# FerrisMind/candle-video

Hardware: AMD Instinct MI355X
Metric: frames/sec end-to-end LTX-Video-2B 512x768x97; DiT step ms; VAE decode ms (higher is better)
Workload: dtype bf16; 1 GPU; LTX-Video-0.9.8-2B-distilled 512x768x97, 7 steps (configs.rs:223-240), untiled VAE decode; preset=0.9.8-2b-distilled, denoise_steps=7, parallelism=replicas x1 (no data-path collective)

## Files before the change

candle-video_amd/csrc/capi_ops.hip:

```cpp
#include "conv3d.h"
#include "../../include/ltxhip_ops.h"
#include "../../include/ltxhip_upsampler_st.h"
#include "../../include/ltxhip_stg.h"
#include "../../include/ltxhip_stepcache.h"

static inline int dtc(int d) { return d == 1 ? LTX_DT_BF16 : LTX_DT_F32; }

extern "C" int ltx_op_linear(const void* x, const void* w, const void* bias, void* y, int M, int N, int K, int dtype, int epi,
                             const void* resid, const float* gate, int rows_per_batch, ltx_stream stream) {
    if (!x || !w || !y) LTX_FAIL(LTX_ERR_ARG, "ltx_op_linear: null tensor");
    if (epi < 0 || epi > 3) LTX_FAIL(LTX_ERR_ARG, "ltx_op_linear: epi must be 0..3");
    if ((epi == 2 || epi == 3) && !resid) LTX_FAIL(LTX_ERR_ARG, "ltx_op_linear: residual epilogue needs resid");
    if (epi == 2 && (!gate || rows_per_batch < 1)) LTX_FAIL(LTX_ERR_ARG, "ltx_op_linear: gated epilogue needs gate");
    GemmArgs g; g.A = x; g.W = w; g.C = y; g.bias = bias; g.resid = resid; g.gate = gate;
    g.M = M; g.N = N; g.K = K; g.lda = K; g.ldc = N; g.ldr = N; g.rows_per_batch = rows_per_batch > 0 ? rows_per_batch : 1; g.gate_stride = N;
    return ltx_launch_gemm(g, dtc(dtype), epi, (hipStream_t)stream);
}

extern "C" int64_t ltx_op_ring_packed_bytes(int N, int K) { return (int64_t)ltx_ring_packed_bytes(N, K); }
extern "C" int ltx_op_ring_pack(const void* w, int N, int K, void* out, ltx_stream stream) { return ltx_pack_ring_weights(w, N, K, out, (hipStream_t)stream); }
extern "C" int ltx_op_linear_packed(const void* x, const void* w, const void* w_packed, const void* bias, void* y, int M, int N, int K, int epi,
                                    const void* resid, const float* gate, int rows_per_batch, ltx_stream stream) {
    if (!x || !w || !w_packed || !y) LTX_FAIL(LTX_ERR_ARG, "ltx_op_linear_packed: null tensor");
    if (epi < 0 || epi > 3) LTX_FAIL(LTX_ERR_ARG, "ltx_op_linear_packed: epi must be 0..3");
    if ((epi == 2 || epi == 3) && !resid) LTX_FAIL(LTX_ERR_ARG, "ltx_op_linear_packed: residual epilogue needs resid");
    if (epi == 2 && (!gate || rows_per_batch < 1)) LTX_FAIL(LTX_ERR_ARG, "ltx_op_linear_packed: gated epilogue needs gate");
    GemmArgs g; g.A = x; g.W = w; g.Wp = w_packed; g.C = y; g.bias = bias; g.resid = resid; g.gate = gate;
    g.M = M; g.N = N; g.K = K; g.lda = K; g.ldc = N; g.ldr = N; g.rows_per_batch = rows_per_batch > 0 ? rows_per_batch : 1; g.gate_stride = N;
    return ltx_launch_gemm(g, LTX_DT_BF16, epi, (hipStream_t)stream);
}

extern "C" int ltx_op_linear_rowsq(const void* x, const void* w, const void* bias, void* y, float* rowsq, int M, int N, int K, int dtype, int epi,
                                   const void* resid, const float* gate, int rows_per_batch, ltx_stream stream) {
    if (!x || !w || !y || !rowsq) LTX_FAIL(LTX_ERR_ARG, "ltx_op_linear_rowsq: null tensor");
    if (epi != 0 && epi != 2 && epi != 3) LTX_FAIL(LTX_ERR_ARG, "ltx_op_linear_rowsq: epi must be 0, 2 or 3");
    if (epi >= 2 && !resid) LTX_FAIL(LTX_ERR_ARG, "ltx_op_linear_rowsq: residual epilogue needs resid");
    if (epi == 2 && (!gate || rows_per_batch < 1)) LTX_FAIL(LTX_ERR_ARG, "ltx_op_linear_rowsq: gated epilogue needs gate");
    GemmArgs g; g.A = x; g.W = w; g.C = y; g.bias = bias; g.resid = resid; g.gate = gate; g.M = M; g.N = N; g.K = K; g.lda = K; g.ldc = N; g.ldr = N;
    g.rows_per_batch = rows_per_batch > 0 ? rows_per_batch : 1; g.gate_stride = N; g.rowsq = rowsq;
    return ltx_launch_gemm(g, dtc(dtype), epi, (hipStream_t)stream);
}
extern "C" int ltx_op_rowsq(const void* x, int64_t rows, int N, int ld, float* rowsq, int dtype, ltx_stream stream) {
    return ltx_launch_rowsq(x, dtc(dtype), rows, N, ld, rowsq, (hipStream_t)stream);
}

namespace {
GemmArgs fold_out_args(const void* x, const void* w, const void* bias, void* y, void* y2, float* rowsq, const float* scale2, int scale2_stride,
                       int M, int N, int K, const void* resid, const float* gate, int rows_per_batch) {
    GemmArgs g; g.A = x; g.W = w; g.C = y; g.bias = bias; g.resid = resid; g.gate = gate; g.M = M; g.N = N; g.K = K; g.lda = K; g.ldc = N; g.ldr = N;
    g.rows_per_batch = rows_per_batch > 0 ? rows_per_batch : 1; g.gate_stride = N; g.rowsq = rowsq;
    g.C2 = y2; g.scale2 = scale2; g.scale2_stride = scale2_stride;
    return g;
}
GemmArgs fold_in_args(const void* x, const void* w, void* y, const float* rs_sq, int rs_n, int rs_D, float eps, const float* cvec, int cvec_stride,
                      int M, int N, int K, int rows_per_batch) {
    GemmArgs g; g.A = x; g.W = w; g.C = y; g.M = M; g.N = N; g.K = K; g.lda = K; g.ldc = N;
    g.rows_per_batch = rows_per_batch > 0 ? rows_per_batch : 1;
// ... 98 lines not shown
    a.presum = presum; a.presum_n = presum_n;
    return ltx_launch_rownorm(a, dtc(dtype), (hipStream_t)stream);
}

extern "C" int ltx_op_timestep_embedding(const float* timesteps_host, int n, int vae_flavour, float multiplier, int dtype, void* out, ltx_stream stream) {
    if (!timesteps_host || !out) LTX_FAIL(LTX_ERR_ARG, "ltx_op_timestep_embedding: null argument");
    if (n < 1 || n > 8) LTX_FAIL(LTX_ERR_ARG, "ltx_op_timestep_embedding: batch must be 1..8");
    float tab[128]; ltx_sinusoid_table(vae_flavour, tab);
    float* dtab = nullptr;
    HIP_TRY(hipMalloc((void**)&dtab, sizeof(tab)));
    int rc = LTX_OK;
    if (hipMemcpy(dtab, tab, sizeof(tab), hipMemcpyHostToDevice) != hipSuccess) rc = LTX_ERR_HIP;
    if (rc == LTX_OK) {
        TimeVec tv; tv.n = n;
        for (int i = 0; i < n; ++i) tv.t[i] = timesteps_host[i];
        rc = ltx_launch_sinusoid(out, dtc(dtype), tv, dtab, 128, dtc(dtype) == LTX_DT_BF16, multiplier, (hipStream_t)stream);
        if (rc == LTX_OK && hipStreamSynchronize((hipStream_t)stream) != hipSuccess) rc = LTX_ERR_HIP;
    }
    (void)hipFree(dtab);
    return rc;
}

extern "C" int ltx_op_qknorm_rope(void* x, int64_t rows, int D, int ld, const void* weight, float eps,
                                  const float* cos, const float* sin, int dtype, ltx_stream stream) {
    if (!x || !weight) LTX_FAIL(LTX_ERR_ARG, "ltx_op_qknorm_rope: null tensor");
    QkNormRopeArgs a; a.x = x; a.rows = rows; a.D = D; a.ld = ld; a.nseg = 1; a.w0 = weight; a.eps = eps; a.cos = cos; a.sin = sin;
    return ltx_launch_qknorm_rope(a, dtc(dtype), (hipStream_t)stream);
}

extern "C" int ltx_op_qknorm_rope_segs(void* x, int64_t rows, int D, int ld, int nseg, int64_t seg_stride, const void* w0, const void* w1, const void* w0b,
                                       float eps, const float* cos, const float* sin, float out_scale0, int dtype, ltx_stream stream) {
    if (!x || !w0) LTX_FAIL(LTX_ERR_ARG, "ltx_op_qknorm_rope_segs: null tensor");
    if ((cos == nullptr) != (sin == nullptr) || seg_stride < 0) LTX_FAIL(LTX_ERR_ARG, "ltx_op_qknorm_rope_segs: cos and sin go together; seg_stride >= 0");
    QkNormRopeArgs a; a.x = x; a.rows = rows; a.D = D; a.ld = ld; a.nseg = nseg; a.seg_stride = seg_stride; a.w0 = w0; a.w1 = w1; a.w0b = w0b;
    a.eps = eps; a.cos = cos; a.sin = sin; a.out_scale0 = out_scale0;
    return ltx_launch_qknorm_rope(a, dtc(dtype), (hipStream_t)stream);
}

extern "C" int ltx_op_norm_route(int64_t rows, int D, int dtype, int kind, int flags, int act, int64_t rows_per_batch, int presum_n, int nparts, char* name, int cap) {
    if (!name || cap < 1 || rows < 1 || D < 1 || presum_n < 0 || nparts < 0 || (flags & ~7)) LTX_FAIL(LTX_ERR_ARG, "ltx_op_norm_route: bad argument");
    NormRouteArgs r;
    r.dtype = dtc(dtype); r.rows = rows; r.D = D; r.kind = kind; r.act = act; r.rows_per_batch = rows_per_batch > 0 ? rows_per_batch : 1;
    r.scale = (flags & LTX_NORM_SCALE) != 0; r.shift = (flags & LTX_NORM_SHIFT) != 0; r.weight = (flags & LTX_NORM_WEIGHT) != 0;
    r.presum = presum_n != 0; r.presum_n = presum_n; r.parts = nparts != 0; r.nparts = nparts;
    snprintf(name, (size_t)cap, "%s", ltx_rownorm_route_name(ltx_rownorm_route(r).route));
    return LTX_OK;
}
extern "C" int ltx_op_qknorm_route(int64_t rows, int D, int dtype, char* name, int cap) {
    if (!name || cap < 1 || rows < 1 || D < 1) LTX_FAIL(LTX_ERR_ARG, "ltx_op_qknorm_route: bad argument");
    snprintf(name, (size_t)cap, "%s", ltx_qknorm_route_name(ltx_qknorm_route(dtc(dtype), rows, D, nullptr)));
    return LTX_OK;
}

extern "C" int ltx_op_rope_table(float* cos, float* sin, const float* coords, int B, int F, int H, int W, int D,
                                 const float* rope_scale_host, ltx_stream stream) {
    if (!cos || !sin) LTX_FAIL(LTX_ERR_ARG, "ltx_op_rope_table: null tensor");
    int steps = D / 6; if (steps < 1) steps = 1;
    std::vector<float> fr(steps);
    const float theta_ln = (float)std::log(10000.0);
    for (int i = 0; i < steps; ++i) {
        float lin = steps <= 1 ? 0.0f : (float)i * (float)(1.0 / (double)(steps - 1));
        fr[i] = (float)std::exp((double)(lin * theta_ln)) * (float)(M_PI / 2.0);
    }
    float* dfr = nullptr;
    HIP_TRY(hipMalloc((void**)&dfr, sizeof(float) * steps));
    HIP_TRY(hipMemcpy(dfr, fr.data(), sizeof(float) * steps, hipMemcpyHostToDevice));
    RopeTableArgs r; r.cos = cos; r.sin = sin; r.freqs = dfr; r.B = B; r.D = D;
    if (coords) { r.use_coords = 1; r.coords = coords; r.F = 1; r.H = 1; r.W = F * H * W;
                  r.gscale[0] = (float)(1.0 / 20.0); r.gscale[1] = (float)(1.0 / 2048.0); r.gscale[2] = (float)(1.0 / 2048.0); }
    else { r.F = F; r.H = H; r.W = W;
           if (rope_scale_host) { r.gscale[0] = (float)((double)rope_scale_host[0] / 20.0); r.gscale[1] = (float)((double)rope_scale_host[1] / 2048.0); r.gscale[2] = (float)((double)rope_scale_host[2] / 2048.0); } }
    int rc = ltx_launch_rope_table(r, (hipStream_t)stream);
    hipError_t e = hipStreamSynchronize((hipStream_t)stream);
    (void)hipFree(dfr);
    if (rc != LTX_OK) return rc;
    if (e != hipSuccess) { ltx_set_error(hipGetErrorString(e)); return LTX_ERR_HIP; }
    return LTX_OK;
}

extern "C" int ltx_op_attention(const void* q, const void* k, const void* v, void* o, int B, int Sq, int Sk, int heads, int hd,
                                int ldq, int ldk, int ldv, int ldo, float scale, const float* key_bias, int dtype, ltx_stream stream) {
    if (!q || !k || !v || !o) LTX_FAIL(LTX_ERR_ARG, "ltx_op_attention: null tensor");
    AttnArgs a; a.q = q; a.k = k; a.v = v; a.o = o; a.ldq = ldq; a.ldk = ldk; a.ldv = ldv; a.ldo = ldo;
    a.B = B; a.Sq = Sq; a.Sk = Sk; a.heads = heads; a.hd = hd; a.scale = scale; a.bias = key_bias;
    return ltx_launch_attention(a, dtc(dtype), (hipStream_t)stream);
}

extern "C" int ltx_op_attention_rowsq(const void* q, const void* k, const void* v, void* o, int B, int Sq, int Sk, int heads, int hd,
                                      int ldq, int ldk, int ldv, int ldo, float scale, const float* key_bias,
                                      const float* q_rowsq, int q_rowsq_n, int q_rowsq_D, float q_rowsq_eps, ltx_stream stream) {
    if (!q || !k || !v || !o || !q_rowsq) LTX_FAIL(LTX_ERR_ARG, "ltx_op_attention_rowsq: null tensor");
    AttnArgs a; a.q = q; a.k = k; a.v = v; a.o = o; a.ldq = ldq; a.ldk = ldk; a.ldv = ldv; a.ldo = ldo;
    a.B = B; a.Sq = Sq; a.Sk = Sk; a.heads = heads; a.hd = hd; a.scale = scale; a.bias = key_bias;
    a.q_rowsq = q_rowsq; a.q_rowsq_n = q_rowsq_n; a.q_rowsq_D = q_rowsq_D; a.q_rowsq_eps = q_rowsq_eps;
    return ltx_launch_attention(a, LTX_DT_BF16, (hipStream_t)stream);
}

extern "C" int ltx_op_attention_compact(const void* q, const void* k, const void* v, void* o, int B, int Sq, int Sk, int heads, int hd,
                                        int ldq, int ldk, int ldv, int ldo, float scale, const float* key_bias,
                                        const float* q_rowsq, int q_rowsq_n, int q_rowsq_D, float q_rowsq_eps, int* counts_out, ltx_stream stream) {
    if (!q || !k || !v || !o || !key_bias) LTX_FAIL(LTX_ERR_ARG, "ltx_op_attention_compact: null tensor");
    if (!ltx_attention_cross64_ok(hd, Sk) || B < 1 || ldk != heads * hd || ldv != heads * hd) LTX_FAIL(LTX_ERR_ARG, "ltx_op_attention_compact: bf16, head_dim 64, at most 128 keys, dense k / v rows");
    hipStream_t s = (hipStream_t)stream;
    const int D = heads * hd;
    void *kc = nullptr, *vc = nullptr, *bc = nullptr, *idx = nullptr, *cnt = nullptr;
    auto free_all = [&]() { for (void* p : {kc, vc, bc, idx, cnt}) if (p) (void)hipFree(p); };
    const size_t rows = (size_t)B * Sk;
    if (hipMalloc(&kc, rows * D * 2) != hipSuccess || hipMalloc(&vc, rows * D * 2) != hipSuccess || hipMalloc(&bc, rows * 4) != hipSuccess ||
        hipMalloc(&idx, rows * 4) != hipSuccess || hipMalloc(&cnt, (size_t)B * 4) != hipSuccess) { free_all(); LTX_FAIL(LTX_ERR_HIP, "hipMalloc"); }
    int rc = ltx_launch_key_compact(key_bias, B, Sk, (int*)idx, (int*)cnt, (float*)bc, s);
    if (rc == LTX_OK) rc = ltx_launch_gather_rows(k, kc, (const int*)idx, (const int*)cnt, 1, B, Sk, D * 2, s);
    if (rc == LTX_OK) rc = ltx_launch_gather_rows(v, vc, (const int*)idx, (const int*)cnt, 1, B, Sk, D * 2, s);
    if (rc == LTX_OK) {
        AttnArgs a; a.q = q; a.k = kc; a.v = vc; a.o = o; a.ldq = ldq; a.ldk = D; a.ldv = D; a.ldo = ldo;
        a.B = B; a.Sq = Sq; a.Sk = Sk; a.heads = heads; a.hd = hd; a.scale = scale; a.bias = (const float*)bc; a.k_count = (const int*)cnt;
        if (q_rowsq) { a.q_rowsq = q_rowsq; a.q_rowsq_n = q_rowsq_n; a.q_rowsq_D = q_rowsq_D; a.q_rowsq_eps = q_rowsq_eps; }
        rc = ltx_launch_attention(a, LTX_DT_BF16, s);
    }
    if (rc == LTX_OK && counts_out && hipMemcpyAsync(counts_out, cnt, (size_t)B * 4, hipMemcpyDeviceToDevice, s) != hipSuccess) rc = LTX_ERR_HIP;
    const hipError_t e = hipStreamSynchronize(s);
    free_all();
    if (rc != LTX_OK) return rc;
    if (e != hipSuccess) { ltx_set_error(hipGetErrorString(e)); return LTX_ERR_HIP; }
    return LTX_OK;
}

extern "C" int ltx_op_xattn_fold_route(int dtype, int head_dim, int heads, int D, int KP, int B, int compact, int* fold) {
    if (!fold) LTX_FAIL(LTX_ERR_ARG, "ltx_op_xattn_fold_route: null result");
    *fold = ltx_xattn_fold_route(dtc(dtype), head_dim, heads, D, KP, B, compact != 0) ? 1 : 0;
    return LTX_OK;
// ... 201 lines not shown
```

candle-video_amd/csrc/dit.hip:

```cpp
#include <cstring>
#include <deque>
#include "model_util.h"
#include "options.h"
#include "../../include/ltxhip_cond.h"
#include "../../include/ltxhip_stg.h"
#include "../../include/ltxhip_stepcache.h"
#include "../host/step_cache.h"
#include "lora.h"

struct DitBlock {
    LinearW qkv1, o1, q2, kv2, o2, ff1, ff2;
    void *nq1 = nullptr, *nk1 = nullptr, *nq2 = nullptr, *nk2 = nullptr;
};

struct DitCtx {
    const void* enc = nullptr; const float* mask = nullptr;
    int B = 0, K = 0, iodt = 0; bool valid = false;
    bool fold_q2 = false;
    DevBuf kv, bias;
    bool compact = false;
    DevBuf kvc, biasc, kidx, kcount;
    bool fold_vo = false, vo_oom = false; int KP = 0, fold_opt = 0;
    DevBuf vo, votab; std::vector<XFoldPtrs> votab_host; int counts_host[8] = {0};
    void release() { kv.release(); bias.release(); kvc.release(); biasc.release(); kidx.release(); kcount.release(); vo.release(); votab.release(); valid = false; }
};

struct DitTimeEntry {
    float t[8] = {0}; int B = 0; hipStream_t stream = nullptr; bool valid = false; uint64_t used = 0;
    DevBuf ada, adaf;
    DevBuf cfold; bool cfold_valid = false;
    void release() { ada.release(); adaf.release(); cfold.release(); valid = cfold_valid = false; }
};
struct DitWfold {
    float t = 0.f; hipStream_t stream = nullptr; bool valid = false; uint64_t used = 0; DevBuf w;
    void release() { w.release(); valid = false; }
};
constexpr int kDitTimeEntries = 64;
struct DitGroupEntry {
    std::vector<float> t; int B = 0, G = 0; hipStream_t stream = nullptr; bool valid = false; uint64_t used = 0;
    DevBuf ada, adaf, cfold; bool cfold_valid = false;
    void release() { ada.release(); adaf.release(); cfold.release(); valid = cfold_valid = false; }
};
constexpr int kDitGroupEntries = 8;

struct ltx_dit {
    ltx_dit_config cfg{};
    int dtype = LTX_DT_BF16;
    int device = 0;
    int D = 0;
    LinearW proj_in, te1, te2, te_lin, cap1, cap2, proj_out;
    void* sst_final = nullptr;
    void* sst_blocks = nullptr;
    std::vector<DitBlock> blocks;
    float* rope_freqs = nullptr;
    float* inv_freq = nullptr;
    std::vector<int> skip_blocks;
    int stg_mode = LTX_STG_TRANSFORMER_BLOCK;
    std::deque<DitCtx> ctxs;
    bool ctx_mode = false;
    std::deque<DitTimeEntry> tcache; uint64_t tclock = 0;
    std::deque<DitWfold> wcache;
    std::deque<DitGroupEntry> gcache;
    bool wfold_off = false;
    struct { bool valid = false; const float* coords = nullptr; float rs[3] = {0, 0, 0}; bool has_rs = false; int B = 0, S = 0, F = 0, H = 0, W = 0; hipStream_t stream = nullptr; } rope_key;
    uint64_t weights_epoch = 0;
    void invalidate_weight_derived() {
        ++weights_epoch;
        for (auto& e : wcache) e.valid = false;
        for (auto& e : ctxs) e.valid = false;
        for (auto& e : tcache) e.cfold_valid = false;
        for (auto& e : gcache) e.cfold_valid = false;
    }
    void release_scaled_weights() { for (auto& e : wcache) e.release(); }
    void release_caches() { auto all = [](auto& c) { for (auto& e : c) e.release(); c.clear(); }; all(ctxs); all(tcache); all(wcache); all(gcache); }
    std::vector<void*> owned;
    struct LoraSlots { void* base[7] = {nullptr}; void* merged[7] = {nullptr}; };
    std::vector<LoraSlots> lora_w;
    int n_adapters = 0;
    DevBuf xin, encin, h, n, qkv, attn, ff, c1, encp, kv2, tproj, e1, emb, embs, temb, ada, adaf, cosb, sinb, bias, orig, orig_hsq, outT, rsq, hsq, parts;
    void free_all() {
        for (void* p : owned) if (p) (void)hipFree(p);
        owned.clear();
        for (auto& ls : lora_w) for (void*& p : ls.merged) if (p) { (void)hipFree(p); p = nullptr; }
        lora_w.clear();
        DevBuf* bs[] = {&xin, &encin, &h, &n, &qkv, &attn, &ff, &c1, &encp, &kv2, &tproj, &e1, &emb, &embs, &temb, &ada, &adaf, &cosb, &sinb, &bias, &orig, &orig_hsq, &outT, &rsq, &hsq, &parts};
        for (DevBuf* b : bs) b->release();
        release_caches();
    }
};

struct ltx_step_cache {
    ltx_dit* dit = nullptr;
    struct Row { bool valid = false; int S = 0; uint64_t epoch = 0; };
    std::vector<Row> rows;
    DevBuf prev, resid, parts, sums;
    int64_t prev_rows = 0; int resid_S = 0;
    double* host = nullptr;
    hipStream_t stream = nullptr; bool used = false;
    StepCacheState st;
    void forget() { st = StepCacheState(); for (auto& r : rows) r.valid = false; }
    void* resid_row(int row) const { return (char*)resid.p + (size_t)row * resid_S * dit->D * ltx_dt_size(dit->dtype); }
    const char* row_unusable(int row, int S) const {
        const Row& r = rows[(size_t)row];
        if (!r.valid) return "holds no residual (never computed, or the cache was reset)";
        if (r.S != S) return "holds the residual of another sequence length";
        if (r.epoch != dit->weights_epoch) return "holds a residual of other weights (the adapters changed)";
        return nullptr;
    }
};
struct StepCacheUse { ltx_step_cache* c = nullptr; int row0 = 0; bool reuse = false; };

namespace {

int own_linear(ltx_dit* m, const WeightMap& wm, const std::string& prefix, int in, int out, LinearW* l) {
    LTX_TRY(ltx_load_linear(wm, prefix, in, out, m->dtype, l));
    m->owned.push_back(l->w); if (l->b) m->owned.push_back(l->b);
    return LTX_OK;
// ... 376 lines not shown
    *out = ctx;
    if (ctx) return LTX_OK;
    if (m->ctxs.size() >= 4 || !m->ctx_mode) { for (auto& e : m->ctxs) e.valid = false; }
    for (auto& e : m->ctxs) if (!e.valid) { ctx = &e; break; }
    if (!ctx) { m->ctxs.emplace_back(); ctx = &m->ctxs.back(); }
    ctx->enc = enc; ctx->mask = enc_mask; ctx->B = B; ctx->K = K; ctx->iodt = p.iodt; ctx->fold_q2 = p.fold_q2;
    ctx->fold_opt = ltx_opt().xattn_fold_vo; ctx->fold_vo = false; ctx->KP = 0; ctx->vo_oom = false;
    LTX_TRY(ctx->kv.ensure((size_t)L * MK * 2 * D * esz)); LTX_TRY(ctx->bias.ensure(MK * sizeof(float)));
    ctx->compact = enc_mask && dt == LTX_DT_BF16 && ltx_attention_cross64_ok(c.attention_head_dim, K) && ltx_opt().xattn_compact;
    if (ctx->compact) {
        LTX_TRY(ctx->kvc.ensure((size_t)L * MK * 2 * D * esz)); LTX_TRY(ctx->biasc.ensure(MK * sizeof(float)));
        LTX_TRY(ctx->kidx.ensure(MK * sizeof(int))); LTX_TRY(ctx->kcount.ensure((size_t)B * sizeof(int)));
    }
    if (enc_mask) LTX_TRY(ltx_launch_mask_bias(ctx->bias.as<float>(), enc_mask, MK, s));
    if (ctx->compact) LTX_TRY(ltx_launch_key_compact(ctx->bias.as<float>(), B, K, ctx->kidx.as<int>(), ctx->kcount.as<int>(), ctx->biasc.as<float>(), s));
    const int H = c.num_attention_heads, hd = c.attention_head_dim;
    if (ctx->compact && B <= 8 && ltx_xattn_fold_route(dt, hd, H, D, 32, B, true)) {
        HIP_TRY(hipMemcpyAsync(ctx->counts_host, ctx->kcount.p, (size_t)B * sizeof(int), hipMemcpyDeviceToHost, s));
        HIP_TRY(hipStreamSynchronize(s));
        ctx->KP = ltx_xattn_fold_kp(ctx->counts_host, B);
        ctx->fold_vo = vo_wanted(m, p, ctx);
        if (ctx->fold_vo) {
            (void)ltx_take_oom();
            int rc = ctx->vo.ensure((size_t)L * B * D * H * ctx->KP * esz);
            if (rc == LTX_OK) rc = ctx->votab.ensure((size_t)L * sizeof(XFoldPtrs));
            if (rc != LTX_OK) {
                if (!ltx_take_oom()) return rc;
                ctx->fold_vo = false; ctx->vo_oom = true;
            }
        }
    }
    LTX_TRY(ltx_launch_cast(enc, p.iodt, m->encin.p, dt, MK * c.caption_channels, s));
    LTX_TRY(ltx_linear(m->cap1, m->encin.p, c.caption_channels, m->c1.p, D, (int)MK, dt, EPI_GELU, s));
    LTX_TRY(ltx_linear(m->cap2, m->c1.p, D, m->encp.p, D, (int)MK, dt, EPI_BIAS, s));
    for (int l = 0; l < L; ++l) {
        void* kvl = (char*)ctx->kv.p + (size_t)l * MK * 2 * D * esz;
        LTX_TRY(ltx_linear(m->blocks[l].kv2, m->encp.p, D, kvl, 2 * D, (int)MK, dt, EPI_BIAS, s));
        QkNormRopeArgs k2; k2.x = kvl; k2.rows = MK; k2.D = D; k2.ld = 2 * D; k2.nseg = 1; k2.w0 = m->blocks[l].nk2; k2.eps = 1e-5f;
        if (p.fold_q2) k2.w0b = m->blocks[l].nq2;
        LTX_TRY(ltx_launch_qknorm_rope(k2, dt, s));
    }
    if (ctx->compact) LTX_TRY(ltx_launch_gather_rows(ctx->kv.p, ctx->kvc.p, ctx->kidx.as<int>(), ctx->kcount.as<int>(), L, B, K, (int)(2 * D * esz), s));
    if (ctx->fold_vo) {
        ctx->votab_host.resize(L);
        for (int l = 0; l < L; ++l) ctx->votab_host[l] = XFoldPtrs{m->blocks[l].o2.w, (const char*)ctx->kvc.p + ((size_t)l * MK * 2 * D + D) * esz};
        HIP_TRY(hipMemcpyAsync(ctx->votab.p, ctx->votab_host.data(), (size_t)L * sizeof(XFoldPtrs), hipMemcpyHostToDevice, s));
        XFoldArgs fa; fa.tab = ctx->votab.as<XFoldPtrs>(); fa.vo = ctx->vo.p; fa.L = L; fa.B = B; fa.K = K; fa.ldv = 2 * D; fa.D = D; fa.H = H; fa.KP = ctx->KP;
        LTX_TRY(ltx_launch_xattn_fold(fa, s));
    }
    ctx->valid = true;
    *out = ctx;
    return LTX_OK;
}
int rope_tables(ltx_dit* m, const DitPlan& p, int num_frames, int height, int width, const float* rope_scale, const float* video_coords, hipStream_t s) {
    const ltx_dit_config& c = m->cfg;
    auto& rk = m->rope_key;
    const bool same = m->ctx_mode && rk.valid && rk.coords == video_coords && rk.B == p.B && rk.S == p.S && rk.F == num_frames && rk.H == height && rk.W == width &&
                      rk.stream == s && rk.has_rs == (rope_scale != nullptr) && (!rope_scale || !memcmp(rk.rs, rope_scale, sizeof(rk.rs)));
    if (same) return LTX_OK;
    rk.valid = false;
    RopeTableArgs r;
    r.cos = m->cosb.as<float>(); r.sin = m->sinb.as<float>(); r.freqs = m->rope_freqs;
    r.B = p.B; r.D = p.D;
    if (video_coords) {
        r.use_coords = 1; r.coords = video_coords; r.F = 1; r.H = 1; r.W = p.S;
        r.gscale[0] = (float)(1.0 / 20.0); r.gscale[1] = (float)(1.0 / 2048.0); r.gscale[2] = (float)(1.0 / 2048.0);
    } else {
        r.F = num_frames; r.H = height; r.W = width;
        if (rope_scale) {
            r.gscale[0] = (float)((double)rope_scale[0] * c.patch_size_t / 20.0);
            r.gscale[1] = (float)((double)rope_scale[1] * c.patch_size / 2048.0);
            r.gscale[2] = (float)((double)rope_scale[2] * c.patch_size / 2048.0);
        }
    }
    LTX_TRY(ltx_launch_rope_table(r, s));
    rk.coords = video_coords; rk.B = p.B; rk.S = p.S; rk.F = num_frames; rk.H = height; rk.W = width; rk.stream = s;
    rk.has_rs = rope_scale != nullptr; if (rope_scale) memcpy(rk.rs, rope_scale, sizeof(rk.rs));
    rk.valid = m->ctx_mode;
    return LTX_OK;
}

struct DitCarry {
    bool hsq_valid = false;
    bool hs_valid = false;
    bool hsq_saved = false;
    bool pending = false; const float* pend_gate = nullptr; const void* pend_bias = nullptr;
    void take_pending(RowNormArgs& rn, const ltx_dit* m, const DitPlan& p) {
        if (!pending) return;
        rn.parts = m->parts.as<float>(); rn.nparts = p.ff2_parts; rn.part_stride = p.M * p.D; rn.d_bias = pend_bias; rn.d_gate = pend_gate; rn.d_gate_stride = 6 * p.D;
        rn.x_out = m->h.p; pending = false;
    }
};
struct DitLayerIn {
    DitTables tab; const DitWfold* we = nullptr; const DitCtx* ctx = nullptr; const float* skip_layer_mask = nullptr;
    bool fold_vo = false;
};
bool block_runs(const ltx_dit* m, const float* skip_layer_mask, int B, int l) {
    for (int sb : m->skip_blocks) if (sb == l) return false;
    if (m->stg_mode != LTX_STG_TRANSFORMER_BLOCK) return true;
    bool all = skip_layer_mask != nullptr;
    for (int b = 0; all && b < B; ++b) all = skip_layer_mask[(size_t)l * B + b] == 1.f;
    return !all;
}
int next_block(const ltx_dit* m, const float* skip_layer_mask, int B, int l) {
    for (int n = l + 1; n < m->cfg.num_layers; ++n) if (block_runs(m, skip_layer_mask, B, n)) return n;
    return -1;
}

int dit_block(ltx_dit* m, const DitPlan& p, int l, const DitLayerIn& in, DitCarry& st, hipStream_t s) {
    const ltx_dit_config& c = m->cfg;
    const int dt = p.dt, D = p.D, B = p.B, S = p.S, NB = p.NB, H = c.num_attention_heads, hd = c.attention_head_dim;
    const int64_t M = p.M; const size_t esz = ltx_dt_size(dt);
    const bool wf = in.we != nullptr, fold_out = p.nfold && !wf;
    const DitBlock& b = m->blocks[l];
    TimeVec mv; mv.n = B; bool any = false;
    for (int i = 0; i < 8; ++i) mv.t[i] = 0.f;
    if (in.skip_layer_mask) for (int bb = 0; bb < B; ++bb) { mv.t[bb] = in.skip_layer_mask[(size_t)l * B + bb]; any |= mv.t[bb] != 0.f; }
    const bool stg_attn = any && m->stg_mode != LTX_STG_TRANSFORMER_BLOCK;
    unsigned char pert[8] = {0};
    if (stg_attn) { for (int bb = 0; bb < B; ++bb) pert[bb] = mv.t[bb] != 0.f; any = false; }
    if (any) {
        HIP_TRY(hipMemcpyAsync(m->orig.p, m->h.p, M * D * esz, hipMemcpyDeviceToDevice, s));
        st.hsq_saved = p.presum && st.hsq_valid;
        if (st.hsq_saved) { LTX_TRY(m->orig_hsq.ensure(M * (D / 128) * sizeof(float))); HIP_TRY(hipMemcpyAsync(m->orig_hsq.p, m->hsq.p, M * (D / 128) * sizeof(float), hipMemcpyDeviceToDevice, s)); }
    }
    const int ln = fold_out ? next_block(m, in.skip_layer_mask, B, l) : -1;
    const float* ada = in.tab.ada + (size_t)l * NB * 6 * D;
    DitOperands x{m->h.p, m->n.p, m->qkv.p, m->attn.p, m->ff.p, m->rsq.as<float>(), m->hsq.as<float>(), m->parts.as<float>(), ada,
                  ln >= 0 ? in.tab.ada + (size_t)ln * NB * 6 * D : nullptr, p.nfold ? in.tab.cfold + (size_t)l * NB * 7 * D : nullptr,
                  wf ? (const char*)in.we->w.p + (size_t)l * 7 * D * D * esz : nullptr, c.norm_eps};
    const DitForm fold_in_form = wf ? kFold2 : kFold1;
    RowNormArgs rn; rn.x = m->h.p; rn.y = m->n.p; rn.rows = M; rn.D = D; rn.ldx = D; rn.ldy = D;
    rn.kind = 0; rn.eps = c.norm_eps; rn.shift = ada; rn.scale = ada + D; rn.rows_per_batch = p.Sg; rn.mod_stride = 6 * D;
    if (p.presum && st.hsq_valid) { rn.presum = m->hsq.as<float>(); rn.presum_n = D / 128; }
    const bool fold1 = p.nfold && st.hsq_valid && (wf || st.hs_valid);
    if (!fold1) { st.take_pending(rn, m, p); LTX_TRY(ltx_launch_rownorm(rn, dt, s)); }
    st.hs_valid = false;
    rn.parts = nullptr; rn.nparts = 0; rn.x_out = nullptr; rn.d_bias = nullptr; rn.d_gate = nullptr;
    LTX_TRY(ltx_launch_gemm(gemm_qkv1(p, fold1 ? fold_in_form : kPass, b, x), dt, EPI_BIAS, s));
    const float attn_scale = 1.0f / std::sqrt((float)hd);
    QkNormRopeArgs qa; qa.x = m->qkv.p; qa.rows = M; qa.D = D; qa.ld = p.ldqkv; qa.seg_stride = p.seg; qa.nseg = 2; qa.w0 = b.nq1; qa.w1 = b.nk1;
    qa.eps = 1e-5f; qa.cos = m->cosb.as<float>(); qa.sin = m->sinb.as<float>();
    if (p.fold_q) qa.out_scale0 = attn_scale * 1.4426950408889634f;
    LTX_TRY(ltx_launch_qknorm_rope(qa, dt, s));
    AttnArgs at; at.q = m->qkv.p; at.k = (char*)m->qkv.p + (size_t)p.seg * esz; at.v = (char*)m->qkv.p + (size_t)2 * p.seg * esz; at.o = m->attn.p;
    at.ldq = at.ldk = at.ldv = p.ldqkv; at.ldo = D; at.B = B; at.Sq = S; at.Sk = S; at.heads = H; at.hd = hd; at.scale = attn_scale;
    at.q_prescaled = p.fold_q ? 1 : 0;
    if (!stg_attn) LTX_TRY(ltx_launch_attention(at, dt, s));
    else {
        auto for_runs = [&](bool perturbed, auto&& fn) -> int {
            for (int b0 = 0; b0 < B; ++b0) {
                int b1 = b0;
                while (b1 < B && (pert[b1] != 0) == perturbed) ++b1;
                if (b1 > b0) { LTX_TRY(fn(b0, b1)); b0 = b1; }
            }
            return LTX_OK;
        };
        LTX_TRY(for_runs(false, [&](int b0, int b1) {
            AttnArgs ar = at; ar.B = b1 - b0;
            const size_t in_off = (size_t)b0 * S * p.ldqkv * esz;
            ar.q = (const char*)at.q + in_off; ar.k = (const char*)at.k + in_off; ar.v = (const char*)at.v + in_off; ar.o = (char*)at.o + (size_t)b0 * S * D * esz;
            return ltx_launch_attention(ar, dt, s);
        }));
        if (m->stg_mode == LTX_STG_ATTENTION_VALUES) LTX_TRY(ltx_launch_stg_fill(m->attn.p, D, at.v, p.ldqkv, pert, B, S, D, dt, s));
        else if (!fold1) LTX_TRY(ltx_launch_stg_fill(m->attn.p, D, m->n.p, D, pert, B, S, D, dt, s));
        else
            LTX_TRY(for_runs(true, [&](int b0, int b1) {
                RowNormArgs rp = rn; rp.presum = nullptr; rp.presum_n = 0;
                const size_t row_off = (size_t)b0 * S * D * esz, tab_off = (size_t)b0 * (NB / B) * 6 * D;
                rp.x = (const char*)m->h.p + row_off; rp.y = (char*)m->attn.p + row_off; rp.rows = (int64_t)(b1 - b0) * S;
                rp.shift = ada + tab_off; rp.scale = ada + D + tab_off;
                return ltx_launch_rownorm(rp, dt, s);
            }));
    }
    LTX_TRY(ltx_linear(b.o1, m->attn.p, D, m->h.p, D, (int)M, dt, EPI_GATE_RESID, s, m->h.p, D, ada + 2 * D, 6 * D, p.Sg));
    st.hsq_valid = false;
    const DitCtx* ctx = in.ctx;
    const char* kvl = (const char*)(ctx->compact ? ctx->kvc.p : ctx->kv.p) + (size_t)l * p.MK * 2 * D * esz;
    AttnArgs ax; ax.q = m->qkv.p; ax.k = kvl; ax.v = kvl + (size_t)D * esz; ax.o = m->attn.p;
    ax.ldq = D; ax.ldk = ax.ldv = 2 * D; ax.ldo = D; ax.B = B; ax.Sq = S; ax.Sk = p.K; ax.heads = H; ax.hd = hd; ax.scale = attn_scale;
    ax.bias = ctx->mask ? ctx->bias.as<float>() : nullptr;
    if (ctx->compact) { ax.bias = ctx->biasc.as<float>(); ax.k_count = ctx->kcount.as<int>(); }
    const int HK = H * ctx->KP;
    if (in.fold_vo) { ax.p_out = m->attn.p; ax.ldp = HK; ax.o = nullptr; }
    if (p.fold_q2) {
        LTX_TRY(ltx_launch_gemm(gemm_q2(p, b, x), dt, EPI_BIAS, s));
        ax.q_rowsq = m->rsq.as<float>(); ax.q_rowsq_n = D / 128; ax.q_rowsq_D = D; ax.q_rowsq_eps = 1e-5f;
    } else {
        LTX_TRY(linear_of(b.q2, gemm_q2(p, b, x), dt, EPI_BIAS, s));
        QkNormRopeArgs q2; q2.x = m->qkv.p; q2.rows = M; q2.D = D; q2.ld = D; q2.nseg = 1; q2.w0 = b.nq2; q2.eps = 1e-5f;
        LTX_TRY(ltx_launch_qknorm_rope(q2, dt, s));
    }
    LTX_TRY(ltx_launch_attention(ax, dt, s));
    if (in.fold_vo) {
        for (int bb = 0; bb < B; ++bb) {
            const DitVo vo{(const char*)ctx->vo.p + (size_t)l * B * D * HK * esz, HK, bb};
            LTX_TRY(ltx_launch_gemm(gemm_o2(p, fold_out ? kFold1 : kPass, b, x, &vo), dt, EPI_RESID, s));
        }
        st.hs_valid = fold_out;
    } else if (fold_out) { LTX_TRY(ltx_launch_gemm(gemm_o2(p, kFold1, b, x), dt, EPI_RESID, s)); st.hs_valid = true; }
    else LTX_TRY(linear_of(b.o2, gemm_o2(p, kPass, b, x), dt, EPI_RESID, s));
    st.hsq_valid = p.presum;
    if (p.nfold && st.hsq_valid && (wf || st.hs_valid)) LTX_TRY(ltx_launch_gemm(gemm_ff1(p, fold_in_form, b, x), dt, EPI_GELU, s));
    else {
        rn.shift = ada + 3 * D; rn.scale = ada + 4 * D;
        rn.presum = nullptr; rn.presum_n = 0;
        if (p.presum && st.hsq_valid) { rn.presum = m->hsq.as<float>(); rn.presum_n = D / 128; }
        LTX_TRY(ltx_launch_rownorm(rn, dt, s));
        LTX_TRY(linear_of(b.ff1, gemm_ff1(p, kPass, b, x), dt, EPI_GELU, s));
    }
    st.hs_valid = false;
    if (p.defer_ff2) {
        LTX_TRY(ltx_launch_gemm(gemm_ff2(p, kDefer, b, x), dt, EPI_BIAS, s));
        st.pending = true; st.pend_gate = ada + 5 * D; st.pend_bias = b.ff2.b;
    } else if (ln >= 0) { LTX_TRY(ltx_launch_gemm(gemm_ff2(p, kFold1, b, x), dt, EPI_GATE_RESID, s)); st.hs_valid = true; }
    else LTX_TRY(linear_of(b.ff2, gemm_ff2(p, kPass, b, x), dt, EPI_GATE_RESID, s));
    st.hsq_valid = p.presum;
    if (!any) return LTX_OK;
    LTX_TRY(ltx_launch_skip_blend(m->h.p, m->orig.p, mv, S, D, dt, s));
    bool binary = true;
    for (int bb = 0; bb < B; ++bb) binary &= mv.t[bb] == 0.f || mv.t[bb] == 1.f;
    if (st.hsq_valid && st.hsq_saved && binary) {
        const size_t rowb = (size_t)S * (D / 128) * sizeof(float);
        for (int bb = 0; bb < B; ++bb)
            if (mv.t[bb] == 1.f) HIP_TRY(hipMemcpyAsync((char*)m->hsq.p + bb * rowb, (const char*)m->orig_hsq.p + bb * rowb, rowb, hipMemcpyDeviceToDevice, s));
    } else st.hsq_valid = false;
    st.hs_valid = false;
    if (fold_out && st.hsq_valid && ln >= 0) { LTX_TRY(ltx_launch_mod_scale(m->h.p, x.ada_next + D, 6 * D, m->n.p, NB, p.Sg, D, dt, s)); st.hs_valid = true; }
    return LTX_OK;
}

int dit_forward_b8(ltx_dit* m, const void* hidden, const void* enc, const float* timestep, int G,
                   const float* enc_mask, int B, int S, int K, int num_frames, int height, int width,
                   const float* rope_scale, const float* video_coords, const float* skip_layer_mask,
                   ltx_dtype io_dtype, void* out, ltx_stream stream, const StepCacheUse* sc = nullptr) {
    if (B < 1 || B > 8) LTX_FAIL(LTX_ERR_ARG, "ltx_dit_forward: internal batch chunk must be 1..8");
    if (S < 1 || K < 1) LTX_FAIL(LTX_ERR_ARG, "ltx_dit_forward: empty sequence");
    if (!video_coords && (int64_t)num_frames * height * width != S)
        LTX_FAIL(LTX_ERR_ARG, "ltx_dit_forward: num_frames*height*width must equal S when video_coords is absent");
    HIP_TRY(hipSetDevice(m->device));
    if (G < 1 || S % G != 0) LTX_FAIL(LTX_ERR_ARG, "ltx_dit_forward: the modulation groups must divide the sequence");
    hipStream_t s = (hipStream_t)stream;
    const ltx_dit_config& c = m->cfg;
    const DitPlan p = ltx_dit_plan(c, m->dtype, io_dtype == LTX_BF16 ? LTX_DT_BF16 : LTX_DT_F32, B, S, K, G, skip_layer_mask != nullptr);
    const int dt = p.dt, D = p.D, L = c.num_layers;
    const int64_t M = p.M, MK = p.MK; const size_t esz = ltx_dt_size(dt);
    const size_t nte = p.NB == p.B ? (size_t)p.B : 8;
    const size_t MD = M * D * esz, KD = MK * D * esz, part = M * (D / 128) * sizeof(float), rope = M * (D / 2) * sizeof(float);
    const std::pair<DevBuf*, size_t> ws[] = {
        {&m->xin, M * c.in_channels * esz}, {&m->encin, MK * c.caption_channels * esz}, {&m->h, MD}, {&m->n, MD}, {&m->qkv, 3 * MD}, {&m->attn, MD}, {&m->ff, 4 * MD},
        {&m->c1, KD}, {&m->encp, KD}, {&m->kv2, 2 * KD}, {&m->tproj, nte * 256 * esz}, {&m->e1, nte * D * esz}, {&m->emb, nte * D * esz}, {&m->embs, nte * D * esz},
        {&m->temb, nte * 6 * D * esz}, {&m->cosb, rope}, {&m->sinb, rope}, {&m->bias, MK * sizeof(float)}, {&m->outT, M * c.out_channels * esz},
        {&m->rsq, p.fold_q2 ? part : 0}, {&m->hsq, p.presum ? part : 0}, {&m->parts, p.defer_ff2 ? (size_t)p.ff2_parts * M * D * sizeof(float) : 0}, {&m->orig, skip_layer_mask ? MD : 0}};
    for (const auto& w : ws) LTX_TRY(w.first->ensure(w.second));
    const bool reuse = sc && sc->reuse;
    if (reuse) {
        for (int b = 0; b < B; ++b)
            if (const char* why = sc->c->row_unusable(sc->row0 + b, S))
                LTX_FAIL(LTX_ERR_ARG, "ltx_dit_forward_cached: reuse asked of cache row " + std::to_string(sc->row0 + b) + ", which " + why);
    } else if (sc) {
        ltx_step_cache* k = sc->c;
        if (k->resid_S != S) { for (auto& r : k->rows) r.valid = false; k->resid_S = S; }
        LTX_TRY(k->resid.ensure(k->rows.size() * (size_t)S * D * esz));
        for (int b = 0; b < B; ++b) k->rows[(size_t)sc->row0 + b].valid = false;
    }

    LTX_TRY(ltx_launch_cast(hidden, p.iodt, m->xin.p, dt, p.M * c.in_channels, s));
    if (reuse) LTX_TRY(ltx_linear(m->proj_in, m->xin.p, c.in_channels, m->h.p, D, (int)p.M, dt, EPI_RESID, s, sc->c->resid_row(sc->row0), D));
    else LTX_TRY(ltx_linear(m->proj_in, m->xin.p, c.in_channels, m->h.p, D, (int)p.M, dt, EPI_BIAS, s));
    if (sc && !reuse) HIP_TRY(hipMemcpyAsync(sc->c->resid_row(sc->row0), m->h.p, MD, hipMemcpyDeviceToDevice, s));

    DitLayerIn in; in.skip_layer_mask = skip_layer_mask;
    DitPlan pt = p; if (reuse) pt.nfold = false;
    LTX_TRY(G == 1 ? time_tables(m, pt, timestep, B, s, &in.tab) : group_tables(m, pt, timestep, s, &in.tab));
    DitCtx* ctx = nullptr;
    DitCarry st;
    if (!reuse) {
        LTX_TRY(scaled_weights(m, p, timestep, in.tab.ada, s, &in.we));
        LTX_TRY(text_context(m, p, enc, enc_mask, s, &ctx)); in.ctx = ctx;
        in.fold_vo = ctx->fold_vo;
        LTX_TRY(rope_tables(m, p, num_frames, height, width, rope_scale, video_coords, s));

        for (int l = 0; l < L; ++l)
            if (block_runs(m, skip_layer_mask, B, l)) LTX_TRY(dit_block(m, p, l, in, st, s));
    }
    const bool resid_late = sc && !reuse && st.pending;
    if (sc && !reuse && !resid_late) LTX_TRY(ltx_launch_step_residual(m->h.p, sc->c->resid_row(sc->row0), p.M, D, dt, s));

    RowNormArgs rn; rn.x = m->h.p; rn.y = m->n.p; rn.rows = p.M; rn.D = D; rn.ldx = D; rn.ldy = D;
    rn.kind = 1; rn.eps = 1e-6f; rn.shift = in.tab.adaf; rn.scale = in.tab.adaf + (size_t)p.NB * D;
    rn.rows_per_batch = p.Sg; rn.mod_stride = D;
    st.take_pending(rn, m, p);
    LTX_TRY(ltx_launch_rownorm(rn, dt, s));
    if (resid_late) LTX_TRY(ltx_launch_step_residual(m->h.p, sc->c->resid_row(sc->row0), p.M, D, dt, s));
    if (sc && !reuse)
        for (int b = 0; b < B; ++b) sc->c->rows[(size_t)sc->row0 + b] = {true, S, m->weights_epoch};
    void* dst = p.iodt == dt ? out : m->outT.p;
    LTX_TRY(ltx_linear(m->proj_out, m->n.p, D, dst, c.out_channels, (int)p.M, dt, EPI_BIAS, s));
    if (p.iodt != dt) LTX_TRY(ltx_launch_cast(m->outT.p, dt, out, p.iodt, p.M * c.out_channels, s));
    if (ctx && !m->ctx_mode) ctx->valid = false;
    return LTX_OK;
// ... 6 lines not shown
    const size_t esz = io_dtype == LTX_BF16 ? 2 : 4;
    const int L = m->cfg.num_layers;
    if (skip_layer_mask && m->stg_mode != LTX_STG_TRANSFORMER_BLOCK)
        for (size_t i = 0; i < (size_t)L * B; ++i)
            if (skip_layer_mask[i] != 0.f && skip_layer_mask[i] != 1.f)
                LTX_FAIL(LTX_ERR_ARG, "ltx_dit_forward: skip_layer_mask[" + std::to_string(i / B) + ", " + std::to_string(i % B) + "] = " + std::to_string(skip_layer_mask[i]) +
                                      ": the attention STG modes take 0 and 1 only (fractional masks: LTX_STG_TRANSFORMER_BLOCK)");
    std::vector<float> mask_chunk;
    float t_row[8];
    for (int b0 = 0; b0 < B; b0 += 8) {
        const int bc = B - b0 < 8 ? B - b0 : 8;
        const float* slm = skip_layer_mask;
        if (skip_layer_mask && bc != B) {
            mask_chunk.resize((size_t)L * bc);
            for (int l = 0; l < L; ++l) for (int b = 0; b < bc; ++b) mask_chunk[(size_t)l * bc + b] = skip_layer_mask[(size_t)l * B + b0 + b];
            slm = mask_chunk.data();
        }
        const float* tc = timestep + (size_t)b0 * (F ? F : 1);
        int G = 1;
        if (F) {
            bool uniform = true;
            for (int b = 0; b < bc; ++b) for (int f = 1; f < F; ++f) uniform = uniform && memcmp(&tc[(size_t)b * F + f], &tc[(size_t)b * F], sizeof(float)) == 0;
            if (uniform) { for (int b = 0; b < bc; ++b) t_row[b] = tc[(size_t)b * F]; tc = t_row; } else G = F;
        }
        StepCacheUse use; if (sc) { use = *sc; use.row0 += b0; }
        LTX_TRY(dit_forward_b8(m, (const char*)hidden + (size_t)b0 * S * m->cfg.in_channels * esz, enc ? (const char*)enc + (size_t)b0 * K * m->cfg.caption_channels * esz : nullptr,
                               tc, G, enc_mask ? enc_mask + (size_t)b0 * K : nullptr, bc, S, K, num_frames, height, width, rope_scale,
                               video_coords ? video_coords + (size_t)b0 * S * 3 : nullptr, slm, io_dtype,
                               (char*)out + (size_t)b0 * S * m->cfg.out_channels * esz, stream, sc ? &use : nullptr));
    }
    return LTX_OK;
}

}

extern "C" int ltx_dit_forward(ltx_dit* m, const void* hidden, const void* enc, const float* timestep,
                               const float* enc_mask, int B, int S, int K, int num_frames, int height, int width,
                               const float* rope_scale, const float* video_coords, const float* skip_layer_mask,
                               ltx_dtype io_dtype, void* out, ltx_stream stream) {
    if (!m || !hidden || !enc || !timestep || !out) LTX_FAIL(LTX_ERR_ARG, "ltx_dit_forward: null argument");
    if (B < 1) LTX_FAIL(LTX_ERR_ARG, "ltx_dit_forward: batch must be at least 1");
    return dit_forward_chunks(m, hidden, enc, timestep, 0, enc_mask, B, S, K, num_frames, height, width, rope_scale, video_coords, skip_layer_mask, io_dtype, out, stream);
}

extern "C" int ltx_dit_forward_frames(ltx_dit* m, const void* hidden, const void* enc, const float* timestep,
                                      const float* enc_mask, int B, int S, int K, int num_frames, int height, int width,
                                      const float* rope_scale, const float* video_coords, const float* skip_layer_mask,
                                      ltx_dtype io_dtype, void* out, ltx_stream stream) {
    if (!m || !hidden || !enc || !timestep || !out) LTX_FAIL(LTX_ERR_ARG, "ltx_dit_forward_frames: null argument");
    if (B < 1) LTX_FAIL(LTX_ERR_ARG, "ltx_dit_forward_frames: batch must be at least 1");
    if (num_frames < 1 || height < 1 || width < 1 || (int64_t)num_frames * height * width != S)
        LTX_FAIL(LTX_ERR_ARG, "ltx_dit_forward_frames: S must equal num_frames*height*width (tokens in pack order, with or without video_coords)");
    return dit_forward_chunks(m, hidden, enc, timestep, num_frames, enc_mask, B, S, K, num_frames, height, width, rope_scale, video_coords, skip_layer_mask, io_dtype, out, stream);
}

extern "C" int ltx_dit_context_cache(ltx_dit* m, int enable) {
    if (!m) LTX_FAIL(LTX_ERR_ARG, "ltx_dit_context_cache: null handle");
    for (auto& e : m->ctxs) e.valid = false;
    m->rope_key.valid = false;
    m->ctx_mode = enable != 0;
    return LTX_OK;
}

extern "C" void ltx_step_cache_params_default(ltx_step_cache_params* p) {
    if (!p) return;
    const StepCachePolicy d;
    p->rel_l1_thresh = d.thresh; for (int k = 0; k < 5; ++k) p->coeff[k] = d.coeff[k];
    p->pattern = nullptr; p->n_pattern = 0;
}

extern "C" int ltx_step_cache_create(ltx_dit* dit, int rows, ltx_step_cache** out) {
    if (!dit || !out) LTX_FAIL(LTX_ERR_ARG, "ltx_step_cache_create: null argument");
    *out = nullptr;
    if (rows < 1) LTX_FAIL(LTX_ERR_ARG, "ltx_step_cache_create: rows must be at least 1, got " + std::to_string(rows));
    if (!ltx_step_measure_blocks(1, dit->D, dit->dtype))
        LTX_FAIL(LTX_ERR_UNSUPPORTED, "ltx_step_cache_create: inner dim " + std::to_string(dit->D) + " is not a multiple of 128 the measure kernel serves");
    HIP_TRY(hipSetDevice(dit->device));
    ltx_step_cache* c = new ltx_step_cache();
    c->dit = dit; c->rows.resize((size_t)rows);
    int rc = c->sums.ensure(2 * sizeof(double));
    if (rc == LTX_OK && hipHostMalloc((void**)&c->host, 2 * sizeof(double), hipHostMallocDefault) != hipSuccess) {
        (void)hipGetLastError(); ltx_set_error("ltx_step_cache_create: hipHostMalloc of the result pair"); rc = LTX_ERR_HIP;
    }
    if (rc != LTX_OK) { c->sums.release(); delete c; return rc; }
    *out = c;
    return LTX_OK;
}

extern "C" void ltx_step_cache_destroy(ltx_step_cache* c) {
    if (!c) return;
    (void)hipSetDevice(c->dit->device);
    if (c->used) (void)hipStreamSynchronize(c->stream);
    c->prev.release(); c->resid.release(); c->parts.release(); c->sums.release();
    if (c->host) (void)hipHostFree(c->host);
    delete c;
}

extern "C" int ltx_step_cache_reset(ltx_step_cache* c) {
    if (!c) LTX_FAIL(LTX_ERR_ARG, "ltx_step_cache_reset: null handle");
    c->forget();
    return LTX_OK;
}

static int step_cache_policy_of(const ltx_step_cache_params* params, const char* who, StepCachePolicy* pol) {
    if (!params) LTX_FAIL(LTX_ERR_ARG, std::string(who) + ": null step cache parameters");
    pol->thresh = params->rel_l1_thresh; for (int k = 0; k < 5; ++k) pol->coeff[k] = params->coeff[k];
// ... 192 lines not shown
```

candle-video_amd/csrc/kernels.h:

```cpp
#pragma once
#include <hip/hip_runtime.h>
#include <hip/hip_ext.h>
#include <stdint.h>

enum { LTX_DT_F32 = 0, LTX_DT_BF16 = 1 };
static inline size_t ltx_dt_size(int dt) { return dt == LTX_DT_BF16 ? 2 : 4; }

enum { LTX_PROF_GEMM = 0, LTX_PROF_CONV = 1, LTX_PROF_ATTN_SELF = 2, LTX_PROF_ATTN_CROSS = 3, LTX_PROF_ROWNORM = 4, LTX_PROF_NKINDS = 5 };
bool ltx_prof_begin(int kind, double work, hipStream_t s, void** token);
void ltx_prof_end(void* token, hipStream_t s);
enum { LTX_PROFK_GEMM128 = 0, LTX_PROFK_GEMM_BIG = 1, LTX_PROFK_GEMM_P8 = 2, LTX_PROFK_CONV_HALO = 3, LTX_PROFK_GEMM_ASM = 4, LTX_PROFK_GEMM_ASM16 = 5, LTX_PROFK_GEMM_RING = 6, LTX_PROFK_N = 7 };
void ltx_prof_kernel(int which);
bool ltx_prof_kernel_events(hipEvent_t* a, hipEvent_t* b);
#define LTX_LAUNCH_TIMED(kernel, grid, block, shmem, stream, ...) do {                                           \
        hipEvent_t _pa = nullptr, _pb = nullptr;                                                                   \
        if (ltx_prof_kernel_events(&_pa, &_pb)) hipExtLaunchKernelGGL(kernel, grid, block, shmem, stream, _pa, _pb, 0, __VA_ARGS__); \
        else hipLaunchKernelGGL(kernel, grid, block, shmem, stream, __VA_ARGS__);                                  \
    } while (0)

enum { EPI_BIAS = 0, EPI_GELU = 1, EPI_GATE_RESID = 2, EPI_RESID = 3, EPI_D2S = 4, EPI_UNPATCH = 5, EPI_S2D = 6, EPI_D2S_G = 7 };

struct GemmArgs {
    const void* A = nullptr;
    const void* W = nullptr;
// ... 72 lines not shown
struct RowNormArgs {
    const void* x = nullptr; void* y = nullptr;
    int64_t rows = 0; int D = 0; int ldx = 0, ldy = 0;
    int kind = 0;
    float eps = 1e-6f;
    const void* weight = nullptr;
    const float* scale = nullptr;
    const float* shift = nullptr;
    int64_t rows_per_batch = 1; int mod_stride = 0;
    int act = 0;
    const float* presum = nullptr; int presum_n = 0;
    const float* parts = nullptr; int nparts = 0; int64_t part_stride = 0;
    const void* d_bias = nullptr; const float* d_gate = nullptr; int d_gate_stride = 0; void* x_out = nullptr;
};
int ltx_launch_rownorm(const RowNormArgs& a, int dtype, hipStream_t s);

enum NormRoute { NORM_REFUSED = 0, NORM_NARROW, NORM_BLOCK, NORM_WIDE, NORM_REREAD, NORM_PRESUM, NORM_PRESUM_LEAN,
                 NORM_WIDE_DEFER, NORM_WIDE_DEFER4, NORM_BLOCK_DEFER, NORM_BLOCK_DEFER4,
                 NORM_WIDE_ROWS };
struct NormRouteArgs {
    int dtype = LTX_DT_BF16; int64_t rows = 0; int D = 0; int kind = 0;
    bool scale = false, shift = false, weight = false; int act = 0; int64_t rows_per_batch = 1;
    bool presum = false; int presum_n = 0;
    bool parts = false; int nparts = 0;
};
struct NormDecision {
    NormRoute route = NORM_REFUSED; const char* why = nullptr;
    int presum_r = 4; bool presum_wide = false, presum_nt = false;
};
NormRouteArgs ltx_rownorm_route_args(const RowNormArgs& a, int dtype);
NormDecision ltx_rownorm_route(const NormRouteArgs& r);
const char* ltx_rownorm_route_name(NormRoute r);

struct StepMeasureArgs {
    const void* h = nullptr; void* prev = nullptr;
    const float* shift = nullptr; const float* scale = nullptr; int mod_stride = 0;
    int64_t rows = 0; int D = 0; int64_t rows_per_batch = 1; float eps = 1e-6f; int first = 0;
    double* part = nullptr;
};
int64_t ltx_step_measure_blocks(int64_t rows, int D, int dtype);
int ltx_launch_step_measure(const StepMeasureArgs& a, int dtype, hipStream_t s);
int ltx_launch_step_measure_finish(const double* part, int64_t nblk, double* sums, hipStream_t s);
int ltx_launch_step_residual(const void* h, void* r, int64_t rows, int D, int dtype, hipStream_t s);

struct QkNormRopeArgs {
    void* x = nullptr;
    int64_t rows = 0; int D = 0; int ld = 0; int nseg = 1;
    int64_t seg_stride = 0;
    const void* w0 = nullptr; const void* w1 = nullptr;
    const void* w0b = nullptr;
    float eps = 1e-5f;
    const float* cos = nullptr; const float* sin = nullptr;
    float out_scale0 = 1.f;
};
int ltx_launch_qknorm_rope(const QkNormRopeArgs& a, int dtype, hipStream_t s);
enum QkNormRoute { QKNORM_REFUSED = 0, QKNORM_BLOCK, QKNORM_FUSED4, QKNORM_FUSED8, QKNORM_CACHED, QKNORM_REREAD };
QkNormRoute ltx_qknorm_route(int dtype, int64_t rows, int D, const char** why);
const char* ltx_qknorm_route_name(QkNormRoute r);

struct RopeTableArgs {
    float* cos = nullptr; float* sin = nullptr;
    const float* coords = nullptr;
    const float* freqs = nullptr;
    int B = 1, F = 1, H = 1, W = 1, D = 0;
    int use_coords = 0;
    float gscale[3] = {1.f, 1.f, 1.f};
};
int ltx_launch_rope_table(const RopeTableArgs& a, hipStream_t s);

struct AttnArgs {
    const void* q = nullptr; const void* k = nullptr; const void* v = nullptr; void* o = nullptr;
    int ldq = 0, ldk = 0, ldv = 0, ldo = 0;
    int B = 1, Sq = 0, Sk = 0, heads = 0, hd = 0;
    float scale = 1.f;
    const float* bias = nullptr;
    const float* bias2d = nullptr;
    int q_prescaled = 0;
    int xcd_heads = 0;
    int wide_o = 0;
    const float* q_rowsq = nullptr; int q_rowsq_n = 0, q_rowsq_D = 0; float q_rowsq_eps = 0.f;
    const int* k_count = nullptr;
    void* p_out = nullptr; int ldp = 0;
    const int* gate_flag = nullptr; int gate_ticket = 0;
};
bool ltx_attention_q128_fits(const AttnArgs& a);
int ltx_launch_attention_q128(const AttnArgs& a, hipStream_t s, int** flag_out, int* ticket_out);
int ltx_q64_fallback_read(unsigned long long* out, int reset);
int ltx_q128_fallback_read(unsigned long long* out, int reset);
int ltx_attention_q128_prepare();
int ltx_launch_attention(const AttnArgs& a, int dtype, hipStream_t s);
int ltx_launch_attention_q64(const AttnArgs& a, hipStream_t s);
bool ltx_attention_q64_fits(const AttnArgs& a);
bool ltx_attention_prescale_ok(int hd);
bool ltx_attention_cross64_ok(int hd, int Sk);
bool ltx_xattn_fold_route(int dtype, int head_dim, int heads, int D, int KP, int B, bool compact);
int ltx_xattn_fold_kp(const int* counts_host, int B);
struct XFoldPtrs { const void* w; const void* v; };
struct XFoldArgs { const XFoldPtrs* tab = nullptr; void* vo = nullptr; int L = 0, B = 0, K = 0, ldv = 0, D = 0, H = 0, KP = 0; };
int ltx_launch_xattn_fold(const XFoldArgs& a, hipStream_t s);
bool ltx_attention_rowsq_ok(int hd, int Sk, int D);

constexpr int LTX_MAX_BATCH = 16;
struct TimeVec { float t[LTX_MAX_BATCH]; int n; };
int ltx_launch_gguf_dequant(const void* blocks_dev, int ggml_type, int64_t numel, void* dst, int dst_dtype, hipStream_t s);
int ltx_launch_sinusoid(void* out, int dtype, const TimeVec& tv, const float* tab, int half, int round_t, float tmul, hipStream_t s);
int ltx_launch_silu(const void* x, void* y, int64_t n, int dtype, hipStream_t s);
int ltx_launch_noise_inject(const void* x, void* y, const float* noise, const void* scale, const void* resid, int64_t rows, int C, int64_t HW, int dtype, hipStream_t s);
int ltx_launch_cast(const void* x, int xdt, void* y, int ydt, int64_t n, hipStream_t s);
int ltx_launch_ada(float* out, const void* tables, const void* temb, int nl, int B, int width, int dtype, hipStream_t s);
int ltx_launch_mask_bias(float* out, const float* mask, int64_t n, hipStream_t s);
int ltx_launch_key_compact(const float* bias, int B, int K, int* idx, int* count, float* bias_c, hipStream_t s);
int ltx_launch_gather_rows(const void* src, void* dst, const int* idx, const int* count, int nl, int B, int K, int row_bytes, hipStream_t s);
int ltx_launch_skip_blend(void* h, const void* orig, const TimeVec& m, int64_t rows_per_batch, int D, int dtype, hipStream_t s);
struct StgRows { int n; int b[LTX_MAX_BATCH]; };
int ltx_launch_stg_fill(void* dst, int ldd, const void* src, int lds, const unsigned char* rows_host, int B, int64_t S, int D, int dtype, hipStream_t s);
int ltx_launch_scale_cols(const void* W, const float* scale, void* out, int64_t N, int K, int dtype, hipStream_t s);
int ltx_launch_mod_scale(const void* h, const float* scale, int scale_stride, void* y, int B, int64_t rows_per_batch, int D, int dtype, hipStream_t s);

struct GroupIdx { int v[128]; };
// ... 52 lines not shown
```

candle-video_amd/csrc/model_util.h:

```cpp
#pragma once
#include <map>
#include <memory>
#include <string>
#include <vector>
#include <cmath>
#include "common.h"
#include "kernels.h"
#include "../../include/ltxhip.h"
#include "../../include/ltxhip_stepcache.h"

void ltx_note_oom();
bool ltx_take_oom();

struct DevBuf {
    void* p = nullptr;
    size_t bytes = 0;
    int ensure(size_t n) {
        if (n <= bytes) return LTX_OK;
        if (p) { HIP_TRY(hipDeviceSynchronize()); HIP_TRY(hipFree(p)); p = nullptr; bytes = 0; }
        const hipError_t e = hipMalloc(&p, n);
        if (e != hipSuccess) {
            p = nullptr;
            if (e == hipErrorOutOfMemory) ltx_note_oom();
            (void)hipGetLastError();
// ... 9 lines not shown
struct LinearW {
    void* w = nullptr;
    void* b = nullptr;
    int in = 0, out = 0;
    mutable std::shared_ptr<void> wp;
    mutable bool wp_tried = false;
};

struct WeightMap {
    std::map<std::string, const ltx_weight*> m;
    WeightMap(const ltx_weight* w, size_t n) { for (size_t i = 0; i < n; ++i) if (w[i].name) m[w[i].name] = &w[i]; }
    const ltx_weight* find(const std::string& k) const { auto it = m.find(k); return it == m.end() ? nullptr : it->second; }
};

static inline int64_t ltx_numel(const ltx_weight* w) {
    int64_t n = 1;
    for (int i = 0; i < w->ndim; ++i) n *= w->shape[i];
    return n;
}

int ltx_upload_cast(const ltx_weight* w, void* dst, int dst_dtype, int64_t expect_numel, const std::string& name);
int ltx_load_tensor(const WeightMap& wm, const std::string& name, int64_t numel, int dtype, void** out, bool optional = false);
int ltx_load_linear(const WeightMap& wm, const std::string& prefix, int in, int out, int dtype, LinearW* l);
int ltx_stage_src(const ltx_weight* w, const void** dev_src, void** temp_to_free);

inline void ltx_sinusoid_table(int vae_flavour, float tab[128]) {
    if (!vae_flavour) {
        for (int i = 0; i < 128; ++i) { const float ex = (float)i / 128.0f; const float pw = (float)std::pow(10000.0, (double)ex); tab[i] = 1.0f / pw; }
    } else {
        const float coef = (float)(-std::log(10000.0) / 128.0);
        for (int i = 0; i < 128; ++i) { const float x = (float)i * coef; tab[i] = (float)std::exp((double)x); }
    }
}

int ltx_linear(const LinearW& l, const void* x, int lda, void* y, int ldc, int M, int dtype, int epi, hipStream_t s,
               const void* resid = nullptr, int ldr = 0, const float* gate = nullptr, int gate_stride = 0, int rows_per_batch = 1,
               float* rowsq = nullptr);

struct DitPlan {
    int dt = 0, iodt = 0, D = 0, B = 0, S = 0, K = 0;
    int64_t M = 0, MK = 0;
    int NB = 0, Sg = 0;
    int64_t seg = 0; int ldqkv = 0;
    bool fold_q2 = false;
    bool presum = false;
    bool nfold = false;
    bool defer_ff2 = false; int ff2_parts = 1;
    bool dense_qkv = false;
    bool fold_q = false;
};
DitPlan ltx_dit_plan(const ltx_dit_config& c, int dt, int iodt, int B, int S, int K, int G, bool skip_mask);

int ltx_step_cache_params_check(const ltx_step_cache_params* params, const char* who);

int ltx_pipeline_schedule(const ltx_pipeline_params* p, int S, std::vector<float>* sig, std::vector<int64_t>* ts);
```

candle-video_amd/csrc/options.cpp:

```cpp
#include "options.h"
#include <atomic>
#include <cstdio>
#include <cstdlib>
#include <cstring>
#include <map>
#include <mutex>
#include <string>
#include "errors.h"

namespace {
std::mutex g_mu;
LtxOptions g_opt;
std::atomic<bool> g_loaded{false};
std::map<std::string, int> g_exp;

struct ListBit { const char* name; unsigned bit; };
const ListBit kFam[] = {{"asm16", LTX_FAM_ASM16}, {"ring", LTX_FAM_RING}, {"p8", LTX_FAM_P8}, {"halo", LTX_FAM_HALO}, {"halo_out", LTX_FAM_HALO_OUT}, {"big", LTX_FAM_BIG}};
const ListBit kAttn[] = {{"q64", LTX_ATTN_Q64}, {"q128", LTX_ATTN_Q128}, {"cross", LTX_ATTN_CROSS}, {"pipe", LTX_ATTN_PIPE}};

template <size_t N> bool parse_list(const char* v, const ListBit (&tab)[N], unsigned* out) {
    unsigned bits = 0;
    std::string s(v ? v : "");
    size_t p = 0;
    while (p < s.size()) {
        size_t q = s.find('+', p); if (q == std::string::npos) q = s.size();
        const std::string item = s.substr(p, q - p);
        bool ok = item.empty();
        for (const auto& t : tab) if (item == t.name) { bits |= t.bit; ok = true; }
        if (!ok) return false;
        p = q + 1;
    }
    *out = bits;
    return true;
}

struct IntField { const char* name; int LtxOptions::*field; };
const IntField kInts[] = {
    {"gemm_tune", &LtxOptions::gemm_tune}, {"gemm_wide_epi", &LtxOptions::gemm_wide_epi}, {"gemm_trace", &LtxOptions::gemm_trace},
    {"attn_q64_big", &LtxOptions::attn_q64_big}, {"vae_tile_batch", &LtxOptions::vae_tile_batch}, {"prof_kernel_events", &LtxOptions::prof_kernel_events}, {"ff2_defer", &LtxOptions::ff2_defer},
    {"gemm_splitk", &LtxOptions::gemm_splitk}, {"q2_fold", &LtxOptions::q2_fold}, {"norm_presum", &LtxOptions::norm_presum}, {"norm_lean", &LtxOptions::norm_lean},
    {"xattn_compact", &LtxOptions::xattn_compact}, {"xattn_fold_vo", &LtxOptions::xattn_fold_vo}, {"dense_qkv", &LtxOptions::dense_qkv}, {"vae_fuse_norm", &LtxOptions::vae_fuse_norm}, {"t5_attn_mfma", &LtxOptions::t5_attn_mfma}, {"guidance_batch", &LtxOptions::guidance_batch}, {"norm_fold", &LtxOptions::norm_fold}, {"norm_fold_copies", &LtxOptions::norm_fold_copies}, {"attn_q64_stream", &LtxOptions::attn_q64_stream},
};

bool set_one(LtxOptions& o, const std::string& key, const char* value) {
    static const LtxOptions dflt;
    for (const auto& f : kInts) if (key == f.name) {
        if (!value) { o.*(f.field) = dflt.*(f.field); return true; }
        char* end = nullptr; const long v = strtol(value, &end, 10);
        if (end == value || *end) return false;
        o.*(f.field) = (int)v; return true;
    }
    if (key == "gemm_plan") {
        if (!value) { o.gemm_plan[0] = 0; return true; }
        if (strlen(value) >= sizeof(o.gemm_plan)) return false;
        strcpy(o.gemm_plan, value); return true;
    }
    if (key == "gemm_off") return value ? parse_list(value, kFam, &o.gemm_off) : (o.gemm_off = 0, true);
    if (key == "attn_off") return value ? parse_list(value, kAttn, &o.attn_off) : (o.attn_off = 0, true);
    if (key.rfind("x_", 0) == 0) {
        if (!value) { g_exp.erase(key); return true; }
        char* end = nullptr; const long v = strtol(value, &end, 10);
        if (end == value || *end) return false;
        g_exp[key] = (int)v; return true;
    }
    return false;
}

bool parse_string(LtxOptions& o, const char* text, std::string* bad) {
    std::string s(text ? text : "");
    size_t p = 0;
    while (p < s.size()) {
        size_t q = s.find(',', p); if (q == std::string::npos) q = s.size();
        const std::string item = s.substr(p, q - p);
        p = q + 1;
        if (item.empty()) continue;
        const size_t eq = item.find('=');
        if (eq == std::string::npos || !set_one(o, item.substr(0, eq), item.c_str() + eq + 1)) { if (bad) *bad = item; return false; }
    }
    return true;
}

void load_locked() {
    g_opt = LtxOptions(); g_exp.clear();
    std::string bad;
    if (!parse_string(g_opt, getenv("LTX_OPTIONS"), &bad))
        fprintf(stderr, "[ltx] LTX_OPTIONS: entry '%s' not understood (see include/ltxhip.h); it and what follows it are ignored\n", bad.c_str());
    g_loaded.store(true, std::memory_order_release);
}
}

const LtxOptions& ltx_opt() {
    if (!g_loaded.load(std::memory_order_acquire)) { std::lock_guard<std::mutex> lock(g_mu); if (!g_loaded.load(std::memory_order_relaxed)) load_locked(); }
// ... 50 lines not shown
```

candle-video_amd/csrc/options.h:

```cpp
#pragma once

enum { LTX_FAM_ASM16 = 1, LTX_FAM_RING = 2, LTX_FAM_P8 = 4, LTX_FAM_HALO = 8, LTX_FAM_HALO_OUT = 16, LTX_FAM_BIG = 32 };
enum { LTX_ATTN_Q64 = 1, LTX_ATTN_Q128 = 2, LTX_ATTN_CROSS = 4, LTX_ATTN_PIPE = 8 };

struct LtxOptions {
    int gemm_tune = 1;
    char gemm_plan[40] = {0};
    unsigned gemm_off = 0;
    int gemm_wide_epi = 1;
    int gemm_trace = 0;
    int attn_q64_big = -1;
    int vae_tile_batch = 0;
    int prof_kernel_events = 1;
    int ff2_defer = 1;
    int gemm_splitk = 1;
    int q2_fold = 1;
    int norm_presum = 1;
    int norm_lean = 1;
    int xattn_compact = 1;
    int xattn_fold_vo = 1;
    int attn_q64_stream = 0;
    int norm_fold = 2;
    int norm_fold_copies = 10;
    int guidance_batch = 1;
    int dense_qkv = 1;
    int vae_fuse_norm = 1;
    int t5_attn_mfma = 1;
    unsigned attn_off = 0;
};

const LtxOptions& ltx_opt();
int ltx_exp_lookup(const char* name, int dflt);
#ifdef LTX_EXPERIMENTS
#define ltx_exp(name, dflt) ltx_exp_lookup(name, dflt)
#else
#define ltx_exp(name, dflt) (dflt)
#endif
```

candle-video_amd/csrc/qknorm_rope.hip:

```cpp
#include "common.h"
#include "kernels.h"
#include "norm_common.h"
#include "options.h"

namespace {

template <typename T>
__device__ __forceinline__ void qk_finish(Chunk16 v, float rinv, int c, const T* w, const T* wb, bool rope, const Chunk16& co, const Chunk16& si, T* x, bool active) {
    constexpr int CH = ElemTraits<T>::CHUNK;
    float f[CH]; chunk_to_f32<T>(v, f);
    Chunk16 wc; wc.u = *reinterpret_cast<const u32x4*>(w + c * CH);
    float wv[CH]; chunk_to_f32<T>(wc, wv);
#pragma unroll
    for (int j = 0; j < CH; ++j) f[j] = f[j] * rinv * wv[j];
    if (wb) {
        Chunk16 wc2; wc2.u = *reinterpret_cast<const u32x4*>(wb + c * CH);
        float wv2[CH]; chunk_to_f32<T>(wc2, wv2);
#pragma unroll
        for (int j = 0; j < CH; ++j) f[j] *= wv2[j];
    }
    if (rope) {
#pragma unroll
        for (int p = 0; p < CH / 2; ++p) {
            const float re = f[2 * p], im = f[2 * p + 1];
            f[2 * p] = re * co.f[p] - im * si.f[p];
            f[2 * p + 1] = im * co.f[p] + re * si.f[p];
        }
    }
    Chunk16 o; f32_to_chunk<T>(f, o);
    if (active) *reinterpret_cast<u32x4*>(x + c * CH) = o.u;
}

template <typename T, bool CACHED>
__global__ __launch_bounds__(256) void qknorm_rope_kernel(const QkNormRopeArgs a, int lpr) {
    constexpr int CH = ElemTraits<T>::CHUNK;
    const int lane = threadIdx.x & 63, wave = threadIdx.x >> 6;
    const int rpw = 64 / lpr;
    const int64_t row = ((int64_t)blockIdx.x * 4 + wave) * rpw + lane / lpr;
    const int sub = lane % lpr;
    const bool active = row < a.rows;
    const int64_t rr = active ? row : a.rows - 1;
    const int nch = a.D / CH;
    const float* cs = a.cos ? a.cos + rr * (a.D / 2) : nullptr;
    const float* sn = a.sin ? a.sin + rr * (a.D / 2) : nullptr;
    auto finish = [&](Chunk16 v, int c, float rinv, const T* w, const T* wb, T* x) {
        float f[CH]; chunk_to_f32<T>(v, f);
        Chunk16 wc; wc.u = *reinterpret_cast<const u32x4*>(w + c * CH);
        float wv[CH]; chunk_to_f32<T>(wc, wv);
#pragma unroll
        for (int i = 0; i < CH; ++i) f[i] = f[i] * rinv * wv[i];
        if (wb) {
            Chunk16 wc2; wc2.u = *reinterpret_cast<const u32x4*>(wb + c * CH);
            float wv2[CH]; chunk_to_f32<T>(wc2, wv2);
#pragma unroll
            for (int i = 0; i < CH; ++i) f[i] *= wv2[i];
        }
        if (cs) {
            float co[CH / 2], si[CH / 2];
            if constexpr (CH == 8) {
                f32x4 c4 = *reinterpret_cast<const f32x4*>(cs + c * 4), s4 = *reinterpret_cast<const f32x4*>(sn + c * 4);
#pragma unroll
                for (int p = 0; p < 4; ++p) { co[p] = c4[p]; si[p] = s4[p]; }
            } else {
#pragma unroll
                for (int p = 0; p < CH / 2; ++p) { co[p] = cs[c * (CH / 2) + p]; si[p] = sn[c * (CH / 2) + p]; }
            }
#pragma unroll
            for (int p = 0; p < CH / 2; ++p) {
                float re = f[2 * p], im = f[2 * p + 1];
                f[2 * p] = re * co[p] - im * si[p];
                f[2 * p + 1] = im * co[p] + re * si[p];
            }
        }
        Chunk16 o; f32_to_chunk<T>(f, o);
        if (active) *reinterpret_cast<u32x4*>(x + c * CH) = o.u;
    };
    for (int seg = 0; seg < a.nseg; ++seg) {
        T* x = reinterpret_cast<T*>(a.x) + rr * a.ld + (int64_t)seg * (a.seg_stride ? a.seg_stride : a.D);
        const T* w = reinterpret_cast<const T*>(seg == 0 ? a.w0 : a.w1);
        const T* wb = seg == 0 ? reinterpret_cast<const T*>(a.w0b) : nullptr;
        const float oscale = seg == 0 ? a.out_scale0 : 1.0f;
        if constexpr (CACHED) {
            Chunk16 v[NSLOT];
#pragma unroll
            for (int i = 0; i < NSLOT; ++i) {
                int c = sub + i * lpr;
                v[i].u = (u32x4){0u, 0u, 0u, 0u};
                if (c < nch) v[i].u = *reinterpret_cast<const u32x4*>(x + c * CH);
            }
            const float rinv = rinv_qk(group_sum(cached_sq<T>(v), lpr), a.D, a.eps, oscale);
#pragma unroll
            for (int i = 0; i < NSLOT; ++i) { int c = sub + i * lpr; if (c < nch) finish(v[i], c, rinv, w, wb, x); }
        } else {
            float ss = 0.f;
            for (int c = sub; c < nch; c += lpr) { Chunk16 v; v.u = *reinterpret_cast<const u32x4*>(x + c * CH); ss = add_sq<T>(v, ss); }
            const float rinv = rinv_qk(group_sum(ss, lpr), a.D, a.eps, oscale);
            for (int c = sub; c < nch; c += lpr) { Chunk16 v; v.u = *reinterpret_cast<const u32x4*>(x + c * CH); finish(v, c, rinv, w, wb, x); }
        }
    }
}

template <typename T, int NS, int OCC = 5>
__global__ __launch_bounds__(256, OCC) void qknorm_rope_fused_kernel(const QkNormRopeArgs a, int lpr) {
    constexpr int CH = ElemTraits<T>::CHUNK;
    static_assert(CH == 8, "bf16 rows only");
    const int lane = threadIdx.x & 63, wave = threadIdx.x >> 6;
    const int rpw = 64 / lpr;
    const int64_t row = ((int64_t)blockIdx.x * 4 + wave) * rpw + lane / lpr;
    const int sub = lane % lpr;
    const bool active = row < a.rows;
    const int64_t rr = active ? row : a.rows - 1;
    const int nch = a.D / CH;
    const bool rope = a.cos != nullptr;
    const float* cs = rope ? a.cos + rr * (a.D / 2) : nullptr;
    const float* sn = rope ? a.sin + rr * (a.D / 2) : nullptr;
    T* x0 = reinterpret_cast<T*>(a.x) + rr * a.ld;
    const int64_t sst = a.seg_stride ? a.seg_stride : a.D;
    Chunk16 v[2][NS];
    Chunk16 co[NS], si[NS];
#pragma unroll
    for (int i = 0; i < NS; ++i) {
        const int c = sub + i * lpr;
        const bool in = c < nch;
        v[0][i].u = (u32x4){0u, 0u, 0u, 0u}; v[1][i].u = (u32x4){0u, 0u, 0u, 0u};
        if (in) v[0][i].u = *reinterpret_cast<const u32x4*>(x0 + c * CH);
        if (in && a.nseg == 2) v[1][i].u = *reinterpret_cast<const u32x4*>(x0 + sst + c * CH);
        if (in && rope) { co[i].u = *reinterpret_cast<const u32x4*>(cs + c * 4); si[i].u = *reinterpret_cast<const u32x4*>(sn + c * 4); }
    }
    float rinv[2] = {0.f, 0.f};
#pragma unroll
    for (int seg = 0; seg < 2; ++seg) {
        if (seg >= a.nseg) break;
        rinv[seg] = rinv_qk(group_sum(cached_sq<T>(v[seg]), lpr), a.D, a.eps, seg == 0 ? a.out_scale0 : 1.0f);
    }
#pragma unroll
    for (int i = 0; i < NS; ++i) {
        const int c = sub + i * lpr;
        if (c >= nch) continue;
#pragma unroll
        for (int seg = 0; seg < 2; ++seg) {
            if (seg >= a.nseg) break;
            const T* w = reinterpret_cast<const T*>(seg == 0 ? a.w0 : a.w1);
            const T* wb = seg == 0 ? reinterpret_cast<const T*>(a.w0b) : nullptr;
            asm volatile("" : "+v"(v[seg][i].u));
            qk_finish<T>(v[seg][i], rinv[seg], c, w, wb, rope, co[i], si[i], x0 + seg * sst, active);
            __builtin_amdgcn_sched_barrier(0);
        }
    }
}

template <typename T>
__global__ __launch_bounds__(256) void qknorm_rope_block_kernel(const QkNormRopeArgs a) {
    constexpr int CH = ElemTraits<T>::CHUNK, NC = 2;
    static_assert(CH == 8, "bf16 rows only");
    __shared__ float red[2][4];
    const int tid = threadIdx.x, lane = tid & 63, wave = tid >> 6;
    const int64_t row = blockIdx.x;
    const int nch = a.D / CH;
    const bool rope = a.cos != nullptr;
    const float* cs = rope ? a.cos + row * (a.D / 2) : nullptr;
    const float* sn = rope ? a.sin + row * (a.D / 2) : nullptr;
    T* x0 = reinterpret_cast<T*>(a.x) + row * a.ld;
    const int64_t sst = a.seg_stride ? a.seg_stride : a.D;
    Chunk16 v[2][NC];
    Chunk16 co[NC], si[NC];
#pragma unroll
    for (int i = 0; i < NC; ++i) {
        const int c = tid + i * 256;
        const bool in = c < nch;
        v[0][i].u = (u32x4){0u, 0u, 0u, 0u}; v[1][i].u = (u32x4){0u, 0u, 0u, 0u};
        if (in) v[0][i].u = *reinterpret_cast<const u32x4*>(x0 + c * CH);
        if (in && a.nseg == 2) v[1][i].u = *reinterpret_cast<const u32x4*>(x0 + sst + c * CH);
        if (in && rope) { co[i].u = *reinterpret_cast<const u32x4*>(cs + c * 4); si[i].u = *reinterpret_cast<const u32x4*>(sn + c * 4); }
    }
    float ss[2] = {cached_sq<T>(v[0]), cached_sq<T>(v[1])};
    block_sum<2>(ss, red, lane, wave);
    const float rinv[2] = {rinv_qk(ss[0], a.D, a.eps, a.out_scale0), rinv_qk(ss[1], a.D, a.eps, 1.0f)};
#pragma unroll
    for (int i = 0; i < NC; ++i) {
        const int c = tid + i * 256;
        if (c >= nch) continue;
#pragma unroll
        for (int seg = 0; seg < 2; ++seg) {
            if (seg >= a.nseg) break;
            const T* w = reinterpret_cast<const T*>(seg == 0 ? a.w0 : a.w1);
            const T* wb = seg == 0 ? reinterpret_cast<const T*>(a.w0b) : nullptr;
            qk_finish<T>(v[seg][i], rinv[seg], c, w, wb, rope, co[i], si[i], x0 + seg * sst, true);
        }
    }
}

__global__ void rope_table_kernel(const RopeTableArgs a) {
    const int half = a.D / 2;
    const int64_t S = (int64_t)a.F * a.H * a.W;
    const int64_t total = (int64_t)a.B * S * half;
    const int rem_pairs = (a.D % 6) / 2;
    for (int64_t i = (int64_t)blockIdx.x * blockDim.x + threadIdx.x; i < total; i += (int64_t)gridDim.x * blockDim.x) {
        const int p = (int)(i % half);
        const int64_t row = i / half;
        float co = 1.0f, si = 0.0f;
        if (p >= rem_pairs) {
            const int fi = p - rem_pairs;
            const int step = fi / 3, ax = fi - step * 3;
            float g;
            if (a.use_coords) {
                g = a.coords[row * 3 + ax] * a.gscale[ax];
            } else {
                const int64_t s = row % S;
                const int w = (int)(s % a.W); const int64_t t1 = s / a.W;
                const int h = (int)(t1 % a.H); const int f = (int)(t1 / a.H);
                const float idx = ax == 0 ? (float)f : (ax == 1 ? (float)h : (float)w);
                g = idx * a.gscale[ax];
            }
            const float ang = a.freqs[step] * (g * 2.0f - 1.0f);
            co = cosf(ang); si = sinf(ang);
        }
        a.cos[i] = co; a.sin[i] = si;
    }
}

}

QkNormRoute ltx_qknorm_route(int dtype, int64_t rows, int D, const char** why) {
    const int ch = dtype == LTX_DT_BF16 ? 8 : 4;
    if (D < ch || D % ch != 0) { if (why) *why = "qknorm: D/ld must be multiples of the 16-byte chunk"; return QKNORM_REFUSED; }
    const int nch = D / ch, lpr = pick_lpr(nch);
    const bool cached = nch <= NSLOT * lpr;
    if (dtype == LTX_DT_BF16) {
        if (rows <= 512 && nch > 64 && nch <= 512) return QKNORM_BLOCK;
        if (nch <= 4 * lpr) return QKNORM_FUSED4;
        if (nch <= 8 * lpr && ltx_exp("qknorm_fused8", 1)) return QKNORM_FUSED8;
    }
    return cached ? QKNORM_CACHED : QKNORM_REREAD;
}

const char* ltx_qknorm_route_name(QkNormRoute r) {
    static const char* const names[] = {"refused", "block", "fused4", "fused8", "cached", "reread"};
    return names[r];
}

int ltx_launch_qknorm_rope(const QkNormRopeArgs& a, int dtype, hipStream_t s) {
    const int ch = dtype == LTX_DT_BF16 ? 8 : 4;
    if (a.rows <= 0) return LTX_OK;
    if (a.D % ch != 0 || a.ld % ch != 0) LTX_FAIL(LTX_ERR_ARG, "qknorm: D/ld must be multiples of the 16-byte chunk");
    if (a.nseg < 1 || a.nseg > 2 || !a.w0 || (a.nseg == 2 && !a.w1)) LTX_FAIL(LTX_ERR_ARG, "qknorm: bad segments/weights");
    const char* why = nullptr;
    const QkNormRoute route = ltx_qknorm_route(dtype, a.rows, a.D, &why);
    if (route == QKNORM_REFUSED) LTX_FAIL(LTX_ERR_ARG, why);
    const int nch = a.D / ch, lpr = pick_lpr(nch);
    const int64_t rows_per_block = 4 * (64 / lpr);
    dim3 grid((unsigned)cdiv64(a.rows, rows_per_block)), block(256);
    const bool bf16 = dtype == LTX_DT_BF16;
    switch (route) {
    case QKNORM_BLOCK: hipLaunchKernelGGL((qknorm_rope_block_kernel<bf16_t>), dim3((unsigned)a.rows), block, 0, s, a); break;
    case QKNORM_FUSED4: hipLaunchKernelGGL((qknorm_rope_fused_kernel<bf16_t, 4>), grid, block, 0, s, a, lpr); break;
    case QKNORM_FUSED8: hipLaunchKernelGGL((qknorm_rope_fused_kernel<bf16_t, 8, 2>), grid, block, 0, s, a, lpr); break;
    case QKNORM_CACHED:
        if (bf16) hipLaunchKernelGGL((qknorm_rope_kernel<bf16_t, true>), grid, block, 0, s, a, lpr);
        else hipLaunchKernelGGL((qknorm_rope_kernel<float, true>), grid, block, 0, s, a, lpr);
        break;
    default:
        if (bf16) hipLaunchKernelGGL((qknorm_rope_kernel<bf16_t, false>), grid, block, 0, s, a, lpr);
        else hipLaunchKernelGGL((qknorm_rope_kernel<float, false>), grid, block, 0, s, a, lpr);
        break;
    }
    LTX_CHECK_LAUNCH();
    return LTX_OK;
}

int ltx_launch_rope_table(const RopeTableArgs& a, hipStream_t s) {
    if (a.D % 2 != 0 || a.D < 6) LTX_FAIL(LTX_ERR_ARG, "rope: dim must be even and >= 6");
    const int64_t total = (int64_t)a.B * a.F * a.H * a.W * (a.D / 2);
    int64_t blocks = cdiv64(total, 256); if (blocks > 8192) blocks = 8192;
    hipLaunchKernelGGL(rope_table_kernel, dim3((unsigned)blocks), dim3(256), 0, s, a);
    LTX_CHECK_LAUNCH();
    return LTX_OK;
}
```

candle-video_amd/host/pipeline.hip:

```cpp
#include <cmath>
#include <cstring>
#include <string>
#include <vector>
#include "../csrc/model_util.h"
#include "../csrc/options.h"
#include "../../include/ltxhip_cond.h"
#include "../../include/ltxhip_guidance.h"
#include "../../include/ltxhip_keyframes.h"
#include "../../include/ltxhip_stepcache.h"
#include "cond_plan.h"
#include "step_plan.h"

extern "C" float ltx_calculate_shift(int seq_len, int base_seq_len, int max_seq_len, float base_shift, float max_shift) {
    float m = (max_shift - base_shift) / (float)(max_seq_len - base_seq_len);
    float b = base_shift - m * (float)base_seq_len;
    return (float)seq_len * m + b;
}

extern "C" int ltx_sched_set_timesteps(const float* sigmas_in, int n, float mu, int use_mu, float shift,
                                       float shift_terminal, int use_shift_terminal, float* sigmas_out, int64_t* timesteps_out) {
    if (!sigmas_in || n < 1 || !sigmas_out) LTX_FAIL(LTX_ERR_ARG, "ltx_sched_set_timesteps: bad argument");
    std::vector<float> s(sigmas_in, sigmas_in + n);
    if (use_mu) {
        const float emu = std::exp(mu);
        for (float& v : s) { float base = std::pow(1.0f / v - 1.0f, 1.0f); v = emu / (emu + base); }
    } else {
        for (float& v : s) v = shift * v / (1.0f + (shift - 1.0f) * v);
    }
    if (use_shift_terminal) {
        const float one_minus_last = 1.0f - s[n - 1];
        const float denom = 1.0f - shift_terminal;
        if (std::fabs(denom) < 1e-12f) LTX_FAIL(LTX_ERR_ARG, "shift_terminal too close to 1.0");
        const float scale = one_minus_last / denom;
        for (float& v : s) v = 1.0f - ((1.0f - v) / scale);
    }
    for (int i = 0; i < n; ++i) {
        sigmas_out[i] = s[i];
        if (timesteps_out) timesteps_out[i] = (int64_t)(s[i] * 1000.0f);
    }
    sigmas_out[n] = 0.0f;
    return LTX_OK;
}

namespace {
double betacf(double a, double b, double x) {
    const double tiny = 1e-300;
    double c = 1.0, d = 1.0 - (a + b) * x / (a + 1.0);
    if (std::fabs(d) < tiny) d = tiny;
    d = 1.0 / d;
    double h = d;
    for (int m = 1; m <= 500; ++m) {
        const double m2 = 2.0 * m;
        double aa = m * (b - m) * x / ((a + m2 - 1.0) * (a + m2));
        d = 1.0 + aa * d; if (std::fabs(d) < tiny) d = tiny;
        c = 1.0 + aa / c; if (std::fabs(c) < tiny) c = tiny;
        d = 1.0 / d; h *= d * c;
        aa = -(a + m) * (a + b + m) * x / ((a + m2) * (a + m2 + 1.0));
        d = 1.0 + aa * d; if (std::fabs(d) < tiny) d = tiny;
        c = 1.0 + aa / c; if (std::fabs(c) < tiny) c = tiny;
        d = 1.0 / d;
        const double del = d * c;
        h *= del;
        if (std::fabs(del - 1.0) < 1e-16) break;
    }
// ... 68 lines not shown
        state = old * 6364136223846793005ULL + inc;
        uint32_t xorshifted = (uint32_t)(((old >> 18) ^ old) >> 27);
        uint32_t rot = (uint32_t)(old >> 59);
        return (xorshifted >> rot) | (xorshifted << ((0u - rot) & 31));
    }
    float next_f32() { return (float)(next_u32() >> 8) * 5.9604645e-8f; }
    void next_gaussian(float& z0, float& z1) {
        float u1;
        do { u1 = next_f32(); } while (!(u1 > 1e-7f));
        float u2 = next_f32();
        float mag = std::sqrt(-2.0f * std::log(u1));
        const float two_pi_u2 = 2.0f * 3.14159265358979323846f * u2;
        z0 = mag * std::cos(two_pi_u2); z1 = mag * std::sin(two_pi_u2);
    }
};
}

extern "C" int ltx_pcg32_randn(uint64_t seed, uint64_t inc, size_t n, float* out) {
    if (!out) LTX_FAIL(LTX_ERR_ARG, "ltx_pcg32_randn: null output");
    Pcg32 r(seed, inc);
    for (size_t i = 0; i < n; i += 2) {
        float a, b; r.next_gaussian(a, b);
        out[i] = a; if (i + 1 < n) out[i + 1] = b;
    }
    return LTX_OK;
}

extern "C" int ltx_pcg32_u32(uint64_t seed, uint64_t inc, size_t n, uint32_t* out) {
    if (!out) LTX_FAIL(LTX_ERR_ARG, "ltx_pcg32_u32: null output");
    Pcg32 r(seed, inc);
    for (size_t i = 0; i < n; ++i) out[i] = r.next_u32();
    return LTX_OK;
}

extern "C" int ltx_device_alloc(size_t bytes, int device, void** out) {
    if (!out) LTX_FAIL(LTX_ERR_ARG, "ltx_device_alloc: null output");
    HIP_TRY(hipSetDevice(device));
    HIP_TRY(hipMalloc(out, bytes ? bytes : 1));
    return LTX_OK;
}
extern "C" int ltx_device_free(void* p) { if (p) HIP_TRY(hipFree(p)); return LTX_OK; }
extern "C" int ltx_memcpy_h2d(void* dst_device, const void* src_host, size_t bytes, ltx_stream stream) {
    HIP_TRY(hipMemcpyAsync(dst_device, src_host, bytes, hipMemcpyHostToDevice, (hipStream_t)stream));
    return LTX_OK;
}
extern "C" int ltx_memcpy_d2h(void* dst_host, const void* src_device, size_t bytes, ltx_stream stream) {
    HIP_TRY(hipMemcpyAsync(dst_host, src_device, bytes, hipMemcpyDeviceToHost, (hipStream_t)stream));
    return LTX_OK;
}
extern "C" int ltx_stream_synchronize(ltx_stream stream) { HIP_TRY(hipStreamSynchronize((hipStream_t)stream)); return LTX_OK; }

extern "C" int ltx_build_video_coords(int F, int H, int W, int frame_rate, int ts_ratio, int sp_ratio, float* out) {
    if (!out || F < 1 || H < 1 || W < 1 || frame_rate < 1) LTX_FAIL(LTX_ERR_ARG, "ltx_build_video_coords: bad argument");
    const float inv_fr = (float)(1.0 / (double)frame_rate);
    size_t i = 0;
    for (int f = 0; f < F; ++f)
        for (int h = 0; h < H; ++h)
            for (int w = 0; w < W; ++w) {
                float vf = (float)f * (float)ts_ratio + (1.0f - (float)ts_ratio);
                vf = std::fmin(std::fmax(vf, 0.0f), 1000.0f) * inv_fr;
                out[i++] = vf; out[i++] = (float)h * (float)sp_ratio; out[i++] = (float)w * (float)sp_ratio;
            }
    return LTX_OK;
}

static GuidanceArgs guidance_args(const void* text, const void* uncond, const void* perturbed, ltx_dtype pred_dtype, float* latents, float* noise_pred_out,
                                  int B, int64_t n, float guidance_scale, float guidance_rescale, float stg_scale, float dt, float sigma, float sigma_next,
                                  const float* step_noise, void* stats_ws, const unsigned char* hold, int num_frames, int64_t frame_elems) {
    GuidanceArgs a;
    a.text = text; a.uncond = uncond; a.pert = perturbed; a.pred_dtype = pred_dtype == LTX_BF16 ? LTX_DT_BF16 : LTX_DT_F32;
    a.latents = latents; a.noise_out = noise_pred_out; a.B = B; a.n_per_batch = n;
    a.guidance_scale = guidance_scale; a.guidance_rescale = guidance_rescale; a.stg_scale = stg_scale;
    if (step_noise) { a.sigma = sigma; a.sigma_next = sigma_next; a.step_noise = step_noise; } else a.dt = dt;
    a.stats = reinterpret_cast<double*>(stats_ws);
    if (hold) { a.hold = hold; a.num_frames = num_frames; a.frame_elems = frame_elems; }
    return a;
}

extern "C" int ltx_guidance_step(const void* text, const void* uncond, const void* perturbed, ltx_dtype pred_dtype,
                                 float* latents, float* noise_pred_out, int B, int64_t n,
                                 float guidance_scale, float guidance_rescale, float stg_scale, float dt,
                                 void* stats_ws, ltx_stream stream) {
    return ltx_launch_guidance_step(guidance_args(text, uncond, perturbed, pred_dtype, latents, noise_pred_out, B, n, guidance_scale, guidance_rescale, stg_scale,
                                                  dt, 0.0f, 0.0f, nullptr, stats_ws, nullptr, 1, 0), (hipStream_t)stream);
}

extern "C" int ltx_guidance_step_stochastic(const void* text, const void* uncond, const void* perturbed, ltx_dtype pred_dtype,
                                            float* latents, float* noise_pred_out, int B, int64_t n,
                                            float guidance_scale, float guidance_rescale, float stg_scale,
                                            float sigma, float sigma_next, const float* step_noise,
                                            void* stats_ws, ltx_stream stream) {
    if (!step_noise || !latents) LTX_FAIL(LTX_ERR_ARG, "ltx_guidance_step_stochastic: latents and step_noise are required");
    return ltx_launch_guidance_step(guidance_args(text, uncond, perturbed, pred_dtype, latents, noise_pred_out, B, n, guidance_scale, guidance_rescale, stg_scale,
                                                  0.0f, sigma, sigma_next, step_noise, stats_ws, nullptr, 1, 0), (hipStream_t)stream);
}

extern "C" int ltx_guidance_step_held(const void* text, const void* uncond, const void* perturbed, ltx_dtype pred_dtype,
                                      float* latents, float* noise_pred_out, int B, int64_t n,
                                      float guidance_scale, float guidance_rescale, float stg_scale, float dt,
                                      void* stats_ws, const unsigned char* hold, int num_frames, int64_t frame_elems, ltx_stream stream) {
    if (!hold) LTX_FAIL(LTX_ERR_ARG, "ltx_guidance_step_held: hold is required");
    return ltx_launch_guidance_step_held(guidance_args(text, uncond, perturbed, pred_dtype, latents, noise_pred_out, B, n, guidance_scale, guidance_rescale, stg_scale,
                                                       dt, 0.0f, 0.0f, nullptr, stats_ws, hold, num_frames, frame_elems), (hipStream_t)stream);
}

extern "C" int ltx_guidance_step_stochastic_held(const void* text, const void* uncond, const void* perturbed, ltx_dtype pred_dtype,
                                                 float* latents, float* noise_pred_out, int B, int64_t n,
                                                 float guidance_scale, float guidance_rescale, float stg_scale,
                                                 float sigma, float sigma_next, const float* step_noise,
                                                 void* stats_ws, const unsigned char* hold, int num_frames, int64_t frame_elems, ltx_stream stream) {
    if (!step_noise || !latents) LTX_FAIL(LTX_ERR_ARG, "ltx_guidance_step_stochastic_held: latents and step_noise are required");
    if (!hold) LTX_FAIL(LTX_ERR_ARG, "ltx_guidance_step_stochastic_held: hold is required");
    return ltx_launch_guidance_step_held(guidance_args(text, uncond, perturbed, pred_dtype, latents, noise_pred_out, B, n, guidance_scale, guidance_rescale, stg_scale,
                                                       0.0f, sigma, sigma_next, step_noise, stats_ws, hold, num_frames, frame_elems), (hipStream_t)stream);
}
// ... 52 lines not shown
    if (stg_scale < 0.0f) LTX_FAIL(LTX_ERR_ARG, "ltx_guidance_step_ex: negative stg_scale");
    if (pred_dtype != LTX_F32 && pred_dtype != LTX_BF16) LTX_FAIL(LTX_ERR_ARG, "ltx_guidance_step_ex: bad dtype");
    GuidanceExArgs a;
    a.g = guidance_args(text, uncond, perturbed, pred_dtype, latents, noise_pred_out, B, n, guidance_scale, guidance_rescale, stg_scale,
                        dt, sigma, sigma_next, step_noise, nullptr, hold, num_frames, frame_elems);
    a.cfg_star = cfg_star; a.rescale_form = rescale_form; a.ws = ws; a.scalars_out = scalars_out;
    return ltx_launch_guidance_step_ex(a, (hipStream_t)stream);
}

extern "C" int ltx_cond_apply(float* latents, const float* cond_tokens, int cond_frames, const unsigned char* hold,
                              int B, int num_frames, int tokens_per_frame, int channels, ltx_stream stream) {
    if (!hold) LTX_FAIL(LTX_ERR_ARG, "ltx_cond_apply: hold is required");
    if (!latents || !cond_tokens || B < 1 || num_frames < 1 || cond_frames < 1 || tokens_per_frame < 1 || channels < 1)
        LTX_FAIL(LTX_ERR_ARG, "ltx_cond_apply: bad argument");
    bool any = false;
    for (int b = 0; b < B; ++b)
        for (int f = 0; f < num_frames; ++f)
            if (hold[(size_t)b * num_frames + f]) {
                if (f >= cond_frames) LTX_FAIL(LTX_ERR_ARG, "ltx_cond_apply: held frame " + std::to_string(f) + " lies beyond the " + std::to_string(cond_frames) + " conditioning frame(s)");
                any = true;
            }
    if (!any) return LTX_OK;
    hipStream_t s = (hipStream_t)stream;
    const size_t nh = (size_t)B * num_frames;
    unsigned char* hd = nullptr;
    HIP_TRY(hipMalloc((void**)&hd, nh));
    struct Free { void* p; ~Free() { (void)hipFree(p); } } guard{hd};
    HIP_TRY(hipMemcpyAsync(hd, hold, nh, hipMemcpyHostToDevice, s));
    LTX_TRY(ltx_launch_cond_apply(latents, cond_tokens, cond_frames, hd, B, num_frames, (int64_t)tokens_per_frame * channels, s));
    HIP_TRY(hipStreamSynchronize(s));
    return LTX_OK;
}

static thread_local float g_timing[4] = {0, 0, 0, 0};
extern "C" int ltx_pipeline_last_timing(float ms[4]) {
    if (!ms) LTX_FAIL(LTX_ERR_ARG, "null output");
    for (int i = 0; i < 4; ++i) ms[i] = g_timing[i];
    return LTX_OK;
}

static thread_local int t_steps[2] = {0, 0};
extern "C" int ltx_pipeline_last_steps(int* executed, int* requested) {
    if (executed) *executed = t_steps[0];
    if (requested) *requested = t_steps[1];
    return LTX_OK;
}

namespace {
struct PipeCache {
    DevBuf stats, coords, hold, gws;
    DevBuf kf_coords, kf_clean, kf_grid;
    DevBuf g_lat, g_emb, g_mask, g_pred, g_coords;
    int coords_key[6] = {-1, -1, -1, -1, -1, -1};
};
PipeCache& pipe_cache(int device) {
    thread_local std::map<int, PipeCache> caches;
    return caches[device];
}
struct PipeScratch {
    hipEvent_t ev[4] = {nullptr, nullptr, nullptr, nullptr};
    std::vector<hipEvent_t> step_ev;
    int new_event(hipEvent_t* out) {
        hipEvent_t e = nullptr;
        HIP_TRY(hipEventCreate(&e));
        step_ev.push_back(e); *out = e;
        return LTX_OK;
    }
    ~PipeScratch() {
        for (auto e : ev) if (e) (void)hipEventDestroy(e);
        for (auto e : step_ev) (void)hipEventDestroy(e);
    }
};
}

int ltx_pipeline_schedule(const ltx_pipeline_params* p, int S, std::vector<float>* sig, std::vector<int64_t>* ts) {
    const int N = p->num_inference_steps;
    if (N < 1) LTX_FAIL(LTX_ERR_ARG, "num_inference_steps must be >= 1");
    std::vector<float> sig_in(N);
    sig->assign(N + 1, 0.0f); ts->assign(N, 0);
    const bool custom = p->sigmas != nullptr;
    for (int i = 0; i < N; ++i)
        sig_in[i] = custom ? p->sigmas[i] : (N == 1 ? 1.0f : 1.0f + (1.0f / (float)N - 1.0f) * (float)i / (float)(N - 1));
    const float mu = custom ? 0.0f : ltx_calculate_shift(S, 256, 4096, 0.5f, 1.15f);
    return ltx_sched_set_timesteps(sig_in.data(), N, mu, 1, 1.0f, p->shift_terminal, p->use_shift_terminal, sig->data(), ts->data());
}

struct CondRun {
    int G = 0, E = 0;
    std::vector<float> tcap;
    std::vector<unsigned char> hold;
    int hold_rows = 1;
    const float* coords = nullptr;
    std::vector<CondPlaceEntry> place;
    float noise_scale = 0.0f; const float* cond_noise = nullptr;
    std::vector<int> hard;
};

struct LatentGeom { int ts_ratio = 8, sp_ratio = 32, F = 0, H = 0, W = 0; };
static int latent_geom(ltx_vae* vae, const ltx_pipeline_params* p, LatentGeom* g) {
    if (vae) { ltx_vae_config vc; LTX_TRY(ltx_vae_get_config(vae, &vc)); g->ts_ratio = vc.temporal_compression_ratio; g->sp_ratio = vc.spatial_compression_ratio; }
    if (g->ts_ratio >= 1) g->F = (p->num_frames - 1) / g->ts_ratio + 1;
    if (g->sp_ratio >= 1) { g->H = p->height / g->sp_ratio; g->W = p->width / g->sp_ratio; }
    return LTX_OK;
}
static bool any_held(const unsigned char* hold, int B, int F) {
    for (size_t j = 0; j < (size_t)B * (F > 0 ? F : 0); ++j) if (hold[j]) return true;
// ... 13 lines not shown
        LTX_TRY(pc.g_pred.ensure((size_t)3 * B * n * sizeof(float)));
        if (!plan.any_batched) return LTX_OK;
        LTX_TRY(pc.g_lat.ensure((size_t)3 * B * n * sizeof(float))); LTX_TRY(pc.g_emb.ensure(3 * emb_n * sizeof(float)));
        LTX_TRY(pc.g_mask.ensure(3 * mask_n * sizeof(float))); LTX_TRY(pc.g_coords.ensure(3 * coords_n * sizeof(float)));
        const bool present[3] = {plan.any_cfg, true, plan.any_stg};
        for (int k = 0; k < 3; ++k) {
            if (!present[k]) continue;
            HIP_TRY(hipMemcpyAsync(pc.g_emb.as<float>() + (size_t)k * emb_n, src_emb[k], emb_n * sizeof(float), hipMemcpyDeviceToDevice, s));
            HIP_TRY(hipMemcpyAsync(pc.g_mask.as<float>() + (size_t)k * mask_n, src_mask[k], mask_n * sizeof(float), hipMemcpyDeviceToDevice, s));
            HIP_TRY(hipMemcpyAsync(pc.g_coords.as<float>() + (size_t)k * coords_n, coords_dev, coords_n * sizeof(float), hipMemcpyDeviceToDevice, s));
        }
        return LTX_OK;
    }
};

struct PipeStepCache { const ltx_step_cache_params* params; unsigned char* reused_out; float* distance_out; };

static int pipeline_run(ltx_dit* dit, ltx_vae* vae, const ltx_pipeline_params* p, const CondRun* cr, const StepPlan& plan, const PipeIO& io,
                        const PipeStepCache* scd = nullptr) {
    float* const latents = io.latents; const int B = io.B, K = io.K;
    if (!dit || !p || !latents || !io.prompt_embeds || !io.prompt_mask) LTX_FAIL(LTX_ERR_ARG, "ltx_pipeline_call: null argument");
    if (!p->output_latent && (!vae || !io.out_video)) LTX_FAIL(LTX_ERR_ARG, "ltx_pipeline_call: decode requested without vae/out_video");
    if (p->height % 32 != 0 || p->width % 32 != 0) LTX_FAIL(LTX_ERR_ARG, "`height` and `width` must be divisible by 32");
    if (p->num_inference_steps < 1) LTX_FAIL(LTX_ERR_ARG, "num_inference_steps must be >= 1");
    if (plan.any_cfg && (!io.neg_embeds || !io.neg_mask)) LTX_FAIL(LTX_ERR_ARG, "classifier-free guidance needs negative embeddings and mask");
    if (p->stochastic_sampling && !p->step_noise) LTX_FAIL(LTX_ERR_ARG, "stochastic_sampling needs step_noise [steps,B,S*C]");
    hipStream_t s = (hipStream_t)io.stream;
    ltx_dit_config dc; LTX_TRY(ltx_dit_get_config(dit, &dc));
    LatentGeom lg; LTX_TRY(latent_geom(vae, p, &lg));
    const int F = lg.F, H = lg.H, W = lg.W;
    const int G = cr ? cr->G : F, E = cr ? cr->E : 0;
    const int S = G * H * W, C = dc.in_channels, L = dc.num_layers;
    const int64_t n = (int64_t)S * C;
    if (cr && (G != E + F || cr->tcap.size() != (size_t)B * G || cr->hold.size() != (size_t)cr->hold_rows * B * G ||
               (cr->hold_rows != 1 && cr->hold_rows != p->num_inference_steps) || (E > 0 && !cr->coords)))
        LTX_FAIL(LTX_ERR_ARG, "pipeline: inconsistent conditioning description");

    if (plan.set_skip) LTX_TRY(ltx_dit_set_skip_blocks(dit, plan.perm_skip, plan.n_perm_skip));
    const int N = p->num_inference_steps;
    std::vector<float> sig; std::vector<int64_t> ts;
    LTX_TRY(ltx_pipeline_schedule(p, F * H * W, &sig, &ts));

    PipeScratch sc;
    int cur_dev = 0; HIP_TRY(hipGetDevice(&cur_dev));
    PipeCache& pc = pipe_cache(cur_dev);
    const bool classic = plan.mix == STEP_MIX_CLASSIC;
    LTX_TRY(pc.stats.ensure(64 * B));
    if (!classic) LTX_TRY(pc.gws.ensure(ltx_guidance_ex_ws_bytes(B, n)));
    if (cr) {
        LTX_TRY(pc.hold.ensure(cr->hold.size()));
        HIP_TRY(hipMemcpyAsync(pc.hold.p, cr->hold.data(), cr->hold.size(), hipMemcpyHostToDevice, s));
        HIP_TRY(hipStreamSynchronize(s));
    }
    auto upload_coords = [&](DevBuf& buf, const float* row) -> int {
        std::vector<float> all((size_t)B * S * 3);
        for (int b = 0; b < B; ++b) std::memcpy(all.data() + (size_t)b * S * 3, row, sizeof(float) * S * 3);
        LTX_TRY(buf.ensure(all.size() * sizeof(float)));
        HIP_TRY(hipMemcpyAsync(buf.p, all.data(), all.size() * sizeof(float), hipMemcpyHostToDevice, s));
        HIP_TRY(hipStreamSynchronize(s));
        return LTX_OK;
    };
    const int key[6] = {B, F, H, W, p->frame_rate, lg.ts_ratio * 1000 + lg.sp_ratio};
    if (cr && cr->coords) {
        LTX_TRY(upload_coords(pc.kf_coords, cr->coords));
    } else if (std::memcmp(key, pc.coords_key, sizeof(key)) != 0) {
        std::vector<float> vc((size_t)S * 3);
        LTX_TRY(ltx_build_video_coords(F, H, W, p->frame_rate, lg.ts_ratio, lg.sp_ratio, vc.data()));
        LTX_TRY(upload_coords(pc.coords, vc.data()));
        std::memcpy(pc.coords_key, key, sizeof(key));
    }
    const float* coords = (cr && cr->coords ? pc.kf_coords : pc.coords).as<float>();
    BranchBatch bb{pc, B, n, (size_t)B * K * dc.caption_channels, (size_t)B * K, (size_t)B * S * 3,
                   {io.neg_embeds, io.prompt_embeds, io.prompt_embeds}, {io.neg_mask, io.prompt_mask, io.prompt_mask}};
    LTX_TRY(bb.stage(plan, coords, s));
    for (auto& e : sc.ev) HIP_TRY(hipEventCreate(&e));
    HIP_TRY(hipEventRecord(sc.ev[0], s));
    const int64_t group_elems = (int64_t)H * W * C;
    const bool noised = cr && cr->noise_scale > 0.0f && !cr->hard.empty();
    if (cr && !cr->place.empty()) LTX_TRY(ltx_launch_cond_place(latents, cr->place.data(), (int)cr->place.size(), B, G, group_elems, s));
    if (noised) {
        LTX_TRY(pc.kf_clean.ensure((size_t)B * n * sizeof(float)));
        HIP_TRY(hipMemcpyAsync(pc.kf_clean.p, latents, (size_t)B * n * sizeof(float), hipMemcpyDeviceToDevice, s));
    }
    struct CtxScope { ltx_dit* d; ~CtxScope() { (void)ltx_dit_context_cache(d, 0); } } ctx_scope{dit};
    LTX_TRY(ltx_dit_context_cache(dit, 1));
    struct CacheScope { ltx_step_cache* c = nullptr; ~CacheScope() { ltx_step_cache_destroy(c); } } cache;
    if (scd) {
        LTX_TRY(ltx_step_cache_create(dit, 3 * B, &cache.c));
        for (int i = 0; i < N; ++i) { if (scd->reused_out) scd->reused_out[i] = 0; if (scd->distance_out) scd->distance_out[i] = 0.0f; }
    }
    const bool hooked = p->interrupt != nullptr || p->on_step != nullptr;
    bool stopped = false; int steps_run = 0;
    std::vector<float> tframes;
    std::vector<float> slm;
    std::vector<hipEvent_t> done_ev;
    for (int i = 0; i < N; ++i) {
        if (hooked) {
            if (done_ev.size() >= 2) HIP_TRY(hipEventSynchronize(done_ev[done_ev.size() - 2]));
            if (!stopped && p->on_step && p->on_step(p->on_step_user, i, N, ts[i]) != 0) stopped = true;
            if (stopped || (p->interrupt && *p->interrupt)) continue;
        }
        ++steps_run;
        float tvals[8]; for (int b = 0; b < 8; ++b) tvals[b] = (float)ts[i];
        hipEvent_t e0, e1, e2;
        LTX_TRY(sc.new_event(&e0)); LTX_TRY(sc.new_event(&e1)); LTX_TRY(sc.new_event(&e2));
        HIP_TRY(hipEventRecord(e0, s));
        const StepEntry& st = plan.steps[(size_t)i];
        const int frows = st.batched ? st.rows : B;
        if (cr) {
            tframes.resize((size_t)frows * G);
            for (size_t r = 0; r < tframes.size() / ((size_t)B * G); ++r)
                for (size_t j = 0; j < (size_t)B * G; ++j) tframes[r * B * G + j] = std::fmin((float)ts[i], cr->tcap[j]);
        }
        if (noised) {
            const float kn = (float)((double)cr->noise_scale * (double)sig[i] * (double)sig[i]);
            LTX_TRY(ltx_launch_cond_noise(latents, pc.kf_clean.as<float>(), cr->cond_noise + (size_t)i * B * n, cr->hard.data(), (int)cr->hard.size(), B, G, group_elems, kn, s));
        }
        const unsigned char* hold_i = cr ? pc.hold.as<unsigned char>() + (cr->hold_rows > 1 ? (size_t)i * B * G : 0) : nullptr;
        int reuse = 0;
        if (scd) {
            float dist = 0.0f;
            LTX_TRY(ltx_step_cache_decide(cache.c, dit, latents, cr ? tframes.data() : tvals, cr ? G : 0, B, S, cr ? G : F, H, W, LTX_F32, i, N, scd->params, &reuse, &dist, s));
            LTX_TRY(ltx_step_cache_require(cache.c, dit, st.slot0 * B, st.nbr * B, S, &reuse));
            if (scd->reused_out) scd->reused_out[i] = (unsigned char)reuse;
            if (scd->distance_out) scd->distance_out[i] = dist;
        }
        auto forward = [&](const void* x, const void* emb, const float* mk, int rows, const float* vc, const float* skip, void* pred, int slot) -> int {
            if (scd) return ltx_dit_forward_cached(dit, cache.c, slot * B, reuse, cr ? G : 0, x, emb, cr ? tframes.data() : tvals, mk, rows, S, K, cr ? G : F, H, W, nullptr, vc, skip, LTX_F32, pred, s);
            if (cr) return ltx_dit_forward_frames(dit, x, emb, tframes.data(), mk, rows, S, K, G, H, W, nullptr, vc, skip, LTX_F32, pred, s);
            return ltx_dit_forward(dit, x, emb, tvals, mk, rows, S, K, F, H, W, nullptr, vc, skip, LTX_F32, pred, s);
        };
        if (st.stg) step_skip_rows(L, frows, st.batched ? (st.nbr - 1) * B : 0, B, st.guide.skip, st.guide.n_skip, &slm);
        if (st.batched) {
            for (int r = 0; r < st.nbr; ++r) HIP_TRY(hipMemcpyAsync(pc.g_lat.as<float>() + (size_t)r * B * n, latents, (size_t)B * n * sizeof(float), hipMemcpyDeviceToDevice, s));
            LTX_TRY(forward(pc.g_lat.p, bb.emb(st.slot0), bb.mask(st.slot0), st.rows, bb.coords(st.slot0), st.stg ? slm.data() : nullptr, bb.pred(st.slot0), st.slot0));
        } else {
            for (int k = st.slot0; k < st.slot0 + st.nbr; ++k) LTX_TRY(forward(latents, bb.src_emb[k], bb.src_mask[k], B, coords, k == 2 ? slm.data() : nullptr, bb.pred(k), k));
        }
// ... 279 lines not shown
```

candle-video_amd/ltxhip/__init__.py:

```python
from __future__ import annotations

import ctypes as C
import os
from dataclasses import dataclass, field
from typing import Dict, List, Optional, Sequence, Tuple

import torch

_HERE = os.path.dirname(os.path.abspath(__file__))
_LIB_PATH = os.environ.get("LTXHIP_LIB") or os.path.join(os.path.dirname(_HERE), "libltxhip.so")

if not os.path.exists(_LIB_PATH):
    raise ImportError(
        f"ltxhip: {_LIB_PATH} is missing — build it with `make -C candle-video_amd` "
        "(or `python -c 'import __graft_entry__ as g; g.build()'`). There is no CPU fallback.")
lib = C.CDLL(_LIB_PATH)

LTX_F32, LTX_BF16 = 0, 1


class LtxError(RuntimeError):
    pass


# ... 227 lines not shown
UPSAMPLER_SYMBOLS = sorted(_UP_SIGS)
for _name, _sig in _UP_SIGS.items():
    _fn = getattr(lib, _name)
    _fn.argtypes = _sig
    _fn.restype = None if _name in ("ltx_upsampler_config_default", "ltx_upsampler_destroy") else C.c_int
LTX_GN_SILU, LTX_GN_GUARDS = 1, 2


class UpsamplerStConfigC(C.Structure):
    _fields_ = [("in_channels", C.c_int), ("mid_channels", C.c_int), ("num_blocks_per_stage", C.c_int),
                ("spatial_upsample", C.c_int), ("temporal_upsample", C.c_int)]


_UP_ST_SIGS = {
    "ltx_upsampler_st_config_default": [_vp], "ltx_upsampler_create_st": [_vp, _vp, _sz, _i, _i, _vp],
    "ltx_upsampler_create_from_file_st": [_vp, C.c_char_p, _i, _i, _vp], "ltx_upsampler_get_st_config": [_vp, _vp],
    "ltx_upsampler_out_shape": [_vp, _i, _i, _i, _vp, _vp, _vp],
    "ltx_op_conv3d_shuffle": [_vp, _vp, _vp, _i, _vp, _i, _i, _i, _i, _i, _i, _i, _i, _i, _vp],
    "ltx_op_pixel_shuffle_guarded": [_vp, _vp, _i, _i, _i, _i, _i, _i, _vp],
}
UPSAMPLER_ST_SYMBOLS = sorted(_UP_ST_SIGS)
for _name, _sig in _UP_ST_SIGS.items():
    _fn = getattr(lib, _name)
    _fn.argtypes = _sig
    _fn.restype = None if _name == "ltx_upsampler_st_config_default" else C.c_int


_STG_SIGS = {
    "ltx_dit_set_stg_mode": [_vp, _i], "ltx_dit_get_stg_mode": [_vp, C.POINTER(C.c_int)],
    "ltx_stg_mode_from_name": [C.c_char_p, C.POINTER(C.c_int)],
    "ltx_op_stg_fill": [_vp, _i, _vp, _i, _vp, _i, _i, _i, _i, _vp],
}
STG_SYMBOLS = sorted(_STG_SIGS)
for _name, _sig in _STG_SIGS.items():
    _fn = getattr(lib, _name)
    _fn.argtypes = _sig
    _fn.restype = C.c_int
LTX_STG_TRANSFORMER_BLOCK, LTX_STG_ATTENTION_SKIP, LTX_STG_ATTENTION_VALUES = 0, 1, 2
STG_MODES = ("transformer_block", "attention_skip", "attention_values")


def stg_mode_from_name(name: str) -> int:
    out = C.c_int(0)
    _check(lib.ltx_stg_mode_from_name(name.encode() if name is not None else None, C.byref(out)))
    return out.value


class GuidanceScheduleC(C.Structure):
    _fields_ = [("n", C.c_int), ("guidance_scale", C.POINTER(C.c_float)), ("stg_scale", C.POINTER(C.c_float)), ("rescale", C.POINTER(C.c_float)),
                ("skip_blocks", C.POINTER(C.c_int)), ("skip_offsets", C.POINTER(C.c_int)), ("guidance_timesteps", C.POINTER(C.c_float)),
                ("cfg_star", C.c_int), ("rescale_form", C.c_int)]


_GUIDANCE_SIGS = {
    "ltx_guidance_schedule_resolve": [_vp, _vp, _i, _vp],
    "ltx_guidance_ws_bytes": [_i, _i64],
    "ltx_guidance_step_ex": [_vp, _vp, _vp, _i, _vp, _vp, _i, _i64, _f, _f, _f, _i, _i, _f, _f, _f, _vp, _vp, _i, _i64, _vp, _vp, _vp],
    "ltx_pipeline_call_sched": [_vp, _vp, _vp, _vp, _vp, _vp, _vp, _vp, _vp, _vp, _vp, _i, _i, _vp, _vp],
    "ltx_pipeline_call_multiscale_sched": [_vp, _vp, _vp, _vp, _vp, _vp, _vp, _f, _vp, _vp, _vp, _vp, _vp, _vp, _vp, _i, _i, _vp, _vp, _vp],
}
GUIDANCE_SYMBOLS = sorted(_GUIDANCE_SIGS)
for _name, _sig in _GUIDANCE_SIGS.items():
    _fn = getattr(lib, _name)
    _fn.argtypes = _sig
    _fn.restype = C.c_size_t if _name == "ltx_guidance_ws_bytes" else C.c_int
LTX_RESCALE_CFG, LTX_RESCALE_MIX = 0, 1
RESCALE_FORMS = ("cfg", "mix")


class CondItemC(C.Structure):
    _fields_ = [("tokens", C.POINTER(C.c_float)), ("cond_frames", C.c_int), ("frame_index", C.c_int), ("strength", C.c_float)]


class CondGroupC(C.Structure):
    _fields_ = [("item", C.c_int), ("item_frame", C.c_int), ("strength", C.c_float)]


_KEYFRAME_SIGS = {
    "ltx_cond_layout": [_vp, _i, _i, _i, _i, _i, _i, _i, _vp, _vp, _vp, _i, _vp],
    "ltx_cond_place": [_vp, _vp, _i, _vp, _i, _i, _i, _i, _vp],
    "ltx_cond_noise": [_vp, _vp, _vp, _vp, _i, _i, _i, _i, _f, _f, _vp],
    "ltx_cond_step_hold": [_vp, _i, _f, _f, _vp, _vp],
    "ltx_pipeline_call_keyframes": [_vp, _vp, _vp, _vp, _vp, _i, _f, _vp, _vp, _vp, _vp, _vp, _vp, _vp, _i, _i, _vp, _vp],
}
KEYFRAME_SYMBOLS = sorted(_KEYFRAME_SIGS)
for _name, _sig in _KEYFRAME_SIGS.items():
    _fn = getattr(lib, _name)
    _fn.argtypes = _sig
    _fn.restype = C.c_int


class StepCacheParamsC(C.Structure):
    _fields_ = [("rel_l1_thresh", C.c_float), ("coeff", C.c_float * 5), ("pattern", C.POINTER(C.c_ubyte)), ("n_pattern", C.c_int)]


_STEPCACHE_SIGS = {
    "ltx_step_cache_params_default": [_vp], "ltx_step_cache_create": [_vp, _i, _vp], "ltx_step_cache_destroy": [_vp], "ltx_step_cache_reset": [_vp],
    "ltx_step_cache_decide": [_vp, _vp, _vp, _vp, _i, _i, _i, _i, _i, _i, _i, _i, _i, _vp, _vp, _vp, _vp],
    "ltx_step_cache_require": [_vp, _vp, _i, _i, _i, _vp],
    "ltx_dit_forward_cached": [_vp, _vp, _i, _i, _i, _vp, _vp, _vp, _vp, _i, _i, _i, _i, _i, _i, _vp, _vp, _vp, _i, _vp, _vp],
    "ltx_step_cache_read_residual": [_vp, _i, _vp, _vp],
    "ltx_pipeline_call_cached": [_vp, _vp, _vp, _vp, _vp, _vp, _vp, _vp, _vp, _vp, _vp, _vp, _i, _i, _vp, _vp, _vp, _vp],
    "ltx_op_step_measure_ws_bytes": [_i64, _i, _i],
    "ltx_op_step_measure": [_vp, _vp, _vp, _vp, _i, _i64, _i, _i64, _f, _i, _i, _vp, _vp, _vp],
    "ltx_op_step_residual": [_vp, _vp, _i64, _i, _i, _vp],
}
# ... 206 lines not shown
                               "the dtype the call uses (hidden_states' dtype / float32): a temporary copy has no stable identity")
        vc = _dev(video_coords, torch.float32) if video_coords is not None else None
        if getattr(self, "_ctx_cache", False) and vc is not None and vc.data_ptr() != video_coords.data_ptr():
            raise LtxError("context_cache(True) needs video_coords that are already a contiguous float32 device tensor: the RoPE "
                           "tables of the scope are kept per coords POINTER, a temporary copy has no stable identity")
        slm = None
        if skip_layer_mask is not None:
            slm = _floats(skip_layer_mask.detach().float().cpu().flatten().tolist())
        rs = _floats(rope_interpolation_scale) if rope_interpolation_scale is not None else None
        out = torch.empty(B, S, self.config.out_channels, dtype=io, device=h.device)
        _check(lib.ltx_dit_forward(self._h, _ptr(h), _ptr(e), _floats(t), _ptr(m), B, S, K, num_frames, height, width,
                                   rs, _ptr(vc), slm, _dt(io), _ptr(out), _stream()))
        return out


    def forward_frames(self, hidden_states: torch.Tensor, encoder_hidden_states: torch.Tensor, timestep,
                       encoder_attention_mask: Optional[torch.Tensor], num_frames: int, height: int, width: int,
                       rope_interpolation_scale: Optional[Tuple[float, float, float]] = None,
                       video_coords: Optional[torch.Tensor] = None,
                       skip_layer_mask: Optional[torch.Tensor] = None) -> torch.Tensor:
        io = hidden_states.dtype if hidden_states.dtype in (torch.float32, torch.bfloat16) else torch.float32
        h = _dev(hidden_states, io)
        e = _dev(encoder_hidden_states, io)
        if h.dim() != 3 or e.dim() != 3:
            raise LtxError("hidden_states must be [B,S,C] and encoder_hidden_states [B,K,C]")
        B, S, _ = h.shape
        K = e.shape[1]
        t = torch.as_tensor(timestep, dtype=torch.float32).detach().flatten().cpu().tolist()
        if len(t) != B * num_frames:
            raise LtxError(f"timestep must have {B} x {num_frames} entries (batch rows x latent frames)")
        if num_frames * height * width != S:
            raise LtxError("forward_frames: S must equal num_frames*height*width (tokens in pack order, with or without video_coords)")
        m = _dev(encoder_attention_mask, torch.float32) if encoder_attention_mask is not None else None
        vc = _dev(video_coords, torch.float32) if video_coords is not None else None
        if getattr(self, "_ctx_cache", False) and (e.data_ptr() != encoder_hidden_states.data_ptr() or (m is not None and m.data_ptr() != encoder_attention_mask.data_ptr())
                                                   or (vc is not None and vc.data_ptr() != video_coords.data_ptr())):
            raise LtxError("context_cache(True) needs encoder_hidden_states / encoder_attention_mask / video_coords that are already contiguous "
                           "device tensors of the dtype the call uses: a temporary copy has no stable identity")
        slm = _floats(skip_layer_mask.detach().float().cpu().flatten().tolist()) if skip_layer_mask is not None else None
        rs = _floats(rope_interpolation_scale) if rope_interpolation_scale is not None else None
        out = torch.empty(B, S, self.config.out_channels, dtype=io, device=h.device)
        _check(lib.ltx_dit_forward_frames(self._h, _ptr(h), _ptr(e), _floats(t), _ptr(m), B, S, K, num_frames, height, width,
                                          rs, _ptr(vc), slm, _dt(io), _ptr(out), _stream()))
        return out

    def set_stg_mode(self, mode):
        _check(lib.ltx_dit_set_stg_mode(self._h, stg_mode_from_name(mode) if isinstance(mode, str) else int(mode)))

    @property
    def stg_mode(self) -> str:
        out = C.c_int(0)
        _check(lib.ltx_dit_get_stg_mode(self._h, C.byref(out)))
        return STG_MODES[out.value]

    def set_adapters(self, loras: Sequence["LtxLora"] = (), scales: Optional[Sequence[float]] = None):
        loras = list(loras)
        scales = [1.0] * len(loras) if scales is None else [float(v) for v in scales]
        if len(scales) != len(loras):
            raise LtxError(f"set_adapters: {len(loras)} adapters but {len(scales)} scales")
        arr = (C.c_void_p * max(len(loras), 1))(*[l._h for l in loras])
        _check(lib.ltx_dit_set_adapters(self._h, arr, _floats(scales) if scales else None, len(loras), _stream()))
        self._adapters = loras

    def adapter_count(self) -> int:
        return int(lib.ltx_dit_adapter_count(self._h))

    def linear_shape(self, which: int):
        D = self.config.num_attention_heads * self.config.attention_head_dim
        return (4 * D if which == 8 else D, 4 * D if which == 9 else self.config.cross_attention_dim if which in (5, 6) else D)

    def read_linear(self, block: int, which: int, device="cuda") -> torch.Tensor:
        if not 0 <= which < 10:
            raise LtxError("read_linear: which must be 0..9 (LORA_TARGETS)")
        out = torch.empty(self.linear_shape(which), dtype=self.dtype, device=device)
        _check(lib.ltx_dit_read_linear(self._h, block, which, _ptr(out), _stream()))
        return out


def lora_parse_key(key: str):
    buf = C.create_string_buffer(1024)
    role = C.c_int(0)
    _check(lib.ltx_lora_parse_key(key.encode(), buf, C.c_size_t(len(buf)), C.byref(role)))
    return buf.value.decode(), role.value


class LtxLora:

    def __init__(self):
        raise LtxError("use LtxLora.from_file or LtxLora.from_tensors")

    @classmethod
    def from_tensors(cls, model: LtxVideoTransformer3DModel, tensors: Dict[str, torch.Tensor], strict: bool = False) -> "LtxLora":
        self = cls.__new__(cls)
        arr, keep = _make_weights(tensors)
        self._h = C.c_void_p()
        nu = C.c_int(0)
        _check(lib.ltx_lora_create(model._h, arr, C.c_size_t(len(tensors)), int(strict), C.byref(self._h), C.byref(nu)))
        del keep
        self.n_unmatched = nu.value
        return self

    @classmethod
    def from_file(cls, model: LtxVideoTransformer3DModel, path: str, strict: bool = False) -> "LtxLora":
        self = cls.__new__(cls)
        self._h = C.c_void_p()
        nu = C.c_int(0)
# ... 1566 lines not shown
    def rownorm_presum(x, presum, eps=1e-6, weight=None, scale=None, shift=None, rows_per_batch=1, act=0):
        rows, D = x.shape
        y = torch.empty_like(x)
        ms = scale.shape[-1] if scale is not None else 0
        _check(lib.ltx_op_rownorm_presum(_ptr(x.contiguous()), _ptr(y), C.c_int64(rows), D, C.c_float(eps), _ptr(weight), _ptr(scale), _ptr(shift),
                                         C.c_int64(rows_per_batch), ms, act, _ptr(presum), presum.shape[-1], _dt(x.dtype), _stream()))
        return y

    @staticmethod
    def qknorm_rope(x, weight, eps=1e-5, cos=None, sin=None):
        x = x.clone().contiguous()
        rows, D = x.shape
        _check(lib.ltx_op_qknorm_rope(_ptr(x), C.c_int64(rows), D, D, _ptr(weight), C.c_float(eps), _ptr(cos), _ptr(sin),
                                      _dt(x.dtype), _stream()))
        return x

    @staticmethod
    def qknorm_rope_segs(x, rows, D, ld, nseg, seg_stride, w0, w1=None, w0b=None, eps=1e-5, cos=None, sin=None, out_scale0=1.0):
        if not x.is_contiguous():
            raise LtxError("qknorm_rope_segs: the buffer is used as it lies in memory; pass a contiguous tensor")
        _check(lib.ltx_op_qknorm_rope_segs(_ptr(x), C.c_int64(rows), D, ld, nseg, C.c_int64(seg_stride), _ptr(w0), _ptr(w1), _ptr(w0b),
                                           C.c_float(eps), _ptr(cos), _ptr(sin), C.c_float(out_scale0), _dt(x.dtype), _stream()))
        return x

    @staticmethod
    def norm_route(rows, D, dtype=torch.bfloat16, kind=0, scale=False, shift=None, weight=False, act=0, rows_per_batch=1, presum_n=0, nparts=0) -> str:
        buf = C.create_string_buffer(32)
        flags = (1 if scale else 0) | (2 if (scale if shift is None else shift) else 0) | (4 if weight else 0)
        _check(lib.ltx_op_norm_route(C.c_int64(rows), D, _dt(dtype), kind, flags, act, C.c_int64(rows_per_batch), presum_n, nparts, buf, 32))
        return buf.value.decode()

    @staticmethod
    def qknorm_route(rows, D, dtype=torch.bfloat16) -> str:
        buf = C.create_string_buffer(32)
        _check(lib.ltx_op_qknorm_route(C.c_int64(rows), D, _dt(dtype), buf, 32))
        return buf.value.decode()

    @staticmethod
    def timestep_embedding(timesteps, vae_flavour=False, multiplier=1.0, dtype=torch.float32, device="cuda"):
        ts = [float(t) for t in timesteps]
        out = torch.empty(len(ts), 256, dtype=dtype, device=device)
        _check(lib.ltx_op_timestep_embedding(_floats(ts), len(ts), int(bool(vae_flavour)), C.c_float(multiplier), _dt(dtype), _ptr(out), _stream()))
        return out

    @staticmethod
    def rope_table(B, F, H, W, D, coords=None, rope_scale=None, device="cuda"):
        cos = torch.empty(B * F * H * W, D // 2, dtype=torch.float32, device=device)
        sin = torch.empty_like(cos)
        _check(lib.ltx_op_rope_table(_ptr(cos), _ptr(sin), _ptr(coords), B, F, H, W, D,
                                     _floats(rope_scale) if rope_scale is not None else None, _stream()))
        return cos, sin

    @staticmethod
    def attention(q, k, v, heads, scale, key_bias=None):
        B, Sq, D = q.shape
        Sk = k.shape[1]
        o = torch.empty_like(q)
        _check(lib.ltx_op_attention(_ptr(q.contiguous()), _ptr(k.contiguous()), _ptr(v.contiguous()), _ptr(o), B, Sq, Sk, heads, D // heads,
                                    D, D, D, D, C.c_float(scale), _ptr(key_bias), _dt(q.dtype), _stream()))
        return o

    @staticmethod
    def attention_prescaled(q, k, v, heads):
        B, Sq, D = q.shape
        def rows(t):
            return t if t.stride(2) == 1 and t.stride(0) == t.shape[1] * t.stride(1) and t.stride(1) % 8 == 0 else t.contiguous()
        q, k, v = rows(q), rows(k), rows(v)
        o = torch.empty(B, Sq, D, dtype=q.dtype, device=q.device)
        _check(lib.ltx_op_attention_prescaled(_ptr(q), _ptr(k), _ptr(v), _ptr(o), B, Sq, k.shape[1],
                                              heads, D // heads, q.stride(1), k.stride(1), v.stride(1), D, _stream()))
        return o

    @staticmethod
    def conv3d(x_cl, w, bias, causal=False, resid=None):
        B, T, H, W, Cin = x_cl.shape
        Cout = w.shape[0]
        y = torch.empty(B, T, H, W, Cout, dtype=x_cl.dtype, device=x_cl.device)
        _check(lib.ltx_op_conv3d(_ptr(x_cl.contiguous()), _ptr(w.contiguous()), _ptr(bias.to(w.dtype).contiguous()), _dt(w.dtype), _ptr(y), _ptr(resid),
                                 B, T, H, W, Cin, Cout, int(causal), _dt(x_cl.dtype), _stream()))
        return y

    @staticmethod
    def conv3d_norm(x_cl, w, bias, causal=False, eps=1e-6, act=1, scale=None, shift=None):
        B, T, H, W, Cin = x_cl.shape
        Cout = w.shape[0]
        if (scale is None) != (shift is None):
            raise LtxError("conv3d_norm: scale and shift come together")
        ms = 0
        if scale is not None:
            for t in (scale, shift):
                if t.dtype != torch.float32 or tuple(t.shape) != (B, Cout) or t.stride(1) != 1:
                    raise LtxError(f"conv3d_norm: scale / shift must be f32 [{B}, {Cout}] with dense rows")
            ms = scale.stride(0) if B > 1 else max(scale.stride(0), Cout)
            if B > 1 and shift.stride(0) != ms:
                raise LtxError("conv3d_norm: scale and shift must share one row stride")
        y = torch.empty(B, T, H, W, Cout, dtype=x_cl.dtype, device=x_cl.device)
        _check(lib.ltx_op_conv3d_norm(_ptr(x_cl.contiguous()), _ptr(w.contiguous()), _ptr(bias.to(w.dtype).contiguous()), _dt(w.dtype), _ptr(y),
                                      _ptr(scale), _ptr(shift), ms, C.c_float(eps), act, B, T, H, W, Cin, Cout, int(causal), _dt(x_cl.dtype), _stream()))
        return y

    @staticmethod
    def upsample3d(x_cl, w, bias, causal=False, residual=True):
        B, T, H, W, Cin = x_cl.shape
        Cout = w.shape[0]
        y = torch.empty(B, 2 * T - 1, 2 * H, 2 * W, Cout // 8, dtype=x_cl.dtype, device=x_cl.device)
        _check(lib.ltx_op_upsample3d(_ptr(x_cl.contiguous()), _ptr(w.contiguous()), _ptr(bias.to(w.dtype).contiguous()), _dt(w.dtype), _ptr(y),
# ... 109 lines not shown
```

rust/ltxhip-sys/src/lib.rs:

```rust
#![allow(non_camel_case_types)]

use core::ffi::{c_char, c_float, c_int, c_void};
use core::mem::{align_of, size_of};

pub const LTX_F32: c_int = 0;
pub const LTX_BF16: c_int = 1;

#[repr(C)]
pub struct ltx_weight {
    pub name: *const c_char,
    pub data: *const c_void,
    pub dtype: c_int,
    pub ndim: c_int,
    pub shape: [i64; 5],
    pub on_device: c_int,
}

#[repr(C)]
#[derive(Clone, Copy, Debug)]
pub struct ltx_dit_config {
    pub in_channels: c_int,
    pub out_channels: c_int,
    pub patch_size: c_int,
    pub patch_size_t: c_int,
// ... 283 lines not shown
    pub fn ltx_latent_renoise(tokens: *mut c_float, noise: *const c_float, sigma: c_float, n: usize, stream: ltx_stream) -> c_int;
    pub fn ltx_pipeline_first_sigma(p: *const ltx_pipeline_params, s: c_int, sigma0: *mut c_float) -> c_int;
    pub fn ltx_upsampler_warmup(up: *mut ltx_upsampler, b: c_int, f: c_int, h: c_int, w: c_int, stream: ltx_stream) -> c_int;
    pub fn ltx_pipeline_call_multiscale(dit: *mut ltx_dit, vae: *mut ltx_vae, up: *mut ltx_upsampler, p_first: *const ltx_pipeline_params,
                                        p_second: *const ltx_pipeline_params, adain_factor: c_float, latents_lo: *mut c_float, noise_hi: *const c_float,
                                        prompt_embeds: *const c_float, prompt_mask: *const c_float, neg_embeds: *const c_float, neg_mask: *const c_float,
                                        decode_noise: *const c_float, b: c_int, k: c_int, latents_hi_out: *mut c_float, out_video: *mut c_float,
                                        stream: ltx_stream) -> c_int;
    pub fn ltx_pipeline_multiscale_last_timing(ms: *mut c_float) -> c_int;
    pub fn ltx_op_groupnorm(x: *const c_void, y: *mut c_void, resid: *const c_void, weight: *const c_void, bias: *const c_void, b: c_int, f: c_int, h: c_int,
                            w: c_int, c: c_int, groups: c_int, eps: c_float, flags: c_int, dtype: c_int, stream: ltx_stream) -> c_int;
}


#[repr(C)]
#[derive(Clone, Copy, Debug)]
pub struct ltx_upsampler_st_config {
    pub in_channels: c_int,
    pub mid_channels: c_int,
    pub num_blocks_per_stage: c_int,
    pub spatial_upsample: c_int,
    pub temporal_upsample: c_int,
}

pub const UPSAMPLER_ST_LAYOUT_LTX_UPSAMPLER_ST_CONFIG: (usize, usize) = (20, 4);
const _: () = assert!(size_of::<ltx_upsampler_st_config>() == UPSAMPLER_ST_LAYOUT_LTX_UPSAMPLER_ST_CONFIG.0 && align_of::<ltx_upsampler_st_config>() == UPSAMPLER_ST_LAYOUT_LTX_UPSAMPLER_ST_CONFIG.1);

extern "C" {
    pub fn ltx_upsampler_st_config_default(cfg: *mut ltx_upsampler_st_config);
    pub fn ltx_upsampler_create_st(cfg: *const ltx_upsampler_st_config, weights: *const ltx_weight, n_weights: usize, model_dtype: c_int, device: c_int,
                                   out: *mut *mut ltx_upsampler) -> c_int;
    pub fn ltx_upsampler_create_from_file_st(cfg: *const ltx_upsampler_st_config, path: *const c_char, model_dtype: c_int, device: c_int,
                                             out: *mut *mut ltx_upsampler) -> c_int;
    pub fn ltx_upsampler_get_st_config(up: *const ltx_upsampler, out: *mut ltx_upsampler_st_config) -> c_int;
    pub fn ltx_upsampler_out_shape(up: *const ltx_upsampler, f: c_int, h: c_int, w: c_int, fo: *mut c_int, ho: *mut c_int, wo: *mut c_int) -> c_int;
    pub fn ltx_op_conv3d_shuffle(x: *const c_void, w: *const c_void, bias: *const c_void, wdtype: c_int, y: *mut c_void, b: c_int, f: c_int, h: c_int,
                                 wd: c_int, cin: c_int, o: c_int, st: c_int, ss: c_int, dtype: c_int, stream: ltx_stream) -> c_int;
    pub fn ltx_op_pixel_shuffle_guarded(x: *const c_void, y: *mut c_void, b: c_int, f: c_int, h: c_int, w: c_int, c: c_int, dtype: c_int, stream: ltx_stream) -> c_int;
}


pub const LTX_STG_TRANSFORMER_BLOCK: c_int = 0;
pub const LTX_STG_ATTENTION_SKIP: c_int = 1;
pub const LTX_STG_ATTENTION_VALUES: c_int = 2;

extern "C" {
    pub fn ltx_dit_set_stg_mode(m: *mut ltx_dit, mode: c_int) -> c_int;
    pub fn ltx_dit_get_stg_mode(m: *const ltx_dit, out: *mut c_int) -> c_int;
    pub fn ltx_stg_mode_from_name(name: *const c_char, out: *mut c_int) -> c_int;
    pub fn ltx_op_stg_fill(dst: *mut c_void, ldd: c_int, src: *const c_void, lds: c_int, rows: *const u8, b: c_int, s: c_int, d: c_int, dtype: c_int,
                           stream: ltx_stream) -> c_int;
}


pub const LTX_RESCALE_CFG: c_int = 0;
pub const LTX_RESCALE_MIX: c_int = 1;

#[repr(C)]
#[derive(Clone, Copy, Debug)]
pub struct ltx_guidance_schedule {
    pub n: c_int,
    pub guidance_scale: *const c_float,
    pub stg_scale: *const c_float,
    pub rescale: *const c_float,
    pub skip_blocks: *const c_int,
    pub skip_offsets: *const c_int,
    pub guidance_timesteps: *const c_float,
    pub cfg_star: c_int,
    pub rescale_form: c_int,
}

pub const GUIDANCE_LAYOUT_LTX_GUIDANCE_SCHEDULE: (usize, usize) = (64, 8);
const _: () = assert!(size_of::<ltx_guidance_schedule>() == GUIDANCE_LAYOUT_LTX_GUIDANCE_SCHEDULE.0 && align_of::<ltx_guidance_schedule>() == GUIDANCE_LAYOUT_LTX_GUIDANCE_SCHEDULE.1);

extern "C" {
    pub fn ltx_guidance_schedule_resolve(sched: *const ltx_guidance_schedule, sigmas: *const c_float, n_steps: c_int, entry_of_step: *mut c_int) -> c_int;
    pub fn ltx_guidance_ws_bytes(b: c_int, n: i64) -> usize;
    pub fn ltx_guidance_step_ex(text: *const c_void, uncond: *const c_void, perturbed: *const c_void, pred_dtype: c_int, latents: *mut c_float,
                                noise_pred_out: *mut c_float, b: c_int, n: i64, guidance_scale: c_float, guidance_rescale: c_float, stg_scale: c_float,
                                cfg_star: c_int, rescale_form: c_int, dt: c_float, sigma: c_float, sigma_next: c_float, step_noise: *const c_float,
                                hold: *const u8, num_frames: c_int, frame_elems: i64, ws: *mut c_void, scalars_out: *mut c_float, stream: ltx_stream) -> c_int;
    pub fn ltx_pipeline_call_sched(dit: *mut ltx_dit, vae: *mut ltx_vae, p: *const ltx_pipeline_params, sched: *const ltx_guidance_schedule,
                                   cond: *const ltx_conditioning, latents: *mut c_float, prompt_embeds: *const c_float, prompt_mask: *const c_float,
                                   neg_embeds: *const c_float, neg_mask: *const c_float, decode_noise: *const c_float, b: c_int, k: c_int,
                                   out_video: *mut c_float, stream: ltx_stream) -> c_int;
    pub fn ltx_pipeline_call_multiscale_sched(dit: *mut ltx_dit, vae: *mut ltx_vae, up: *mut ltx_upsampler, p_first: *const ltx_pipeline_params,
                                              p_second: *const ltx_pipeline_params, sched_first: *const ltx_guidance_schedule,
                                              sched_second: *const ltx_guidance_schedule, adain_factor: c_float, latents_lo: *mut c_float,
                                              noise_hi: *const c_float, prompt_embeds: *const c_float, prompt_mask: *const c_float, neg_embeds: *const c_float,
                                              neg_mask: *const c_float, decode_noise: *const c_float, b: c_int, k: c_int, latents_hi_out: *mut c_float,
                                              out_video: *mut c_float, stream: ltx_stream) -> c_int;
}


#[repr(C)]
#[derive(Clone, Copy, Debug)]
pub struct ltx_cond_item {
    pub tokens: *const c_float,
    pub cond_frames: c_int,
    pub frame_index: c_int,
    pub strength: c_float,
}

#[repr(C)]
#[derive(Clone, Copy, Debug)]
pub struct ltx_cond_group {
// ... 71 lines not shown
```

Measured before the change: 531.4 frames/sec.

## Factor RoPE tables into per-frame and per-pixel parts for raster coordinates

```diff
diff --git a/candle-video_amd/csrc/capi_ops.hip b/candle-video_amd/csrc/capi_ops.hip
--- a/candle-video_amd/csrc/capi_ops.hip
+++ b/candle-video_amd/csrc/capi_ops.hip
@@ -3,6 +3,9 @@
 #include "../../include/ltxhip_upsampler_st.h"
 #include "../../include/ltxhip_stg.h"
 #include "../../include/ltxhip_stepcache.h"
+#include "../../include/ltxhip_rope.h"
+#include "../host/rope_raster.h"
+#include "options.h"
 
 static inline int dtc(int d) { return d == 1 ? LTX_DT_BF16 : LTX_DT_F32; }
 
@@ -207,9 +210,7 @@
     return LTX_OK;
 }
 
-extern "C" int ltx_op_rope_table(float* cos, float* sin, const float* coords, int B, int F, int H, int W, int D,
-                                 const float* rope_scale_host, ltx_stream stream) {
-    if (!cos || !sin) LTX_FAIL(LTX_ERR_ARG, "ltx_op_rope_table: null tensor");
+static int rope_freqs_dev(int D, float** out) {
     int steps = D / 6; if (steps < 1) steps = 1;
     std::vector<float> fr(steps);
     const float theta_ln = (float)std::log(10000.0);
@@ -217,20 +218,80 @@
         float lin = steps <= 1 ? 0.0f : (float)i * (float)(1.0 / (double)(steps - 1));
         fr[i] = (float)std::exp((double)(lin * theta_ln)) * (float)(M_PI / 2.0);
     }
-    float* dfr = nullptr;
-    HIP_TRY(hipMalloc((void**)&dfr, sizeof(float) * steps));
-    HIP_TRY(hipMemcpy(dfr, fr.data(), sizeof(float) * steps, hipMemcpyHostToDevice));
-    RopeTableArgs r; r.cos = cos; r.sin = sin; r.freqs = dfr; r.B = B; r.D = D;
-    if (coords) { r.use_coords = 1; r.coords = coords; r.F = 1; r.H = 1; r.W = F * H * W;
+    HIP_TRY(hipMalloc((void**)out, sizeof(float) * steps));
+    if (hipMemcpy(*out, fr.data(), sizeof(float) * steps, hipMemcpyHostToDevice) != hipSuccess) { (void)hipFree(*out); *out = nullptr; LTX_FAIL(LTX_ERR_HIP, "rope: upload of the frequencies"); }
+    return LTX_OK;
+}
+static void rope_table_source(RopeTableArgs& r, const float* coords, int F, int H, int W, bool factored, const float* rope_scale_host) {
+    if (coords) { r.use_coords = 1; r.coords = coords; r.F = factored ? F : 1; r.H = factored ? H : 1; r.W = factored ? W : F * H * W;
                   r.gscale[0] = (float)(1.0 / 20.0); r.gscale[1] = (float)(1.0 / 2048.0); r.gscale[2] = (float)(1.0 / 2048.0); }
     else { r.F = F; r.H = H; r.W = W;
            if (rope_scale_host) { r.gscale[0] = (float)((double)rope_scale_host[0] / 20.0); r.gscale[1] = (float)((double)rope_scale_host[1] / 2048.0); r.gscale[2] = (float)((double)rope_scale_host[2] / 2048.0); } }
-    int rc = ltx_launch_rope_table(r, (hipStream_t)stream);
-    hipError_t e = hipStreamSynchronize((hipStream_t)stream);
+}
+static int rope_table_run(RopeTableArgs& r, int D, hipStream_t s) {
+    float* dfr = nullptr;
+    LTX_TRY(rope_freqs_dev(D, &dfr));
+    r.freqs = dfr; r.D = D;
+    int rc = ltx_launch_rope_table(r, s);
+    hipError_t e = hipStreamSynchronize(s);
     (void)hipFree(dfr);
     if (rc != LTX_OK) return rc;
     if (e != hipSuccess) { ltx_set_error(hipGetErrorString(e)); return LTX_ERR_HIP; }
     return LTX_OK;
+}
+
+extern "C" int ltx_op_rope_table(float* cos, float* sin, const float* coords, int B, int F, int H, int W, int D,
+                                 const float* rope_scale_host, ltx_stream stream) {
+    if (!cos || !sin) LTX_FAIL(LTX_ERR_ARG, "ltx_op_rope_table: null tensor");
+    RopeTableArgs r; r.cos = cos; r.sin = sin; r.B = B;
+    rope_table_source(r, coords, F, H, W, false, rope_scale_host);
+    return rope_table_run(r, D, (hipStream_t)stream);
+}
+
+extern "C" int ltx_rope_coords_raster(const float* coords_host, int B, int F, int H, int W, int* raster) {
+    if (!coords_host || !raster || B < 1 || F < 1 || H < 1 || W < 1) LTX_FAIL(LTX_ERR_ARG, "ltx_rope_coords_raster: bad argument");
+    *raster = rope_coords_raster(coords_host, B, F, H, W) ? 1 : 0;
+    return LTX_OK;
+}
+
+extern "C" int ltx_op_rope_table_factored(float* cos_t, float* sin_t, float* cos_hw, float* sin_hw, const float* coords, int F, int H, int W, int D,
+                                          const float* rope_scale_host, ltx_stream stream) {
+    if (!cos_t || !sin_t || !cos_hw || !sin_hw) LTX_FAIL(LTX_ERR_ARG, "ltx_op_rope_table_factored: null tensor");
+    if (F < 1 || H < 1 || W < 1) LTX_FAIL(LTX_ERR_ARG, "ltx_op_rope_table_factored: empty raster");
+    RopeTableArgs r; r.cos_t = cos_t; r.sin_t = sin_t; r.cos_hw = cos_hw; r.sin_hw = sin_hw;
+    rope_table_source(r, coords, F, H, W, true, rope_scale_host);
+    return rope_table_run(r, D, (hipStream_t)stream);
+}
+
+extern "C" int ltx_op_qknorm_rope_grid(void* x, int B, int F, int H, int W, int D, int ld, int nseg, int64_t seg_stride, const void* w0, const void* w1, const void* w0b,
+                                       float eps, const float* coords, const float* coords_host, const float* rope_scale_host, float out_scale0, int dtype,
+                                       char* route, int cap, ltx_stream stream) {
+    if (!x || !w0) LTX_FAIL(LTX_ERR_ARG, "ltx_op_qknorm_rope_grid: null tensor");
+    if (B < 1 || F < 1 || H < 1 || W < 1 || D < 6 || D % 2 != 0 || seg_stride < 0 || (route && cap < 1)) LTX_FAIL(LTX_ERR_ARG, "ltx_op_qknorm_rope_grid: bad argument");
+    const int64_t S = (int64_t)F * H * W, rows = (int64_t)B * S;
+    const int half = D / 2;
+    const bool fact = ltx_opt().rope_factored && (!coords || (coords_host && rope_coords_raster(coords_host, B, F, H, W)));
+    const char* why = nullptr;
+    const QkNormRoute rt = ltx_qknorm_route(dtc(dtype), rows, D, &why);
+    if (route) snprintf(route, (size_t)cap, "%s", ltx_qknorm_form_name(rt, fact));
+    const size_t n = (fact ? (size_t)F + (size_t)H * W : (size_t)rows) * half;
+    float* tab = nullptr;
+    HIP_TRY(hipMalloc((void**)&tab, 2 * n * sizeof(float)));
+    RopeTableArgs r; r.B = B;
+    QkNormRopeArgs a; a.x = x; a.rows = rows; a.D = D; a.ld = ld; a.nseg = nseg; a.seg_stride = seg_stride; a.w0 = w0; a.w1 = w1; a.w0b = w0b;
+    a.eps = eps; a.out_scale0 = out_scale0;
+    if (fact) {
+        r.cos_t = tab; r.cos_hw = tab + (size_t)F * half; r.sin_t = tab + n; r.sin_hw = tab + n + (size_t)F * half;
+        a.cos_t = r.cos_t; a.sin_t = r.sin_t; a.cos_hw = r.cos_hw; a.sin_hw = r.sin_hw; a.hw = H * W; a.S = S;
+    } else {
+        r.cos = tab; r.sin = tab + n; a.cos = r.cos; a.sin = r.sin;
+    }
+    rope_table_source(r, coords, F, H, W, fact, rope_scale_host);
+    int rc = rope_table_run(r, D, (hipStream_t)stream);
+    if (rc == LTX_OK) rc = ltx_launch_qknorm_rope(a, dtc(dtype), (hipStream_t)stream);
+    if (rc == LTX_OK && hipStreamSynchronize((hipStream_t)stream) != hipSuccess) { ltx_set_error("ltx_op_qknorm_rope_grid: the launch failed"); rc = LTX_ERR_HIP; }
+    (void)hipFree(tab);
+    return rc;
 }
 
 extern "C" int ltx_op_attention(const void* q, const void* k, const void* v, void* o, int B, int Sq, int Sk, int heads, int hd,
diff --git a/candle-video_amd/csrc/dit.hip b/candle-video_amd/csrc/dit.hip
--- a/candle-video_amd/csrc/dit.hip
+++ b/candle-video_amd/csrc/dit.hip
@@ -62,7 +62,8 @@
     std::deque<DitWfold> wcache;
     std::deque<DitGroupEntry> gcache;
     bool wfold_off = false;
-    struct { bool valid = false; const float* coords = nullptr; float rs[3] = {0, 0, 0}; bool has_rs = false; int B = 0, S = 0, F = 0, H = 0, W = 0; hipStream_t stream = nullptr; } rope_key;
+    struct { bool valid = false; const float* coords = nullptr; float rs[3] = {0, 0, 0}; bool has_rs = false; int B = 0, S = 0, F = 0, H = 0, W = 0; hipStream_t stream = nullptr; bool fact = false; } rope_key;
+    struct { bool raster = false; int F = 0, H = 0, W = 0; } rope_hint;
     uint64_t weights_epoch = 0;
     void invalidate_weight_derived() {
         ++weights_epoch;
@@ -545,18 +546,32 @@
     *out = ctx;
     return LTX_OK;
 }
+bool rope_factored_form(const ltx_dit* m, const DitPlan& p, int num_frames, int height, int width, const float* video_coords) {
+    if (!ltx_opt().rope_factored || num_frames < 1 || height < 1 || width < 1 || (int64_t)num_frames * height * width != p.S) return false;
+    const auto& h = m->rope_hint;
+    return !video_coords || (h.raster && h.F == num_frames && h.H == height && h.W == width);
+}
+size_t rope_table_bytes(const DitPlan& p, bool fact, int num_frames, int height, int width) {
+    return (fact ? (size_t)num_frames + (size_t)height * width : (size_t)p.M) * (p.D / 2) * sizeof(float);
+}
 int rope_tables(ltx_dit* m, const DitPlan& p, int num_frames, int height, int width, const float* rope_scale, const float* video_coords, hipStream_t s) {
     const ltx_dit_config& c = m->cfg;
     auto& rk = m->rope_key;
-    const bool same = m->ctx_mode && rk.valid && rk.coords == video_coords && rk.B == p.B && rk.S == p.S && rk.F == num_frames && rk.H == height && rk.W == width &&
+    const bool fact = rope_factored_form(m, p, num_frames, height, width, video_coords);
+    const bool same = m->ctx_mode && rk.valid && rk.coords == video_coords && rk.B == p.B && rk.S == p.S && rk.F == num_frames && rk.H == height && rk.W == width && rk.fact == fact &&
                       rk.stream == s && rk.has_rs == (rope_scale != nullptr) && (!rope_scale || !memcmp(rk.rs, rope_scale, sizeof(rk.rs)));
     if (same) return LTX_OK;
     rk.valid = false;
     RopeTableArgs r;
     r.cos = m->cosb.as<float>(); r.sin = m->sinb.as<float>(); r.freqs = m->rope_freqs;
     r.B = p.B; r.D = p.D;
+    if (fact) {
+        r.cos_t = r.cos; r.sin_t = r.sin; r.cos_hw = r.cos + (size_t)num_frames * (p.D / 2); r.sin_hw = r.sin + (size_t)num_frames * (p.D / 2);
+        r.cos = r.sin = nullptr;
+    }
     if (video_coords) {
         r.use_coords = 1; r.coords = video_coords; r.F = 1; r.H = 1; r.W = p.S;
+        if (fact) { r.F = num_frames; r.H = height; r.W = width; }
         r.gscale[0] = (float)(1.0 / 20.0); r.gscale[1] = (float)(1.0 / 2048.0); r.gscale[2] = (float)(1.0 / 2048.0);
     } else {
         r.F = num_frames; r.H = height; r.W = width;
@@ -569,8 +584,16 @@
     LTX_TRY(ltx_launch_rope_table(r, s));
     rk.coords = video_coords; rk.B = p.B; rk.S = p.S; rk.F = num_frames; rk.H = height; rk.W = width; rk.stream = s;
     rk.has_rs = rope_scale != nullptr; if (rope_scale) memcpy(rk.rs, rope_scale, sizeof(rk.rs));
+    rk.fact = fact;
     rk.valid = m->ctx_mode;
     return LTX_OK;
+}
+void rope_table_args(const ltx_dit* m, const DitPlan& p, QkNormRopeArgs* q) {
+    const auto& rk = m->rope_key;
+    const float* co = m->cosb.as<float>(); const float* si = m->sinb.as<float>();
+    if (!rk.fact) { q->cos = co; q->sin = si; return; }
+    const size_t nt = (size_t)rk.F * (p.D / 2);
+    q->cos_t = co; q->sin_t = si; q->cos_hw = co + nt; q->sin_hw = si + nt; q->hw = rk.H * rk.W; q->S = p.S;
 }
 
 struct DitCarry {
@@ -633,7 +656,7 @@
     LTX_TRY(ltx_launch_gemm(gemm_qkv1(p, fold1 ? fold_in_form : kPass, b, x), dt, EPI_BIAS, s));
     const float attn_scale = 1.0f / std::sqrt((float)hd);
     QkNormRopeArgs qa; qa.x = m->qkv.p; qa.rows = M; qa.D = D; qa.ld = p.ldqkv; qa.seg_stride = p.seg; qa.nseg = 2; qa.w0 = b.nq1; qa.w1 = b.nk1;
-    qa.eps = 1e-5f; qa.cos = m->cosb.as<float>(); qa.sin = m->sinb.as<float>();
+    qa.eps = 1e-5f; rope_table_args(m, p, &qa);
     if (p.fold_q) qa.out_scale0 = attn_scale * 1.4426950408889634f;
     LTX_TRY(ltx_launch_qknorm_rope(qa, dt, s));
     AttnArgs at; at.q = m->qkv.p; at.k = (char*)m->qkv.p + (size_t)p.seg * esz; at.v = (char*)m->qkv.p + (size_t)2 * p.seg * esz; at.o = m->attn.p;
@@ -739,7 +762,8 @@
     const int dt = p.dt, D = p.D, L = c.num_layers;
     const int64_t M = p.M, MK = p.MK; const size_t esz = ltx_dt_size(dt);
     const size_t nte = p.NB == p.B ? (size_t)p.B : 8;
-    const size_t MD = M * D * esz, KD = MK * D * esz, part = M * (D / 128) * sizeof(float), rope = M * (D / 2) * sizeof(float);
+    const size_t MD = M * D * esz, KD = MK * D * esz, part = M * (D / 128) * sizeof(float);
+    const size_t rope = rope_table_bytes(p, rope_factored_form(m, p, num_frames, height, width, video_coords), num_frames, height, width);
     const std::pair<DevBuf*, size_t> ws[] = {
         {&m->xin, M * c.in_channels * esz}, {&m->encin, MK * c.caption_channels * esz}, {&m->h, MD}, {&m->n, MD}, {&m->qkv, 3 * MD}, {&m->attn, MD}, {&m->ff, 4 * MD},
         {&m->c1, KD}, {&m->encp, KD}, {&m->kv2, 2 * KD}, {&m->tproj, nte * 256 * esz}, {&m->e1, nte * D * esz}, {&m->emb, nte * D * esz}, {&m->embs, nte * D * esz},
@@ -852,6 +876,15 @@
     if (num_frames < 1 || height < 1 || width < 1 || (int64_t)num_frames * height * width != S)
         LTX_FAIL(LTX_ERR_ARG, "ltx_dit_forward_frames: S must equal num_frames*height*width (tokens in pack order, with or without video_coords)");
     return dit_forward_chunks(m, hidden, enc, timestep, num_frames, enc_mask, B, S, K, num_frames, height, width, rope_scale, video_coords, skip_layer_mask, io_dtype, out, stream);
+}
+
+void ltx_dit_rope_raster_hint(ltx_dit* m, int raster, int F, int H, int W) {
+    m->rope_hint.raster = raster != 0; m->rope_hint.F = F; m->rope_hint.H = H; m->rope_hint.W = W;
+}
+extern "C" int ltx_dit_rope_form(const ltx_dit* m, int* factored) {
+    if (!m || !factored) LTX_FAIL(LTX_ERR_ARG, "ltx_dit_rope_form: null argument");
+    *factored = m->rope_key.fact ? 1 : 0;
+    return LTX_OK;
 }
 
 extern "C" int ltx_dit_context_cache(ltx_dit* m, int enable) {
diff --git a/candle-video_amd/csrc/kernels.h b/candle-video_amd/csrc/kernels.h
--- a/candle-video_amd/csrc/kernels.h
+++ b/candle-video_amd/csrc/kernels.h
@@ -148,11 +148,16 @@
     float eps = 1e-5f;
     const float* cos = nullptr; const float* sin = nullptr;
     float out_scale0 = 1.f;
+    const float* cos_t = nullptr; const float* sin_t = nullptr;
+    const float* cos_hw = nullptr; const float* sin_hw = nullptr;
+    int hw = 0; int64_t S = 0;
+    bool factored() const { return cos_t != nullptr; }
 };
 int ltx_launch_qknorm_rope(const QkNormRopeArgs& a, int dtype, hipStream_t s);
 enum QkNormRoute { QKNORM_REFUSED = 0, QKNORM_BLOCK, QKNORM_FUSED4, QKNORM_FUSED8, QKNORM_CACHED, QKNORM_REREAD };
 QkNormRoute ltx_qknorm_route(int dtype, int64_t rows, int D, const char** why);
 const char* ltx_qknorm_route_name(QkNormRoute r);
+const char* ltx_qknorm_form_name(QkNormRoute r, bool factored);
 
 struct RopeTableArgs {
     float* cos = nullptr; float* sin = nullptr;
@@ -161,6 +166,7 @@
     int B = 1, F = 1, H = 1, W = 1, D = 0;
     int use_coords = 0;
     float gscale[3] = {1.f, 1.f, 1.f};
+    float* cos_t = nullptr; float* sin_t = nullptr; float* cos_hw = nullptr; float* sin_hw = nullptr;
 };
 int ltx_launch_rope_table(const RopeTableArgs& a, hipStream_t s);
 
diff --git a/candle-video_amd/csrc/model_util.h b/candle-video_amd/csrc/model_util.h
--- a/candle-video_amd/csrc/model_util.h
+++ b/candle-video_amd/csrc/model_util.h
@@ -85,5 +85,6 @@
 DitPlan ltx_dit_plan(const ltx_dit_config& c, int dt, int iodt, int B, int S, int K, int G, bool skip_mask);
 
 int ltx_step_cache_params_check(const ltx_step_cache_params* params, const char* who);
+void ltx_dit_rope_raster_hint(ltx_dit* m, int raster, int F, int H, int W);
 
 int ltx_pipeline_schedule(const ltx_pipeline_params* p, int S, std::vector<float>* sig, std::vector<int64_t>* ts);
diff --git a/candle-video_amd/csrc/options.cpp b/candle-video_amd/csrc/options.cpp
--- a/candle-video_amd/csrc/options.cpp
+++ b/candle-video_amd/csrc/options.cpp
@@ -37,7 +37,7 @@
 struct IntField { const char* name; int LtxOptions::*field; };
 const IntField kInts[] = {
     {"gemm_tune", &LtxOptions::gemm_tune}, {"gemm_wide_epi", &LtxOptions::gemm_wide_epi}, {"gemm_trace", &LtxOptions::gemm_trace},
-    {"attn_q64_big", &LtxOptions::attn_q64_big}, {"vae_tile_batch", &LtxOptions::vae_tile_batch}, {"prof_kernel_events", &LtxOptions::prof_kernel_events}, {"ff2_defer", &LtxOptions::ff2_defer},
+    {"attn_q64_big", &LtxOptions::attn_q64_big}, {"vae_tile_batch", &LtxOptions::vae_tile_batch}, {"prof_kernel_events", &LtxOptions::prof_kernel_events}, {"ff2_defer", &LtxOptions::ff2_defer}, {"rope_factored", &LtxOptions::rope_factored},
     {"gemm_splitk", &LtxOptions::gemm_splitk}, {"q2_fold", &LtxOptions::q2_fold}, {"norm_presum", &LtxOptions::norm_presum}, {"norm_lean", &LtxOptions::norm_lean},
     {"xattn_compact", &LtxOptions::xattn_compact}, {"xattn_fold_vo", &LtxOptions::xattn_fold_vo}, {"dense_qkv", &LtxOptions::dense_qkv}, {"vae_fuse_norm", &LtxOptions::vae_fuse_norm}, {"t5_attn_mfma", &LtxOptions::t5_attn_mfma}, {"guidance_batch", &LtxOptions::guidance_batch}, {"norm_fold", &LtxOptions::norm_fold}, {"norm_fold_copies", &LtxOptions::norm_fold_copies}, {"attn_q64_stream", &LtxOptions::attn_q64_stream},
 };
diff --git a/candle-video_amd/csrc/options.h b/candle-video_amd/csrc/options.h
--- a/candle-video_amd/csrc/options.h
+++ b/candle-video_amd/csrc/options.h
@@ -13,6 +13,7 @@
     int vae_tile_batch = 0;
     int prof_kernel_events = 1;
     int ff2_defer = 1;
+    int rope_factored = 1;
     int gemm_splitk = 1;
     int q2_fold = 1;
     int norm_presum = 1;
diff --git a/candle-video_amd/csrc/qknorm_rope.hip b/candle-video_amd/csrc/qknorm_rope.hip
--- a/candle-video_amd/csrc/qknorm_rope.hip
+++ b/candle-video_amd/csrc/qknorm_rope.hip
@@ -31,7 +31,29 @@
     if (active) *reinterpret_cast<u32x4*>(x + c * CH) = o.u;
 }
 
-template <typename T, bool CACHED>
+struct RopeRows { const float* c = nullptr; const float* s = nullptr; const float* c2 = nullptr; const float* s2 = nullptr; };
+template <bool FACT>
+__device__ __forceinline__ RopeRows rope_rows(const QkNormRopeArgs& a, int64_t rr, bool uniform) {
+    RopeRows t;
+    const int half = a.D / 2;
+    if constexpr (FACT) {
+        uint32_t r = (uint32_t)rr;
+        if (uniform) r = (uint32_t)__builtin_amdgcn_readfirstlane((int)r);
+        const uint32_t s = r % (uint32_t)a.S, f = s / (uint32_t)a.hw, j = s - f * (uint32_t)a.hw;
+        t.c = a.cos_t + (size_t)f * half; t.s = a.sin_t + (size_t)f * half;
+        t.c2 = a.cos_hw + (size_t)j * half; t.s2 = a.sin_hw + (size_t)j * half;
+    } else if (a.cos) {
+        t.c = a.cos + rr * half; t.s = a.sin + rr * half;
+    }
+    return t;
+}
+template <bool FACT>
+__device__ __forceinline__ void rope_load(const RopeRows& t, int c4, Chunk16& co, Chunk16& si) {
+    co.u = *reinterpret_cast<const u32x4*>(t.c + c4 * 4); si.u = *reinterpret_cast<const u32x4*>(t.s + c4 * 4);
+    if constexpr (FACT) { co.u |= *reinterpret_cast<const u32x4*>(t.c2 + c4 * 4); si.u |= *reinterpret_cast<const u32x4*>(t.s2 + c4 * 4); }
+}
+
+template <typename T, bool CACHED, bool FACT>
 __global__ __launch_bounds__(256) void qknorm_rope_kernel(const QkNormRopeArgs a, int lpr) {
     constexpr int CH = ElemTraits<T>::CHUNK;
     const int lane = threadIdx.x & 63, wave = threadIdx.x >> 6;
@@ -41,8 +63,8 @@
     const bool active = row < a.rows;
     const int64_t rr = active ? row : a.rows - 1;
     const int nch = a.D / CH;
-    const float* cs = a.cos ? a.cos + rr * (a.D / 2) : nullptr;
-    const float* sn = a.sin ? a.sin + rr * (a.D / 2) : nullptr;
+    const RopeRows tab = rope_rows<FACT>(a, rr, lpr == 64);
+    const float* cs = tab.c; const float* sn = tab.s;
     auto finish = [&](Chunk16 v, int c, float rinv, const T* w, const T* wb, T* x) {
         float f[CH]; chunk_to_f32<T>(v, f);
         Chunk16 wc; wc.u = *reinterpret_cast<const u32x4*>(w + c * CH);
@@ -58,12 +80,22 @@
         if (cs) {
             float co[CH / 2], si[CH / 2];
             if constexpr (CH == 8) {
-                f32x4 c4 = *reinterpret_cast<const f32x4*>(cs + c * 4), s4 = *reinterpret_cast<const f32x4*>(sn + c * 4);
-#pragma unroll
-                for (int p = 0; p < 4; ++p) { co[p] = c4[p]; si[p] = s4[p]; }
+                if constexpr (FACT) {
+                    Chunk16 c4, s4; rope_load<true>(tab, c, c4, s4);
+#pragma unroll
+                    for (int p = 0; p < 4; ++p) { co[p] = c4.f[p]; si[p] = s4.f[p]; }
+                } else {
+                    f32x4 c4 = *reinterpret_cast<const f32x4*>(cs + c * 4), s4 = *reinterpret_cast<const f32x4*>(sn + c * 4);
+#pragma unroll
+                    for (int p = 0; p < 4; ++p) { co[p] = c4[p]; si[p] = s4[p]; }
+                }
             } else {
 #pragma unroll
-                for (int p = 0; p < CH / 2; ++p) { co[p] = cs[c * (CH / 2) + p]; si[p] = sn[c * (CH / 2) + p]; }
+                for (int p = 0; p < CH / 2; ++p) {
+                    const int e = c * (CH / 2) + p;
+                    if constexpr (FACT) { co[p] = __uint_as_float(__float_as_uint(cs[e]) | __float_as_uint(tab.c2[e])); si[p] = __uint_as_float(__float_as_uint(sn[e]) | __float_as_uint(tab.s2[e])); }
+                    else { co[p] = cs[e]; si[p] = sn[e]; }
+                }
             }
 #pragma unroll
             for (int p = 0; p < CH / 2; ++p) {
@@ -100,7 +132,7 @@
     }
 }
 
-template <typename T, int NS, int OCC = 5>
+template <typename T, int NS, int OCC, bool FACT>
 __global__ __launch_bounds__(256, OCC) void qknorm_rope_fused_kernel(const QkNormRopeArgs a, int lpr) {
     constexpr int CH = ElemTraits<T>::CHUNK;
     static_assert(CH == 8, "bf16 rows only");
@@ -111,21 +143,47 @@
     const bool active = row < a.rows;
     const int64_t rr = active ? row : a.rows - 1;
     const int nch = a.D / CH;
-    const bool rope = a.cos != nullptr;
-    const float* cs = rope ? a.cos + rr * (a.D / 2) : nullptr;
-    const float* sn = rope ? a.sin + rr * (a.D / 2) : nullptr;
+    const bool rope = (FACT ? a.cos_t : a.cos) != nullptr;
+    const RopeRows tab = rope_rows<FACT>(a, rr, lpr == 64);
     T* x0 = reinterpret_cast<T*>(a.x) + rr * a.ld;
     const int64_t sst = a.seg_stride ? a.seg_stride : a.D;
     Chunk16 v[2][NS];
     Chunk16 co[NS], si[NS];
-#pragma unroll
-    for (int i = 0; i < NS; ++i) {
-        const int c = sub + i * lpr;
-        const bool in = c < nch;
-        v[0][i].u = (u32x4){0u, 0u, 0u, 0u}; v[1][i].u = (u32x4){0u, 0u, 0u, 0u};
-        if (in) v[0][i].u = *reinterpret_cast<const u32x4*>(x0 + c * CH);
-        if (in && a.nseg == 2) v[1][i].u = *reinterpret_cast<const u32x4*>(x0 + sst + c * CH);
-        if (in && rope) { co[i].u = *reinterpret_cast<const u32x4*>(cs + c * 4); si[i].u = *reinterpret_cast<const u32x4*>(sn + c * 4); }
+    if constexpr (FACT) {
+        Chunk16 ch[NS], sh[NS];
+#pragma unroll
+        for (int i = 0; i < NS; ++i) {
+            const int cc = sub + i * lpr < nch ? sub + i * lpr : 0;
+            co[i].u = *reinterpret_cast<const u32x4*>(tab.c + cc * 4); ch[i].u = *reinterpret_cast<const u32x4*>(tab.c2 + cc * 4);
+            si[i].u = *reinterpret_cast<const u32x4*>(tab.s + cc * 4); sh[i].u = *reinterpret_cast<const u32x4*>(tab.s2 + cc * 4);
+        }
+        const int64_t s1 = a.nseg == 2 ? sst : 0;
+#pragma unroll
+        for (int i = 0; i < NS; ++i) {
+            const int cc = sub + i * lpr < nch ? sub + i * lpr : 0;
+            __builtin_amdgcn_sched_barrier(0);
+            co[i].u |= ch[i].u; si[i].u |= sh[i].u;
+            asm volatile("" : "+v"(co[i].u), "+v"(si[i].u));
+            v[0][i].u = *reinterpret_cast<const u32x4*>(x0 + cc * CH);
+            v[1][i].u = *reinterpret_cast<const u32x4*>(x0 + s1 + cc * CH);
+        }
+        __builtin_amdgcn_sched_barrier(0);
+#pragma unroll
+        for (int i = 0; i < NS; ++i) {
+            const bool in = sub + i * lpr < nch;
+            if (!in) v[0][i].u = (u32x4){0u, 0u, 0u, 0u};
+            if (!in || a.nseg != 2) v[1][i].u = (u32x4){0u, 0u, 0u, 0u};
+        }
+    } else {
+#pragma unroll
+        for (int i = 0; i < NS; ++i) {
+            const int c = sub + i * lpr;
+            const bool in = c < nch;
+            v[0][i].u = (u32x4){0u, 0u, 0u, 0u}; v[1][i].u = (u32x4){0u, 0u, 0u, 0u};
+            if (in) v[0][i].u = *reinterpret_cast<const u32x4*>(x0 + c * CH);
+            if (in && a.nseg == 2) v[1][i].u = *reinterpret_cast<const u32x4*>(x0 + sst + c * CH);
+            if (in && rope) { co[i].u = *reinterpret_cast<const u32x4*>(tab.c + c * 4); si[i].u = *reinterpret_cast<const u32x4*>(tab.s + c * 4); }
+        }
     }
     float rinv[2] = {0.f, 0.f};
 #pragma unroll
@@ -149,7 +207,7 @@
     }
 }
 
-template <typename T>
+template <typename T, bool FACT>
 __global__ __launch_bounds__(256) void qknorm_rope_block_kernel(const QkNormRopeArgs a) {
     constexpr int CH = ElemTraits<T>::CHUNK, NC = 2;
     static_assert(CH == 8, "bf16 rows only");
@@ -157,9 +215,8 @@
     const int tid = threadIdx.x, lane = tid & 63, wave = tid >> 6;
     const int64_t row = blockIdx.x;
     const int nch = a.D / CH;
-    const bool rope = a.cos != nullptr;
-    const float* cs = rope ? a.cos + row * (a.D / 2) : nullptr;
-    const float* sn = rope ? a.sin + row * (a.D / 2) : nullptr;
+    const bool rope = (FACT ? a.cos_t : a.cos) != nullptr;
+    const RopeRows tab = rope_rows<FACT>(a, row, true);
     T* x0 = reinterpret_cast<T*>(a.x) + row * a.ld;
     const int64_t sst = a.seg_stride ? a.seg_stride : a.D;
     Chunk16 v[2][NC];
@@ -171,7 +228,7 @@
         v[0][i].u = (u32x4){0u, 0u, 0u, 0u}; v[1][i].u = (u32x4){0u, 0u, 0u, 0u};
         if (in) v[0][i].u = *reinterpret_cast<const u32x4*>(x0 + c * CH);
         if (in && a.nseg == 2) v[1][i].u = *reinterpret_cast<const u32x4*>(x0 + sst + c * CH);
-        if (in && rope) { co[i].u = *reinterpret_cast<const u32x4*>(cs + c * 4); si[i].u = *reinterpret_cast<const u32x4*>(sn + c * 4); }
+        if (in && rope) rope_load<FACT>(tab, c, co[i], si[i]);
     }
     float ss[2] = {cached_sq<T>(v[0]), cached_sq<T>(v[1])};
     block_sum<2>(ss, red, lane, wave);
@@ -190,32 +247,50 @@
     }
 }
 
+__device__ __forceinline__ int rope_pair(const RopeTableArgs& a, int64_t S, int64_t row, int p, float* co, float* si) {
+    const int rem_pairs = (a.D % 6) / 2;
+    *co = 1.0f; *si = 0.0f;
+    if (p < rem_pairs) return -1;
+    const int fi = p - rem_pairs;
+    const int step = fi / 3, ax = fi - step * 3;
+    float g;
+    if (a.use_coords) {
+        g = a.coords[row * 3 + ax] * a.gscale[ax];
+    } else {
+        const int64_t s = row % S;
+        const int w = (int)(s % a.W); const int64_t t1 = s / a.W;
+        const int h = (int)(t1 % a.H); const int f = (int)(t1 / a.H);
+        const float idx = ax == 0 ? (float)f : (ax == 1 ? (float)h : (float)w);
+        g = idx * a.gscale[ax];
+    }
+    const float ang = a.freqs[step] * (g * 2.0f - 1.0f);
+    *co = cosf(ang); *si = sinf(ang);
+    return ax;
+}
+
 __global__ void rope_table_kernel(const RopeTableArgs a) {
     const int half = a.D / 2;
     const int64_t S = (int64_t)a.F * a.H * a.W;
     const int64_t total = (int64_t)a.B * S * half;
-    const int rem_pairs = (a.D % 6) / 2;
     for (int64_t i = (int64_t)blockIdx.x * blockDim.x + threadIdx.x; i < total; i += (int64_t)gridDim.x * blockDim.x) {
-        const int p = (int)(i % half);
-        const int64_t row = i / half;
-        float co = 1.0f, si = 0.0f;
-        if (p >= rem_pairs) {
-            const int fi = p - rem_pairs;
-            const int step = fi / 3, ax = fi - step * 3;
-            float g;
-            if (a.use_coords) {
-                g = a.coords[row * 3 + ax] * a.gscale[ax];
-            } else {
-                const int64_t s = row % S;
-                const int w = (int)(s % a.W); const int64_t t1 = s / a.W;
-                const int h = (int)(t1 % a.H); const int f = (int)(t1 / a.H);
-                const float idx = ax == 0 ? (float)f : (ax == 1 ? (float)h : (float)w);
-                g = idx * a.gscale[ax];
-            }
-            const float ang = a.freqs[step] * (g * 2.0f - 1.0f);
-            co = cosf(ang); si = sinf(ang);
-        }
+        float co, si;
+        rope_pair(a, S, i / half, (int)(i % half), &co, &si);
         a.cos[i] = co; a.sin[i] = si;
+    }
+}
+
+__global__ void rope_table_factored_kernel(const RopeTableArgs a) {
+    const int half = a.D / 2;
+    const int64_t hw = (int64_t)a.H * a.W, S = (int64_t)a.F * hw;
+    const int64_t nt = (int64_t)a.F * half, total = nt + hw * half;
+    for (int64_t i = (int64_t)blockIdx.x * blockDim.x + threadIdx.x; i < total; i += (int64_t)gridDim.x * blockDim.x) {
+        const bool is_t = i < nt;
+        const int64_t e = is_t ? i : i - nt;
+        const int64_t r = e / half;
+        float co, si;
+        const int ax = rope_pair(a, S, is_t ? r * hw : r, (int)(e % half), &co, &si);
+        if (is_t ? ax > 0 : ax <= 0) { co = 0.0f; si = 0.0f; }
+        (is_t ? a.cos_t : a.cos_hw)[e] = co; (is_t ? a.sin_t : a.sin_hw)[e] = si;
     }
 }
 
@@ -238,41 +313,58 @@
     static const char* const names[] = {"refused", "block", "fused4", "fused8", "cached", "reread"};
     return names[r];
 }
+const char* ltx_qknorm_form_name(QkNormRoute r, bool factored) {
+    static const char* const names[] = {"refused", "block+factored", "fused4+factored", "fused8+factored", "cached+factored", "reread+factored"};
+    return factored ? names[r] : ltx_qknorm_route_name(r);
+}
+
+namespace {
+template <bool FACT>
+void launch_qknorm(QkNormRoute route, const QkNormRopeArgs& a, bool bf16, dim3 grid, int lpr, hipStream_t s) {
+    const dim3 block(256);
+    switch (route) {
+    case QKNORM_BLOCK: hipLaunchKernelGGL((qknorm_rope_block_kernel<bf16_t, FACT>), dim3((unsigned)a.rows), block, 0, s, a); break;
+    case QKNORM_FUSED4: hipLaunchKernelGGL((qknorm_rope_fused_kernel<bf16_t, 4, 5, FACT>), grid, block, 0, s, a, lpr); break;
+    case QKNORM_FUSED8: hipLaunchKernelGGL((qknorm_rope_fused_kernel<bf16_t, 8, 2, FACT>), grid, block, 0, s, a, lpr); break;
+    case QKNORM_CACHED:
+        if (bf16) hipLaunchKernelGGL((qknorm_rope_kernel<bf16_t, true, FACT>), grid, block, 0, s, a, lpr);
+        else hipLaunchKernelGGL((qknorm_rope_kernel<float, true, FACT>), grid, block, 0, s, a, lpr);
+        break;
+    default:
+        if (bf16) hipLaunchKernelGGL((qknorm_rope_kernel<bf16_t, false, FACT>), grid, block, 0, s, a, lpr);
+        else hipLaunchKernelGGL((qknorm_rope_kernel<float, false, FACT>), grid, block, 0, s, a, lpr);
+        break;
+    }
+}
+}
 
 int ltx_launch_qknorm_rope(const QkNormRopeArgs& a, int dtype, hipStream_t s) {
     const int ch = dtype == LTX_DT_BF16 ? 8 : 4;
     if (a.rows <= 0) return LTX_OK;
     if (a.D % ch != 0 || a.ld % ch != 0) LTX_FAIL(LTX_ERR_ARG, "qknorm: D/ld must be multiples of the 16-byte chunk");
     if (a.nseg < 1 || a.nseg > 2 || !a.w0 || (a.nseg == 2 && !a.w1)) LTX_FAIL(LTX_ERR_ARG, "qknorm: bad segments/weights");
+    if (a.factored() && (!a.sin_t || !a.cos_hw || !a.sin_hw || a.hw < 1 || a.S < a.hw || a.S % a.hw != 0 || a.S > INT32_MAX || a.rows > INT32_MAX))
+        LTX_FAIL(LTX_ERR_ARG, "qknorm: the factored tables come as four, with hw rows per frame that divide the S rows of a batch row");
     const char* why = nullptr;
     const QkNormRoute route = ltx_qknorm_route(dtype, a.rows, a.D, &why);
     if (route == QKNORM_REFUSED) LTX_FAIL(LTX_ERR_ARG, why);
     const int nch = a.D / ch, lpr = pick_lpr(nch);
     const int64_t rows_per_block = 4 * (64 / lpr);
-    dim3 grid((unsigned)cdiv64(a.rows, rows_per_block)), block(256);
-    const bool bf16 = dtype == LTX_DT_BF16;
-    switch (route) {
-    case QKNORM_BLOCK: hipLaunchKernelGGL((qknorm_rope_block_kernel<bf16_t>), dim3((unsigned)a.rows), block, 0, s, a); break;
-    case QKNORM_FUSED4: hipLaunchKernelGGL((qknorm_rope_fused_kernel<bf16_t, 4>), grid, block, 0, s, a, lpr); break;
-    case QKNORM_FUSED8: hipLaunchKernelGGL((qknorm_rope_fused_kernel<bf16_t, 8, 2>), grid, block, 0, s, a, lpr); break;
-    case QKNORM_CACHED:
-        if (bf16) hipLaunchKernelGGL((qknorm_rope_kernel<bf16_t, true>), grid, block, 0, s, a, lpr);
-        else hipLaunchKernelGGL((qknorm_rope_kernel<float, true>), grid, block, 0, s, a, lpr);
-        break;
-    default:
-        if (bf16) hipLaunchKernelGGL((qknorm_rope_kernel<bf16_t, false>), grid, block, 0, s, a, lpr);
-        else hipLaunchKernelGGL((qknorm_rope_kernel<float, false>), grid, block, 0, s, a, lpr);
-        break;
-    }
+    const dim3 grid((unsigned)cdiv64(a.rows, rows_per_block));
+    if (a.factored()) launch_qknorm<true>(route, a, dtype == LTX_DT_BF16, grid, lpr, s);
+    else launch_qknorm<false>(route, a, dtype == LTX_DT_BF16, grid, lpr, s);
     LTX_CHECK_LAUNCH();
     return LTX_OK;
 }
 
 int ltx_launch_rope_table(const RopeTableArgs& a, hipStream_t s) {
     if (a.D % 2 != 0 || a.D < 6) LTX_FAIL(LTX_ERR_ARG, "rope: dim must be even and >= 6");
-    const int64_t total = (int64_t)a.B * a.F * a.H * a.W * (a.D / 2);
+    const bool fact = a.cos_t != nullptr;
+    if (fact && (!a.sin_t || !a.cos_hw || !a.sin_hw || a.F < 1 || a.H < 1 || a.W < 1)) LTX_FAIL(LTX_ERR_ARG, "rope: the factored form takes four tables and the raster's extents");
+    const int64_t total = fact ? ((int64_t)a.F + (int64_t)a.H * a.W) * (a.D / 2) : (int64_t)a.B * a.F * a.H * a.W * (a.D / 2);
     int64_t blocks = cdiv64(total, 256); if (blocks > 8192) blocks = 8192;
-    hipLaunchKernelGGL(rope_table_kernel, dim3((unsigned)blocks), dim3(256), 0, s, a);
+    if (fact) hipLaunchKernelGGL(rope_table_factored_kernel, dim3((unsigned)blocks), dim3(256), 0, s, a);
+    else hipLaunchKernelGGL(rope_table_kernel, dim3((unsigned)blocks), dim3(256), 0, s, a);
     LTX_CHECK_LAUNCH();
     return LTX_OK;
 }
diff --git a/candle-video_amd/host/pipeline.hip b/candle-video_amd/host/pipeline.hip
--- a/candle-video_amd/host/pipeline.hip
+++ b/candle-video_amd/host/pipeline.hip
@@ -10,6 +10,7 @@
 #include "../../include/ltxhip_stepcache.h"
 #include "cond_plan.h"
 #include "step_plan.h"
+#include "rope_raster.h"
 
 extern "C" float ltx_calculate_shift(int seq_len, int base_seq_len, int max_seq_len, float base_shift, float max_shift) {
     float m = (max_shift - base_shift) / (float)(max_seq_len - base_seq_len);
@@ -184,15 +185,7 @@
 
 extern "C" int ltx_build_video_coords(int F, int H, int W, int frame_rate, int ts_ratio, int sp_ratio, float* out) {
     if (!out || F < 1 || H < 1 || W < 1 || frame_rate < 1) LTX_FAIL(LTX_ERR_ARG, "ltx_build_video_coords: bad argument");
-    const float inv_fr = (float)(1.0 / (double)frame_rate);
-    size_t i = 0;
-    for (int f = 0; f < F; ++f)
-        for (int h = 0; h < H; ++h)
-            for (int w = 0; w < W; ++w) {
-                float vf = (float)f * (float)ts_ratio + (1.0f - (float)ts_ratio);
-                vf = std::fmin(std::fmax(vf, 0.0f), 1000.0f) * inv_fr;
-                out[i++] = vf; out[i++] = (float)h * (float)sp_ratio; out[i++] = (float)w * (float)sp_ratio;
-            }
+    video_coords_fill(F, H, W, frame_rate, ts_ratio, sp_ratio, out);
     return LTX_OK;
 }
 
@@ -351,6 +344,7 @@
     DevBuf kf_coords, kf_clean, kf_grid;
     DevBuf g_lat, g_emb, g_mask, g_pred, g_coords;
     int coords_key[6] = {-1, -1, -1, -1, -1, -1};
+    bool coords_raster = false;
 };
 PipeCache& pipe_cache(int device) {
     thread_local std::map<int, PipeCache> caches;
@@ -470,9 +464,10 @@
         HIP_TRY(hipMemcpyAsync(pc.hold.p, cr->hold.data(), cr->hold.size(), hipMemcpyHostToDevice, s));
         HIP_TRY(hipStreamSynchronize(s));
     }
-    auto upload_coords = [&](DevBuf& buf, const float* row) -> int {
+    auto upload_coords = [&](DevBuf& buf, const float* row, bool* raster) -> int {
         std::vector<float> all((size_t)B * S * 3);
         for (int b = 0; b < B; ++b) std::memcpy(all.data() + (size_t)b * S * 3, row, sizeof(float) * S * 3);
+        if (raster) *raster = rope_coords_raster(all.data(), B, G, H, W);
         LTX_TRY(buf.ensure(all.size() * sizeof(float)));
         HIP_TRY(hipMemcpyAsync(buf.p, all.data(), all.size() * sizeof(float), hipMemcpyHostToDevice, s));
         HIP_TRY(hipStreamSynchronize(s));
@@ -480,11 +475,12 @@
     };
     const int key[6] = {B, F, H, W, p->frame_rate, lg.ts_ratio * 1000 + lg.sp_ratio};
     if (cr && cr->coords) {
-        LTX_TRY(upload_coords(pc.kf_coords, cr->coords));
+        LTX_TRY(upload_coords(pc.kf_coords, cr->coords, nullptr));
     } else if (std::memcmp(key, pc.coords_key, sizeof(key)) != 0) {
         std::vector<float> vc((size_t)S * 3);
         LTX_TRY(ltx_build_video_coords(F, H, W, p->frame_rate, lg.ts_ratio, lg.sp_ratio, vc.data()));
-        LTX_TRY(upload_coords(pc.coords, vc.data()));
+        pc.coords_key[0] = -1; pc.coords_raster = false;
+        LTX_TRY(upload_coords(pc.coords, vc.data(), &pc.coords_raster));
         std::memcpy(pc.coords_key, key, sizeof(key));
     }
     const float* coords = (cr && cr->coords ? pc.kf_coords : pc.coords).as<float>();
@@ -500,8 +496,9 @@
         LTX_TRY(pc.kf_clean.ensure((size_t)B * n * sizeof(float)));
         HIP_TRY(hipMemcpyAsync(pc.kf_clean.p, latents, (size_t)B * n * sizeof(float), hipMemcpyDeviceToDevice, s));
     }
-    struct CtxScope { ltx_dit* d; ~CtxScope() { (void)ltx_dit_context_cache(d, 0); } } ctx_scope{dit};
+    struct CtxScope { ltx_dit* d; ~CtxScope() { ltx_dit_rope_raster_hint(d, 0, 0, 0, 0); (void)ltx_dit_context_cache(d, 0); } } ctx_scope{dit};
     LTX_TRY(ltx_dit_context_cache(dit, 1));
+    if (!(cr && cr->coords)) ltx_dit_rope_raster_hint(dit, pc.coords_raster ? 1 : 0, F, H, W);
     struct CacheScope { ltx_step_cache* c = nullptr; ~CacheScope() { ltx_step_cache_destroy(c); } } cache;
     if (scd) {
         LTX_TRY(ltx_step_cache_create(dit, 3 * B, &cache.c));
diff --git a/candle-video_amd/host/rope_raster.h b/candle-video_amd/host/rope_raster.h
--- /dev/null
+++ b/candle-video_amd/host/rope_raster.h
@@ -0,0 +1,36 @@
+#pragma once
+#include <cmath>
+#include <cstddef>
+#include <cstdint>
+#include <cstring>
+
+inline void video_coords_fill(int F, int H, int W, int frame_rate, int ts_ratio, int sp_ratio, float* out) {
+    const float inv_fr = (float)(1.0 / (double)frame_rate);
+    size_t i = 0;
+    for (int f = 0; f < F; ++f)
+        for (int h = 0; h < H; ++h)
+            for (int w = 0; w < W; ++w) {
+                float vf = (float)f * (float)ts_ratio + (1.0f - (float)ts_ratio);
+                vf = std::fmin(std::fmax(vf, 0.0f), 1000.0f) * inv_fr;
+                out[i++] = vf; out[i++] = (float)h * (float)sp_ratio; out[i++] = (float)w * (float)sp_ratio;
+            }
+}
+
+inline bool rope_coords_raster(const float* coords, int B, int F, int H, int W) {
+    if (!coords || B < 1 || F < 1 || H < 1 || W < 1) return false;
+    const size_t hw = (size_t)H * (size_t)W, S = (size_t)F * hw;
+    auto bits = [&](size_t row, int ax) { uint32_t u; std::memcpy(&u, coords + row * 3 + ax, sizeof(u)); return u; };
+    for (int f = 0; f < F; ++f) {
+        const uint32_t tv = bits((size_t)f * hw, 0);
+        for (int h = 0; h < H; ++h) {
+            const uint32_t hv = bits((size_t)h * W, 1);
+            for (int w = 0; w < W; ++w) {
+                const size_t row = ((size_t)f * H + h) * W + w;
+                if (bits(row, 0) != tv || bits(row, 1) != hv || bits(row, 2) != bits((size_t)w, 2)) return false;
+            }
+        }
+    }
+    for (int b = 1; b < B; ++b)
+        if (std::memcmp(coords + (size_t)b * S * 3, coords, S * 3 * sizeof(float)) != 0) return false;
+    return true;
+}
diff --git a/candle-video_amd/ltxhip/__init__.py b/candle-video_amd/ltxhip/__init__.py
--- a/candle-video_amd/ltxhip/__init__.py
+++ b/candle-video_amd/ltxhip/__init__.py
@@ -303,6 +303,26 @@
                 ("cfg_star", C.c_int), ("rescale_form", C.c_int)]
 
 
+_ROPE_SIGS = {
+    "ltx_rope_coords_raster": [_vp, _i, _i, _i, _i, C.POINTER(C.c_int)],
+    "ltx_op_rope_table_factored": [_vp, _vp, _vp, _vp, _vp, _i, _i, _i, _i, _vp, _vp],
+    "ltx_op_qknorm_rope_grid": [_vp, _i, _i, _i, _i, _i, _i, _i, _i64, _vp, _vp, _vp, _f, _vp, _vp, _vp, _f, _i, C.c_char_p, _i, _vp],
+    "ltx_dit_rope_form": [_vp, C.POINTER(C.c_int)],
+}
+ROPE_SYMBOLS = sorted(_ROPE_SIGS)
+for _name, _sig in _ROPE_SIGS.items():
+    _fn = getattr(lib, _name)
+    _fn.argtypes = _sig
+    _fn.restype = C.c_int
+
+
+def rope_coords_raster(coords: torch.Tensor, F: int, H: int, W: int) -> bool:
+    c = coords.detach().to("cpu", torch.float32).contiguous()
+    out = C.c_int(0)
+    _check(lib.ltx_rope_coords_raster(_ptr(c), c.shape[0], F, H, W, C.byref(out)))
+    return bool(out.value)
+
+
 _GUIDANCE_SIGS = {
     "ltx_guidance_schedule_resolve": [_vp, _vp, _i, _vp],
     "ltx_guidance_ws_bytes": [_i, _i64],
@@ -615,6 +635,12 @@
         out = C.c_int(0)
         _check(lib.ltx_dit_get_stg_mode(self._h, C.byref(out)))
         return STG_MODES[out.value]
+
+    @property
+    def rope_factored(self) -> bool:
+        out = C.c_int(0)
+        _check(lib.ltx_dit_rope_form(self._h, C.byref(out)))
+        return bool(out.value)
 
     def set_adapters(self, loras: Sequence["LtxLora"] = (), scales: Optional[Sequence[float]] = None):
         loras = list(loras)
@@ -2287,6 +2313,25 @@
         return cos, sin
 
     @staticmethod
+    def rope_table_factored(F, H, W, D, coords=None, rope_scale=None, device="cuda"):
+        ct = torch.empty(F, D // 2, dtype=torch.float32, device=device); st = torch.empty_like(ct)
+        ch = torch.empty(H * W, D // 2, dtype=torch.float32, device=device); sh = torch.empty_like(ch)
+        _check(lib.ltx_op_rope_table_factored(_ptr(ct), _ptr(st), _ptr(ch), _ptr(sh), _ptr(coords), F, H, W, D,
+                                              _floats(rope_scale) if rope_scale is not None else None, _stream()))
+        return ct, st, ch, sh
+
+    @staticmethod
+    def qknorm_rope_grid(x, B, F, H, W, D, ld, nseg, seg_stride, w0, w1=None, w0b=None, eps=1e-5, coords=None, coords_known=True, rope_scale=None, out_scale0=1.0):
+        if not x.is_contiguous():
+            raise LtxError("qknorm_rope_grid: the buffer is used as it lies in memory; pass a contiguous tensor")
+        host = coords.detach().to("cpu", torch.float32).contiguous() if coords is not None and coords_known else None
+        buf = C.create_string_buffer(32)
+        _check(lib.ltx_op_qknorm_rope_grid(_ptr(x), B, F, H, W, D, ld, nseg, C.c_int64(seg_stride), _ptr(w0), _ptr(w1), _ptr(w0b), C.c_float(eps),
+                                           _ptr(coords), _ptr(host), _floats(rope_scale) if rope_scale is not None else None, C.c_float(out_scale0),
+                                           _dt(x.dtype), buf, 32, _stream()))
+        return x, buf.value.decode()
+
+    @staticmethod
     def attention(q, k, v, heads, scale, key_bias=None):
         B, Sq, D = q.shape
         Sk = k.shape[1]
diff --git a/include/ltxhip_rope.h b/include/ltxhip_rope.h
--- /dev/null
+++ b/include/ltxhip_rope.h
@@ -0,0 +1,22 @@
+#ifndef LTXHIP_ROPE_H
+#define LTXHIP_ROPE_H
+#include "ltxhip.h"
+#ifdef __cplusplus
+extern "C" {
+#endif
+
+int ltx_rope_coords_raster(const float* coords_host, int B, int F, int H, int W, int* raster);
+
+int ltx_op_rope_table_factored(float* cos_t, float* sin_t, float* cos_hw, float* sin_hw, const float* coords, int F, int H, int W, int D,
+                               const float* rope_scale_host, ltx_stream stream);
+
+int ltx_op_qknorm_rope_grid(void* x, int B, int F, int H, int W, int D, int ld, int nseg, int64_t seg_stride, const void* w0, const void* w1, const void* w0b,
+                            float eps, const float* coords, const float* coords_host, const float* rope_scale_host, float out_scale0, int dtype,
+                            char* route, int cap, ltx_stream stream);
+
+int ltx_dit_rope_form(const ltx_dit* m, int* factored);
+
+#ifdef __cplusplus
+}
+#endif
+#endif
diff --git a/rust/ltxhip-sys/src/lib.rs b/rust/ltxhip-sys/src/lib.rs
--- a/rust/ltxhip-sys/src/lib.rs
+++ b/rust/ltxhip-sys/src/lib.rs
@@ -359,6 +359,17 @@
                            stream: ltx_stream) -> c_int;
 }
 
+extern "C" {
+    pub fn ltx_rope_coords_raster(coords_host: *const c_float, b: c_int, f: c_int, h: c_int, w: c_int, raster: *mut c_int) -> c_int;
+    pub fn ltx_op_rope_table_factored(cos_t: *mut c_float, sin_t: *mut c_float, cos_hw: *mut c_float, sin_hw: *mut c_float, coords: *const c_float,
+                                      f: c_int, h: c_int, w: c_int, d: c_int, rope_scale_host: *const c_float, stream: ltx_stream) -> c_int;
+    pub fn ltx_op_qknorm_rope_grid(x: *mut c_void, b: c_int, f: c_int, h: c_int, w: c_int, d: c_int, ld: c_int, nseg: c_int, seg_stride: i64,
+                                   w0: *const c_void, w1: *const c_void, w0b: *const c_void, eps: c_float, coords: *const c_float,
+                                   coords_host: *const c_float, rope_scale_host: *const c_float, out_scale0: c_float, dtype: c_int,
+                                   route: *mut c_char, cap: c_int, stream: ltx_stream) -> c_int;
+    pub fn ltx_dit_rope_form(m: *const ltx_dit, factored: *mut c_int) -> c_int;
+}
+
 
 pub const LTX_RESCALE_CFG: c_int = 0;
 pub const LTX_RESCALE_MIX: c_int = 1;
```

Result: no change. 534.6 frames/sec, median of 6 (+0.6%).
